# humansensinglab/AGenDA

Hardware: AMD Instinct MI355X
Metric: 512x512 images/sec + DAAM heatmaps, 50 DDIM steps, SD-1.5 (higher is better)
Workload: dtype bf16

## Files before the change

### agenda_amd/_lib.py

```python
from __future__ import annotations

import ctypes as C
import os

_HERE = os.path.dirname(os.path.abspath(__file__))
LIB_PATH = os.environ.get("AGD_LIB") or os.path.join(_HERE, "libagenda_hip.so")
AGD_MAX_LEVELS = 8
AGD_N_CLASSES = 11


class AgdConfig(C.Structure):
    _fields_ = [
        ("struct_size", C.c_int),
        ("in_channels", C.c_int), ("out_channels", C.c_int), ("n_levels", C.c_int),
        ("block_out_channels", C.c_int * AGD_MAX_LEVELS),
        ("down_cross", C.c_int * AGD_MAX_LEVELS),
        ("num_heads", C.c_int * AGD_MAX_LEVELS),
        ("layers_per_block", C.c_int), ("cross_attention_dim", C.c_int),
        ("use_linear_projection", C.c_int), ("norm_num_groups", C.c_int),
        ("vae_latent_channels", C.c_int), ("vae_out_channels", C.c_int), ("vae_n_levels", C.c_int),
        ("vae_block_out_channels", C.c_int * AGD_MAX_LEVELS),
        ("vae_layers_per_block", C.c_int), ("vae_norm_num_groups", C.c_int),
        ("vae_scaling_factor", C.c_float),
        ("max_tokens", C.c_int),
# ... 70 lines not shown
    "agd_adapter_configure": (C.c_int, [_P, C.POINTER(AgdAdapterConfig)]),
    "agd_adapter_set_cond_hw": (C.c_int, [_P, _P, C.c_int, C.c_int, C.c_int, C.c_int, _P]),
    "agd_adapter_features": (C.c_int, [_P, _P]),
    "agd_adapter_set_schedule": (C.c_int, [_P, C.POINTER(C.c_float), C.c_int]),
    "agd_adapter_clear": (C.c_int, [_P]),
    "agd_adapter_add_counts": (C.c_int, [_P, C.POINTER(C.c_longlong)]),
    "agd_ip_adapter_begin": (C.c_int, [_P, C.c_int, C.c_int]),
    "agd_ip_adapter_tensor": (C.c_int, [_P, C.c_char_p, _P, C.c_int, C.c_int, C.POINTER(C.c_longlong)]),
    "agd_ip_adapter_commit": (C.c_int, [_P]),
    "agd_ip_adapter_unload": (C.c_int, [_P]),
    "agd_ip_adapter_set": (C.c_int, [_P, _P, C.c_int, C.c_float, _P]),
    "agd_ip_adapter_clear": (C.c_int, [_P]),
    "agd_ip_adapter_tokens": (C.c_int, [_P, _P]),
    "agd_ip_adapter_block": (C.c_int, [_P, C.c_char_p, _P, C.c_int, C.c_int, C.c_int, _P, _P]),
    "agd_ip_adapter_counts": (C.c_int, [_P, C.POINTER(C.c_longlong)]),
    "agd_image_encoder_begin": (C.c_int, [_P, C.POINTER(AgdVisionConfig)]),
    "agd_image_encoder_tensor": (C.c_int, [_P, C.c_char_p, _P, C.c_int, C.c_int, C.POINTER(C.c_longlong)]),
    "agd_image_encoder_commit": (C.c_int, [_P]),
    "agd_image_encoder_unload": (C.c_int, [_P]),
    "agd_image_embeds": (C.c_int, [_P, _P, C.c_int, C.c_int, C.c_int, _P, _P]),
    "agd_gligen_configure": (C.c_int, [_P, C.POINTER(AgdGligenConfig)]),
    "agd_gligen_set": (C.c_int, [_P, _P, _P, _P, C.c_int, _P]),
    "agd_gligen_set_schedule": (C.c_int, [_P, C.POINTER(C.c_int), C.c_int]),
    "agd_gligen_clear": (C.c_int, [_P]),
    "agd_gligen_objs": (C.c_int, [_P, _P]),
    "agd_gligen_fuser": (C.c_int, [_P, C.c_char_p, _P, C.c_int, C.c_int, C.c_int, _P, _P]),
    "agd_lora_add": (C.c_int, [_P, C.c_char_p, _P, _P, C.c_int, C.c_float]),
    "agd_lora_set_scale": (C.c_int, [_P, C.c_float, _P]),
    "agd_lora_clear": (C.c_int, [_P]),
    "agd_lora_count": (C.c_int, [_P]),
    "agd_lora_scale": (C.c_float, [_P]),
    "agd_unet_forward": (C.c_int, [_P, _P, C.c_int, C.c_int, C.c_float, _P, _P]),
    "agd_unet_forward_ts": (C.c_int, [_P, _P, C.c_int, C.c_int, C.POINTER(C.c_float), _P, _P]),
    "agd_cfg_ddim_step": (C.c_int, [_P, _P, _P, C.c_int, C.c_int, C.c_float, C.c_float, C.c_float, _P]),
    "agd_denoise": (C.c_int, [_P, _P, C.c_int, C.c_int, C.c_int, C.POINTER(C.c_float), C.POINTER(C.c_float),
                              C.POINTER(C.c_float), C.c_float, _P]),
    "agd_denoise_plms": (C.c_int, [_P, _P, C.c_int, C.c_int, C.c_int, C.POINTER(C.c_float), C.POINTER(C.c_float),
                                   C.POINTER(C.c_float), C.c_float, _P]),
    "agd_denoise_dpm": (C.c_int, [_P, _P, C.c_int, C.c_int, C.c_int, C.POINTER(C.c_float), C.POINTER(C.c_float), C.c_float, _P]),
    "agd_vae_decode": (C.c_int, [_P, _P, C.c_int, C.c_int, _P, _P, _P]),
    "agd_vae_encode": (C.c_int, [_P, _P, C.c_int, C.c_int, _P, _P, _P]),
    "agd_safety_scores_hw": (C.c_int, [_P, _P, C.c_int, C.c_int, C.c_int, _P, _P, _P]),
    "agd_controlnet_set_cond_hw": (C.c_int, [_P, _P, C.c_int, C.c_int, C.c_int, C.c_int, _P]),
    "agd_controlnet_residuals_hw": (C.c_int, [_P, _P, C.c_int, C.c_int, C.c_int, C.c_float, C.c_float, C.c_int, _P, C.POINTER(C.c_longlong), _P]),
    "agd_inpaint_prepare_hw": (C.c_int, [_P, _P, C.c_int, _P, C.c_int, C.c_int, C.c_int, C.c_int, _P, _P, _P, _P]),
    "agd_inpaint_set_hw": (C.c_int, [_P, _P, C.c_int, _P, C.c_int, _P, C.c_int, C.c_int, C.c_int, _P]),
    "agd_unet_forward_hw": (C.c_int, [_P, _P, C.c_int, C.c_int, C.c_int, C.c_float, _P, _P]),
    "agd_unet_forward_ts_hw": (C.c_int, [_P, _P, C.c_int, C.c_int, C.c_int, C.POINTER(C.c_float), _P, _P]),
    "agd_cfg_ddim_step_hw": (C.c_int, [_P, _P, _P, C.c_int, C.c_int, C.c_int, C.c_float, C.c_float, C.c_float, _P]),
    "agd_denoise_hw": (C.c_int, [_P, _P, C.c_int, C.c_int, C.c_int, C.c_int, C.POINTER(C.c_float), C.POINTER(C.c_float),
                                 C.POINTER(C.c_float), C.c_float, _P]),
    "agd_denoise_plms_hw": (C.c_int, [_P, _P, C.c_int, C.c_int, C.c_int, C.c_int, C.POINTER(C.c_float), C.POINTER(C.c_float),
                                      C.POINTER(C.c_float), C.c_float, _P]),
    "agd_denoise_dpm_hw": (C.c_int, [_P, _P, C.c_int, C.c_int, C.c_int, C.c_int, C.POINTER(C.c_float), C.POINTER(C.c_float), C.c_float, _P]),
    "agd_vae_decode_hw": (C.c_int, [_P, _P, C.c_int, C.c_int, C.c_int, _P, _P, _P]),
    "agd_vae_encode_hw": (C.c_int, [_P, _P, C.c_int, C.c_int, C.c_int, _P, _P, _P]),
    "agd_record_reset_hw": (C.c_int, [_P, C.c_int, C.c_int, C.c_int, _P]),
    "agd_set_option": (C.c_int, [_P, C.c_char_p, C.c_int]),
    "agd_record_config": (C.c_int, [_P, C.c_int, C.c_int, C.c_int]),
    "agd_record_reset": (C.c_int, [_P, C.c_int, C.c_int, _P]),
    "agd_daam_global": (C.c_int, [_P, C.c_int, C.c_int, _P, _P]),
    "agd_hook_global": (C.c_int, [_P, _P, _P]),
    "agd_hook_count": (C.c_int, [_P]),
    "agd_hook_last_map": (C.c_int, [_P, _P, C.c_int, _P]),
    "agd_cross_attn": (C.c_int, [_P, C.c_char_p, _P, _P, C.c_int, C.c_int, C.c_int, _P, C.c_int, _P]),
    "agd_attn_processor": (C.c_int, [_P, C.c_char_p, _P, _P, _P, C.c_int, C.c_int, C.c_int, _P, C.c_int, _P]),
    "agd_hook_reset": (C.c_int, [_P, C.c_int, C.c_int, _P]),
    "agd_hook_num_maps": (C.c_int, [_P]),
    "agd_hook_map_dims": (C.c_int, [_P, C.c_int, C.POINTER(C.c_int)]),
    "agd_hook_map": (C.c_int, [_P, C.c_int, _P, _P]),
    "agd_op_attn_reg_loss": (C.c_int, [_P, C.c_int, C.c_int, C.c_int, _P, _P, _P, C.c_float, _P, _P, _P]),
    "agd_attn_processor_backward": (C.c_int, [_P, C.c_char_p, _P, _P, _P, _P, C.c_int, C.c_int, C.c_int, C.c_int, _P, _P, _P]),
    "agd_op_conv2d": (C.c_int, [_P, _P, _P, _P] + [C.c_int] * 9 + [_P]),
    "agd_op_conv2d_ex": (C.c_int, [_P, _P, _P, _P] + [C.c_int] * 10 + [_P]),
    "agd_op_linear": (C.c_int, [_P, _P, _P, _P, _P, C.c_int, C.c_int, C.c_int, C.c_int, _P]),
    "agd_op_groupnorm": (C.c_int, [_P, _P, _P, _P, C.c_int, C.c_int, C.c_int, C.c_int, C.c_float, C.c_int, _P]),
    "agd_op_groupnorm_ex": (C.c_int, [_P] * 5 + [C.c_int] * 5 + [C.c_float, C.c_int, _P, C.c_int, _P, C.c_int, C.POINTER(C.c_int), _P]),
    "agd_op_gn_fold": (C.c_int, [_P, _P] + [C.c_int] * 5 + [C.c_float] + [_P] * 4 + [C.c_int, C.c_int] + [_P] * 5 + [_P]),
    "agd_op_conv_groupnorm": (C.c_int, [_P] * 6 + [C.c_int] * 6 + [C.c_float, C.c_int, C.c_int, _P]),
    "agd_op_layernorm": (C.c_int, [_P, _P, _P, _P, C.c_int, C.c_int, C.c_float, _P]),
    "agd_op_layernorm_ex": (C.c_int, [_P, _P, _P, _P, C.c_int, C.c_int, C.c_float, C.POINTER(C.c_int), _P]),
    "agd_op_ff_fused": (C.c_int, [_P] * 8 + [C.c_int, C.c_int, C.c_float, _P]),
    "agd_op_attn_chain": (C.c_int, [_P] * 9 + [C.c_int] * 5 + [C.c_float, _P]),
    "agd_op_xattn_premul": (C.c_int, [_P] * 9 + [C.c_int] * 5 + [C.c_float, _P]),
    "agd_op_attention": (C.c_int, [_P, _P, _P, _P, C.c_int, C.c_int, C.c_int, C.c_int, C.c_int, C.c_float, _P, _P]),
    "agd_op_attention_ex": (C.c_int, [_P, _P, _P, _P] + [C.c_int] * 5 + [C.c_float, C.c_int, _P, _P, _P, C.c_int, C.c_int, _P, C.c_int, C.c_int, C.c_int, _P]),
    "agd_op_attention_long": (C.c_int, [_P, _P, _P, _P] + [C.c_int] * 5 + [C.c_float, C.c_int, _P, C.c_int, C.c_int, _P]),
    "agd_op_attention_headsum": (C.c_int, [_P, _P, _P, _P, C.c_int, C.c_int, C.c_int, C.c_int, C.c_int, C.c_float, _P, _P]),
    "agd_op_attention_backward": (C.c_int, [_P, _P, _P, _P] + [C.c_int] * 6 + [C.c_float, _P, _P, _P]),
    "agd_op_hook_headmean": (C.c_int, [_P, C.c_int, C.c_int, C.c_int, C.c_int, _P, _P]),
    "agd_op_bicubic_clamp_mean": (C.c_int, [_P, C.c_int, C.c_int, C.c_int, C.c_int, _P, _P]),
    "agd_op_heatmap_u8": (C.c_int, [_P, C.c_int, C.c_int, _P, _P]),
    "agd_op_resize_u8_pil": (C.c_int, [_P, C.c_int, C.c_int, C.c_int, C.c_int, C.c_int, C.c_int, _P, _P]),
    "agd_op_stack_heatmaps": (C.c_int, [_P, _P, _P, C.c_longlong, _P, _P, _P]),
    "agd_op_window_gather": (C.c_int, [_P, _P] + [C.c_int] * 8 + [_P]),
    "agd_op_window_mean": (C.c_int, [_P, _P] + [C.c_int] * 6 + [_P]),
    "agd_denoise_panorama": (C.c_int, [_P, _P] + [C.c_int] * 7 + [C.POINTER(C.c_float)] * 3 + [C.c_float, _P]),
    "agd_daam_global_panorama": (C.c_int, [_P, C.c_int, C.c_int, _P, _P]),
    "agd_freeu_set": (C.c_int, [_P] + [C.c_float] * 4),
    "agd_freeu_clear": (C.c_int, [_P]),
    "agd_freeu_counts": (C.c_int, [_P, C.POINTER(C.c_longlong)]),
    "agd_op_freeu": (C.c_int, [_P, _P, _P, _P] + [C.c_int] * 5 + [C.c_float, C.c_float, _P]),
    "agd_guidance_rescale_set": (C.c_int, [_P, C.c_float]),
    "agd_guidance_rescale_clear": (C.c_int, [_P]),
    "agd_guidance_rescale_counts": (C.c_int, [_P, C.POINTER(C.c_longlong)]),
    "agd_op_guidance_rescale": (C.c_int, [_P, _P] + [C.c_int] * 4 + [C.c_float, C.c_float, _P, _P]),
    "agd_pag_set": (C.c_int, [_P, C.POINTER(C.c_float), C.c_int, C.POINTER(C.c_char_p), C.c_int]),
    "agd_pag_clear": (C.c_int, [_P]),
    "agd_pag_counts": (C.c_int, [_P, C.POINTER(C.c_longlong), C.POINTER(C.c_longlong)]),
    "agd_op_pag_v_rows": (C.c_int, [_P, _P, _P, C.c_int, C.c_int, _P]),
    "agd_op_pag_fold": (C.c_int, [_P, _P, C.c_longlong, C.c_float, _P]),
    "agd_deepcache_set": (C.c_int, [_P, C.POINTER(C.c_int), C.c_int, C.c_int]),
    "agd_deepcache_clear": (C.c_int, [_P]),
    "agd_deepcache_counts": (C.c_int, [_P, C.POINTER(C.c_longlong)]),
    "agd_deepcache_forward_hw": (C.c_int, [_P, _P, C.c_int, C.c_int, C.c_int, C.c_float, C.c_int, C.c_int, _P, _P]),
    "agd_op_deepcache_capture": (C.c_int, [_P, _P, _P, C.c_longlong, _P, _P, C.c_longlong, _P]),
    "agd_profile_begin": (C.c_int, [_P]),
    "agd_profile_end": (C.c_int, [_P, C.POINTER(C.c_double), C.POINTER(C.c_double), C.POINTER(C.c_longlong)]),
    "agd_profile_end_ex": (C.c_int, [_P, C.c_double, C.c_double] + [C.POINTER(C.c_double)] * 5 + [C.POINTER(C.c_longlong)]),
    "agd_profile_class_name": (C.c_char_p, [C.c_int]),
    "agd_version": (C.c_char_p, []),
}

EXPORTS = tuple(_SIGS.keys())
_lib = None


def load():
    global _lib
    if _lib is not None:
        return _lib
    if not os.path.exists(LIB_PATH):
        raise AgendaHipError(
            f"{LIB_PATH} not found: build it with `python -c 'import __graft_entry__ as g; g.build()'` "
            "or `make -C agenda_amd/csrc`. There is no CPU fallback.")
    lib = C.CDLL(LIB_PATH)
    for name, (res, args) in _SIGS.items():
        fn = getattr(lib, name)
        fn.restype = res
        fn.argtypes = args
    _lib = lib
    return lib


def check(rc: int, ctx=None, what: str = ""):
    if rc != 0:
        msg = load().agd_last_error(ctx)
        raise AgendaHipError(f"{what} failed (rc={rc}): {msg.decode() if msg else '?'}")


def ptr(t):
    if t is None:
        return None
    assert t.is_contiguous(), "tensor must be contiguous"
    return C.c_void_p(t.data_ptr())


def current_stream_ptr():
    import torch
    return C.c_void_p(torch.cuda.current_stream().cuda_stream)
```

### agenda_amd/csrc/kernels.h

```cpp
#pragma once
#include "common.h"

#define AGD_MAX_DEVICES 16
struct SplitKWs { float* p = nullptr; size_t cap = 0; };

struct IgemmP {
  const bf16_t* sc0 = nullptr; const bf16_t* sc1 = nullptr; int sc_C0 = 0, sc_C1 = 0;
  int ups4 = 0;
  const bf16_t* src0; const bf16_t* src1;
  int C0, C1;
  int Hin, Win, Hout, Wout;
  int ksize, stride, pad, up;
  const bf16_t* W;
  const float* bias; int bias_mode;
  const float* rowadd; int rowadd_ld;
  const bf16_t* residual; int ldr;
  void* out; int out_f32; int ldo;
  int M, N, K;
  float alpha;
  int geglu;
  int act;
  int batch;
  long long sA0, sA1, sW, sO, sR;
  const bf16_t* zero_page;
  SplitKWs* ws;
  float* splitk_ws;
  int colstat_rows;
  float* colstat_out;
  float* rowstat_out; int rowstat_slots;
  const float* ln_stats; int ln_slots; const float* ln_cs; float ln_invC, ln_eps;
  int* cfg_out;
  int w_per_image;
  int wmajor;
  int warm;
  int halo;
  int p8;
  const float* gn_gamma; const float* gn_beta; bf16_t* gn_y; int gn_groups; float gn_eps; int gn_silu; int gn_keep_out; int* gn_fused;
  int kg2;
  int smap;
  int wreg, wreg_mmin, wreg_mmax;
  const bf16_t* Wfrag; int wfrag_ni;
  int xb_m, xb_n;
  int xcd_block;
  int pc;
  int stagger;
  int dbg;
};
int launch_igemm(const IgemmP& p, hipStream_t st);
int igemm_query(const IgemmP& p, int* cfg3);

struct AttnP {
  const bf16_t* q; const bf16_t* k; const bf16_t* v; bf16_t* o;
  int ldq, ldk, ldv, ldo;
  long long sq, sk, sv, so;
  int B, H, D, Nq, Nk;
  float scale;
  int record_mode; int rec_b0;
  float* rec; long long rec_img_stride; long long rec_head_stride;
  int rec_T;
  int rec_hpb;
  int nqt;
  int causal;
  const float* mask;
  const bf16_t* k2; const bf16_t* v2; int ldk2, ldv2; long long sk2, sv2; int Nk2;
};
int launch_attention(const AttnP& p, hipStream_t st);
constexpr int ATTN_LONG_MAX_KEYS = 320;
int launch_attention_long(const AttnP& p, hipStream_t st);

struct FFusedP {
  const bf16_t* h; bf16_t* out;
  const bf16_t* w1f;
  const float* cs1; const float* b1;
  const bf16_t* w2f;
  const float* b2;
  int M; float ln_eps;
  const bf16_t* wpf; const float* bp; const bf16_t* xres; bf16_t* pout; float* colstat;
  int xres_rows;
  int premul;
};
int launch_ff_fused(const FFusedP& p, int C, hipStream_t st);
struct AttnChainP {
  const bf16_t* h; bf16_t* out;
  const float* gamma; const float* beta; float ln_eps;
  const bf16_t* wqf;
  const bf16_t* wof; const float* bo;
  const bf16_t* kv; int ldkv; long long skv;
  int M, HW, T; float scale;
  int record; float* rec; long long rec_img_stride, rec_head_stride; int rec_T, rec_b0, rec_hpb;
  float* rowstat_out;
  const bf16_t* o1; const bf16_t* wo1f; const float* bo1;
  int rows32;
  int src_rows;
};
int launch_attn_chain(const AttnChainP& p, int C, int heads, hipStream_t st);
struct QkvChainP {
  const bf16_t* x;
  const bf16_t* wbf; long long wb_stride; const float* rowadd;
  bf16_t* h;
  const float* gamma; const float* beta; float ln_eps;
  const bf16_t* wqkvf;
  bf16_t* qkv;
  int M, HW;
  long long rowadd_stride;
  const float* gn_part; int gn_bm, gn_groups; float gn_eps; const float* gn_gamma; const float* gn_beta;
  int rows64;
  int sched2;
};
int launch_qkv_chain(const QkvChainP& p, int C, hipStream_t st);
int launch_frag_order_w1(const bf16_t* src, bf16_t* dst, int C, int HID, hipStream_t st);
int launch_frag_order_w(const bf16_t* src, bf16_t* dst, int N, int K, int NI, int KC, hipStream_t st);

#define XATTN_TP 80
struct XattnPremulP {
  const bf16_t* kv; int ldkv; long long skv;
  const bf16_t* wqT;
  const bf16_t* wo;
  const float* gamma; const float* wqb;
  int B, T, C, H; float scale;
  bf16_t* kpp; float* kcs; float* kbs; bf16_t* vpp;
};
int launch_xattn_premul(const XattnPremulP& p, hipStream_t st);
struct XattnSP {
  const bf16_t* x;
  const float* ln_stats; int ln_slots; float ln_invC, ln_eps;
  const bf16_t* kpp; const float* kcs; const float* kbs;
  bf16_t* P;
  int M, HW, C, H, T;
  float* rec; long long rec_img_stride, rec_head_stride; int rec_T, rec_b0;
};
int launch_xattn_s(const XattnSP& p, hipStream_t st);
int launch_matvec_bf16(const bf16_t* W, const float* v, float* out, int N, int K, hipStream_t st);
int launch_rowstat_bf16(const bf16_t* x, float* out, int M, int C, hipStream_t st);

struct GroupNormP {
  const bf16_t* x0; const bf16_t* x1; int C0, C1;
  bf16_t* y;
  const float* gamma; const float* beta;
  int B, HW, groups; float eps; int silu;
  float* ws;
  const float* part0; const float* part1; int bm0, bm1;
  int* path;
};
int groupnorm_check(int B, int C0, int C1, int HW, int groups);
int layernorm_check(int rows, int C);
int launch_groupnorm(const GroupNormP& p, hipStream_t st);
int launch_gn_fold_weight(const float* part, int bm, int B, int HW, int C, int groups, float eps, const float* gamma, const float* beta,
                          const bf16_t* W, const float* bias, int N, bf16_t* Wb, float* rowadd, hipStream_t st, int frag_ni = 0);
long long groupnorm_ws_floats(int B, int C, int HW, int groups);
int launch_layernorm(const bf16_t* x, bf16_t* y, const float* g, const float* b, int rows, int C, float eps, hipStream_t st,
                     int* inst = nullptr);

int launch_convert_weight(const float* w, bf16_t* out, int N, int Cin, int taps, int Cpad, int geglu_bn, hipStream_t st);
int launch_f32_to_bf16(const float* x, bf16_t* y, long long n, hipStream_t st);
int launch_bf16_to_f32(const bf16_t* x, float* y, long long n, hipStream_t st);
bool igemm_can_fuse_shortcut(const IgemmP& p);
int launch_upsample_phase_weight(const bf16_t* w, bf16_t* out, int Cout, int Cin, hipStream_t st);
int launch_prep_latents(const float* lat_nchw, bf16_t* out_nhwc, int B, int C, int HW, int Cpad, int dup, float scale, hipStream_t st);
int launch_timestep_embed(float t, float* out, int dim, hipStream_t st);
int launch_small_linear(const float* x, const bf16_t* W, const float* bias, float* out, int M, int N, int K, int silu_in,
                        int silu_out, hipStream_t st);
int launch_cfg_ddim(const float* eps_nhwc, int ldc, float* lat_nchw, int B, int C, int HW, float guidance,
                    float a_t, float a_p, int vpred, const float* factor, hipStream_t st);
int launch_cfg_plms(const float* eps_nhwc, int ldc, float* lat, const float* src, const float* h1, const float* h2, const float* h3,
                    float* store, int B, int C, int HW, float guidance, const float* w4, float a, float b, const float* factor, hipStream_t st);
int launch_cfg_dpm(const float* eps_nhwc, int ldc, float* lat, const float* prev, float* store, int B, int C, int HW, float guidance,
                   const float* coef5 , const float* factor, hipStream_t st);
int launch_guidance_factor(const float* eps_nhwc, int ldc, int B, int C, int HW, float guidance, float phi, float* factor, hipStream_t st);
int launch_ln_fold_weight(const bf16_t* W, const float* gamma, const float* beta, const float* bias, int N, int K, int geglu_bn, bf16_t* Wf,
                          float* colsum, float* bias_f, hipStream_t st);
int launch_image_u8(const float* x_nhwc, int ldc, unsigned char* out, long long npix, int C, hipStream_t st);
int launch_nchw_from_nhwc_f32(const float* x, int ldc, float* out, int B, int C, int HW, hipStream_t st);
int launch_softmax_rows(const float* s, bf16_t* p, int rows, int cols, hipStream_t st);

struct HeatLayer { const float* acc; int h, w; int heads; long long img_stride; long long head_stride; };
int launch_daam_global(const HeatLayer* layers, int n_layers, int total_maps, int T, int Sh, int Sw, int img, float* out, hipStream_t st);
int launch_hook_accum(const float* map, int B, int T, int side, int S, float* sum, hipStream_t st);
int launch_scale(float* x, long long n, float s, hipStream_t st);
// ... 83 lines not shown
```

### agenda_amd/csrc/model.hip

```cpp
#include "../../include/agenda_hip.h"
#include "kernels.h"

#include <algorithm>
#include <cmath>
#include <cstdarg>
#include <cstdio>
#include <cstring>
#include <functional>
#include <string>
#include <unordered_map>
#include <unordered_set>
#include <vector>

static thread_local char g_err[2048] = "";
#define AGD_API extern "C" __attribute__((visibility("default")))
extern "C" void agd_set_error(const char* fmt, ...) {
  va_list ap; va_start(ap, fmt); vsnprintf(g_err, sizeof(g_err), fmt, ap); va_end(ap);
}
#define CK(expr) do { if ((expr) != 0) return -1; } while (0)
#define FAIL(...) do { agd_set_error(__VA_ARGS__); return -1; } while (0)

struct WMat { bf16_t* w = nullptr; int N = 0, Cin = 0, Cpad = 0, taps = 0;
              int sc_cols = 0;
              bf16_t* wfrag = nullptr; int wfrag_ni = 0; };
struct Act { bf16_t* p = nullptr; int B = 0, H = 0, W = 0, C = 0; float* cpart = nullptr; int cpart_bm = 0;
             bf16_t* normed = nullptr; const float* normed_gamma = nullptr;
             long long n() const { return (long long)B * H * W * C; } };
struct NextGn { const float* gamma = nullptr; const float* beta = nullptr; float eps = 0.f; int silu = 0; };

struct Arena {
  char* base = nullptr; size_t cap = 0, off = 0, peak = 0;
  void* alloc(size_t bytes) {
    size_t a = (off + 255) & ~(size_t)255;
    if (a + bytes > cap) { agd_set_error("activation arena exhausted: need %zu + %zu > %zu bytes (raise workspace_bytes)", a, bytes, cap); return nullptr; }
    off = a + bytes; if (off > peak) peak = off;
    return base + a;
  }
  size_t mark() const { return off; }
  void release(size_t m) { off = m; }
};

enum { PC_CONV3 = 0, PC_GEMM, PC_ATTN_SELF, PC_ATTN_CROSS, PC_GN, PC_LN, PC_ELEM, PC_HEAT, PC_VAE_ATTN, PC_OTHER, PC_TOUCH };
static const char* kClassNames[AGD_N_CLASSES] = {"igemm_conv3x3", "igemm_linear_1x1", "attn_self_flash", "attn_cross_daam",
                                                 "groupnorm", "layernorm", "elementwise", "heatmap", "vae_attn_softmax", "other", "weight_touch"};

struct DBuf {
  void* p = nullptr; size_t cap = 0;
  template <typename T> T* as() const { return (T*)p; }
  int ensure(size_t bytes) {
    if (p && bytes <= cap) return 0;
    if (p) { (void)hipDeviceSynchronize(); (void)hipFree(p); p = nullptr; cap = 0; }
    const size_t want = bytes ? bytes : 256;
    if (hipMalloc(&p, want) != hipSuccess) { p = nullptr; agd_set_error("hipMalloc(%zu) failed", want); return -1; }
    cap = want;
    return 0;
  }
  void release() { if (p) (void)hipFree(p); p = nullptr; cap = 0; }
};

struct XLayer {
  std::string name; int C = 0, heads = 0, level = 0; bool mid = false;
  bool cn = false;
  WMat wkv; DBuf kvb; bf16_t* kv = nullptr; DBuf accb; float* acc = nullptr; int acc_h = 0, acc_w = 0;
  int acc_heads = 0;
  DBuf wqTb, wkvTb, woTb; WMat wqT, wkvT, woT;
  bf16_t* pm_wqT = nullptr; float* pm_wqb = nullptr; bool pm_ready = false;
  DBuf pm_kppb, pm_vppb, pm_csb; bf16_t* pm_kpp = nullptr; bf16_t* pm_vpp = nullptr; float* pm_kcs = nullptr; float* pm_kbs = nullptr;
};

struct Fuser {
  std::string pre; int C = 0, heads = 0;
  WMat wqkv, wkv; float ta = 0.f, td = 0.f; float* bo_s = nullptr; float* b2_s = nullptr;
  DBuf gkvb;
};

struct IpaLayer {
  std::string pre; int C = 0, heads = 0, cols = 0;
  DBuf wk, wv, kppb, vppb, csbsb;
};

enum : int {
  TBF_FF            = 1 << 0,
  TBF_ATTN2         = 1 << 1,
  TBF_ATTN1_OUT     = 1 << 2,
  TBF_FF_PROJ       = 1 << 3,
  TBF_QKV           = 1 << 4,
  TBF_ATTN2_640     = 1 << 5,
  TBF_LAZY_DUP      = 1 << 6,
  TBF_QKV_GN        = 1 << 7,
  TBF_QKV_640       = 1 << 8,
  TBF_FF_PREMUL     = 1 << 9,
  TBF_ATTN2_ROWS32  = 1 << 10,
  TBF_QKV_ROWS64    = 1 << 11,
  TBF_QKV_SCHED2    = 1 << 12,
  TBF_DEFAULT       = 0x1fff & ~TBF_QKV_640,
};

struct ProfEv { int cls; double flops, bytes; hipEvent_t a, b; };

struct EvalCond {
  float cn_scale = 0.f;
  bool grounded = false;
  float ad_scale = 0.f;
  bool ipa = false;
  bool pag = false;
  int dc = 0;
  int dc_branch = 0;
};
enum : int { DC_CAPTURE = 1, DC_SHALLOW = 2 };

struct agd_ctx {
  int device = 0; agd_config cfg{}; std::string err;
  std::unordered_map<std::string, WMat> W;
  std::unordered_map<std::string, float*> V;
  std::unordered_map<std::string, int> Vn;
  std::vector<void*> owned;
  Arena arena; bf16_t* zero_page = nullptr;
  float* stage = nullptr; size_t stage_bytes = 0;
  bool finalized = false;
  WMat tproj_all; float* tproj_bias = nullptr; float* tproj_out = nullptr; int tproj_total = 0;
  const float* tproj_cur = nullptr;
  int tproj_cur_ld = 0;
  float* tsteps_buf = nullptr; int tsteps_cap = 0;
  std::unordered_map<std::string, int> tproj_off;
  float* temb_buf = nullptr;
  float* t_dev = nullptr;
  std::vector<XLayer> xl; std::unordered_map<std::string, int> xl_idx;
  DBuf ctxb; bf16_t* ctx_bf16 = nullptr; int ctx_B2 = 0, ctx_T = 0;
  int rec_mode = 0, rec_is_train = 0, rec_T_cfg = 0, rec_T = 0, rec_B = 0, rec_L = 0, rec_Lh = 0, rec_Lw = 0;
  DBuf hook_sumb, hook_scratchb, hook_headsb, hook_storeb;
  struct HookRec { size_t off; int Bp, T, N; };
  std::vector<HookRec> hook_recs; size_t hook_store_used = 0;
  DBuf bwd_wsb;
  float* hook_sum = nullptr; float* hook_scratch = nullptr; int hook_count = 0, hook_Bp = 0, hook_T = 0;
  int rec_base = 0, rec_call = 0;
  int pano_B = 0, pano_Lh = 0, pano_Lw = 0, pano_stride = 0;
  DBuf pano_ctxb;
  DBuf pano_viewb, pano_hmb;
  DBuf latb, epsb, vae_imgb, plmsb, dpmb;
  bf16_t* lat_bf16 = nullptr; float* eps_nhwc = nullptr;
  SplitKWs splitk;
  int opt_cfg_share = 1;
  int opt_ln_fold = 1;
  int opt_gn_fused = 1;
  int opt_warm = 3;
  int opt_gn_proj_fold = 1;
  int opt_p8 = 1;
  int opt_halo = 1;
  int opt_tb_fuse = TBF_DEFAULT;
  int opt_ups4 = 7;
  int opt_ffproj = 1;
  int opt_sc_fuse = 3;
  int opt_wreg = 3;
  int opt_kg2 = 1;
  int opt_side = 0;
  hipStream_t side = nullptr; hipEvent_t ev_fork = nullptr, ev_join = nullptr;
  int opt_smap = 1;
  int opt_reduce_gn = 1;
  int opt_xcd_block = 1;
  int opt_pc = 49;
  agd_vision_config vis{}; bool vis_on = false; float* vis_concepts = nullptr;
  agd_vision_config ienc{}; int ienc_state = 0;
  int opt_xpre = 1;
  int opt_touch = 3;
  unsigned* touch_sink = nullptr;
  agd_controlnet_config cnc{}; bool cn_on = false;
  WMat cn_tproj_all; float* cn_tproj_bias = nullptr; float* cn_tproj_out = nullptr; int cn_tproj_total = 0;
  int cn_nres = 0; float* cn_zb = nullptr; float* cn_zbs = nullptr; int cn_zb_total = 0; std::vector<int> cn_zb_off; float cn_zscale = NAN;
  DBuf cn_embb; int cn_emb_B2 = 0, cn_emb_Lh = 0, cn_emb_Lw = 0, cn_emb_rep = 0;
  std::vector<float> cn_sched;
  int ip_mode = 0, ip_B = 0, ip_Lh = 0, ip_Lw = 0, ip_Cm = 0, ip_Cc = 0;
  DBuf ip_maskb, ip_condb, ip_noiseb;
  std::vector<float> ip_sched;
  bool i2_on = false; int i2_B = 0, i2_Lh = 0, i2_Lw = 0; float i2_scale = 1.f;
  int i2_prep_B = 0, i2_prep_Lh = 0, i2_prep_Lw = 0;
  DBuf i2_latb;
  std::vector<std::string> lora_keys; std::vector<LoraMergeD> lora_d; int lora_tiles = 0;
// ... 340 lines not shown
  if (long_ctx && a.record_mode != 0) {
    const double fl = 6.0 * a.B * a.H * (double)a.Nq * a.Nk * a.D;
    const double by = 2.0 * a.B * a.H * (double)a.D * (2.0 * a.Nq + 3.0 * a.Nk) + 8.0 * (a.B - a.rec_b0) * a.H * (double)a.rec_T * a.Nq;
    ProfScope ps(c, st, PC_ATTN_CROSS, fl, by);
    CK(launch_attention_long(a, st));
  } else CK(run_attention(c, st, PC_ATTN_CROSS, a));
  if (hook_call) {
    ProfScope ps(c, st, PC_HEAT, 0);
    CK(launch_hook_headmean(c->hook_headsb.as<float>(), c->hook_Bp, xl.heads, T, N, c->hook_scratch, st));
    if (c->rec_is_train) {
      const size_t bytes = (size_t)c->hook_Bp * T * N * 4, need = c->hook_store_used + bytes;
      if (need > c->hook_storeb.cap) {
        DBuf bigger; CK(bigger.ensure(need * 2 > ((size_t)64 << 20) ? need * 2 : ((size_t)64 << 20)));
        if (c->hook_store_used && hipMemcpyAsync(bigger.p, c->hook_storeb.p, c->hook_store_used, hipMemcpyDeviceToDevice, st) != hipSuccess) FAIL("hook store copy");
        hipStreamSynchronize(st);
        c->hook_storeb.release(); c->hook_storeb = bigger;
      }
      if (hipMemcpyAsync((char*)c->hook_storeb.p + c->hook_store_used, c->hook_scratch, bytes, hipMemcpyDeviceToDevice, st) != hipSuccess) FAIL("hook store");
      c->hook_recs.push_back({c->hook_store_used, c->hook_Bp, T, N});
      c->hook_store_used = need;
    }
    CK(launch_hook_accum(c->hook_scratch, c->hook_Bp, T, side, c->rec_L, c->hook_sum, st));
    c->hook_count++;
  }
  return 0;
}

static int fuser_rows(agd_ctx* c, hipStream_t st, const Fuser& f, bf16_t* h, int B, int HW, bf16_t* qkv, bf16_t* att,
                      const std::function<int(const bf16_t*, int, const WMat&, const GemmOpt&)>& last) {
  const int C = f.C, D = C / f.heads, M = B * HW, NO = c->glc.max_objs;
  if (B != c->gl_B2) FAIL("gligen: the grounding objects are set for %d rows, this forward has %d (agd_gligen_set)", c->gl_B2, B);
  const std::string t = f.pre + "transformer_blocks.0.fuser.";
  bf16_t* n = (bf16_t*)c->arena.alloc((size_t)M * C * 2); bf16_t* ff = (bf16_t*)c->arena.alloc((size_t)M * 4 * C * 2);
  if (!n || !ff) return -1;
  GETV(g1, t + "norm1.weight"); GETV(b1, t + "norm1.bias"); GETV(g2, t + "norm2.weight"); GETV(b2, t + "norm2.bias");
  GETW(wo, t + "attn.to_out.0.weight"); GETW(w1, t + "ff.net.0.proj.weight"); GETV(bb1, t + "ff.net.0.proj.bias"); GETW(w2, t + "ff.net.2.weight");
  { ProfScope ps(c, st, PC_LN, 0, 4.0 * M * (double)C); CK(launch_layernorm(h, n, g1, b1, M, C, 1e-5f, st)); }
  { GemmOpt o; CK(run_conv(c, st, n, C, nullptr, 0, 1, 1, M, f.wqkv, 1, qkv, o, c->zero_page)); }
  AttnP a{}; a.q = qkv; a.k = qkv + C; a.v = qkv + 2 * C; a.o = att;
  a.ldq = a.ldk = a.ldv = 3 * C; a.ldo = C; a.sq = a.sk = a.sv = (long long)HW * 3 * C; a.so = (long long)HW * C;
  a.B = B; a.H = f.heads; a.D = D; a.Nq = HW; a.Nk = HW; a.scale = 1.0f / sqrtf((float)D);
  a.k2 = f.gkvb.as<bf16_t>(); a.v2 = a.k2 + C; a.ldk2 = a.ldv2 = 2 * C; a.sk2 = a.sv2 = (long long)NO * 2 * C; a.Nk2 = NO;
  { const double fl = 4.0 * B * f.heads * (double)HW * (HW + NO) * D, by = 2.0 * B * (double)C * (4.0 * HW + 2.0 * NO);
    ProfScope ps(c, st, PC_ATTN_SELF, fl, by); CK(launch_attention(a, st)); }
  { GemmOpt o; o.bias = f.bo_s; o.alpha = f.ta; o.residual = h; CK(run_conv(c, st, att, C, nullptr, 0, 1, 1, M, *wo, 1, h, o, c->zero_page)); }
  { ProfScope ps(c, st, PC_LN, 0, 4.0 * M * (double)C); CK(launch_layernorm(h, n, g2, b2, M, C, 1e-5f, st)); }
  { GemmOpt o; o.bias = bb1; o.geglu = 1; CK(run_conv(c, st, n, C, nullptr, 0, 1, 1, M, *w1, 1, ff, o, c->zero_page)); }
  GemmOpt o; o.bias = f.b2_s; o.alpha = f.td; o.residual = h;
  return last(ff, 4 * C, *w2, o);
}

static int dup_half(agd_ctx* c, hipStream_t st, bf16_t* p, long long half_elems) {
  ProfScope ps(c, st, PC_ELEM, 0);
  if (hipMemcpyAsync(p + half_elems, p, (size_t)half_elems * 2, hipMemcpyDeviceToDevice, st) != hipSuccess) FAIL("dup_half copy failed");
  return 0;
}

enum TbHead  { HEAD_GN,
               HEAD_FOLD,
               HEAD_QKV,
               HEAD_QKV_GN };
enum TbDup   { DUP_NONE, DUP_COPY,
               DUP_LAZY };
enum TbAttn2 { ATTN2_CHAIN,
               ATTN2_PREMUL,
               ATTN2_KERNELS };
enum TbFf    { FF_FUSED,
               FF_FUSED_PROJ,
               FF_FUSED_PREMUL,
               FF_FFPROJ,
               FF_PLAIN };

struct TBlockPlan {
  bool fold;
  bool x_normed;
  bool gfold;
  TbHead head; int qkv_rows64, qkv_sched2;
  bool attn1_in_chain;
  TbDup dup;
  const Fuser* fuser;
  const IpaLayer* ipa;
  XLayer* xl;
  TbAttn2 attn2; int chain_rows32;
  bool daam;
  TbFf ff;
  bool wreg_proj;
  bool stats_head, stats_attn1, stats_attn2;
  bool stats_ipa;
};

static const float kTbLnEps = 1e-5f;

struct TBlock {
  agd_ctx* c; hipStream_t st; const std::string& pre; const std::string t; const Act& x; Act& out; int heads, groups;
  int C, HW, Bs, B;
  const float* gn_g = nullptr; const float* gn_b = nullptr; const WMat* w_in = nullptr; const float* b_in = nullptr;
  bf16_t* ln = nullptr;
  bf16_t* h = nullptr; bf16_t* qkv = nullptr; bf16_t* att = nullptr;
  const bf16_t* xres;
  int M; const int Mshared;
  float* stats = nullptr; int slots = 0;
  bf16_t* ipaP = nullptr;
  TBlock(agd_ctx* c_, hipStream_t st_, const std::string& pre_, const Act& x_, Act& out_, int heads_, int groups_, int dup)
    : c(c_), st(st_), pre(pre_), t(pre_ + "transformer_blocks.0."), x(x_), out(out_), heads(heads_), groups(groups_), C(x_.C), HW(x_.H * x_.W),
      Bs(x_.B), B(dup ? 2 * x_.B : x_.B), xres(x_.p), M(x_.B * x_.H * x_.W), Mshared(M) {}

  int produce(const bf16_t* A, int K, const WMat& w, GemmOpt o, bool shaped, bool want_stats) {
    const int gb_ = shaped ? M / HW : 1, gh_ = shaped ? x.H : 1, gw_ = shaped ? x.W : M;
    stats = nullptr; slots = 0;
    if (want_stats) {
      int cfg[3] = {0, 0, 0}; GemmOpt qo = o; qo.query_cfg = cfg; qo.want_rowstat = 1;
      CK(run_conv(c, st, A, K, nullptr, 0, gb_, gh_, gw_, w, 1, h, qo, c->zero_page));
      slots = (w.N + cfg[1] - 1) / cfg[1];
      stats = (float*)c->arena.alloc((size_t)B * HW * slots * 2 * sizeof(float)); if (!stats) return -1;
      o.rowstat_out = stats; o.rowstat_slots = slots;
    }
    return run_conv(c, st, A, K, nullptr, 0, gb_, gh_, gw_, w, 1, h, o, c->zero_page);
  }
  int consume(bool fold, const std::string& lnkey, const std::string& wkey, const float* bias, int geglu, bf16_t* outp) {
    if (fold) {
      const std::string k = wkey + ".lnfold";
      GETW(wf, k); GETV(cs, k + ".cs"); GETV(bf, k + ".bias");
      GemmOpt o; o.bias = bf; o.geglu = geglu; o.ln_stats = stats; o.ln_slots = slots; o.ln_cs = cs; o.ln_invC = 1.0f / (float)C; o.ln_eps = kTbLnEps;
      if (geglu && C == 1280 && M >= 1024 && M <= 4096 && (c->opt_wreg & 1) && wf->wfrag) o.wreg = 2;
      return run_conv(c, st, h, C, nullptr, 0, 1, 1, M, *wf, 1, outp, o, c->zero_page);
    }
    GETV(g, lnkey + ".weight"); GETV(b, lnkey + ".bias");
    { ProfScope ps(c, st, PC_LN, 0, 4.0 * M * (double)C); CK(launch_layernorm(h, ln, g, b, M, C, kTbLnEps, st)); }
    GETW(w, wkey); GemmOpt o; o.bias = bias; o.geglu = geglu;
    return run_conv(c, st, ln, C, nullptr, 0, 1, 1, M, *w, 1, outp, o, c->zero_page);
  }
};

static TBlockPlan tblock_plan(const TBlock& s, int dup) {
  agd_ctx* c = s.c; const Act& x = s.x; const std::string& pre = s.pre; const std::string& t = s.t;
  const int C = s.C, HW = s.HW, heads = s.heads, groups = s.groups;
  auto tb = [c](int bit) { return (c->opt_tb_fuse & bit) != 0; };
  auto has = [c](const std::string& key) { return c->W.count(key) != 0; };
  TBlockPlan p{};
  p.fold = c->opt_ln_fold == 1 || (c->opt_ln_fold == 2 && C <= 320) || (c->opt_ln_fold == 3 && C <= 640);
  p.x_normed = x.normed && x.normed_gamma == s.gn_g;
  p.wreg_proj = C == 640 && (c->opt_wreg & 2);
  const bool sums = c->opt_gn_fused && x.cpart && x.cpart_bm > 0 && HW % x.cpart_bm == 0;
  p.gfold = c->opt_gn_proj_fold && sums && C <= (c->opt_gn_proj_fold >= 2 ? 640 : 320) && HW % 128 == 0;
  if (p.gfold) {
    const bool qkv = tb(TBF_QKV) && C == 320 && s.w_in->N == C && has(t + "attn1.qkv.frag");
    const bool gn_inside = qkv && tb(TBF_QKV_GN) && groups <= 32 && has(pre + "proj_in.frag");
    p.head = gn_inside ? HEAD_QKV_GN : qkv ? HEAD_QKV : HEAD_FOLD;
    p.qkv_rows64 = qkv && tb(TBF_QKV_ROWS64) && HW % 64 == 0;
  } else if (C == 640 && tb(TBF_QKV) && tb(TBF_QKV_640) && tb(TBF_QKV_GN) && sums && HW % 64 == 0 && groups <= 32 && !p.x_normed && !dup &&
             has(pre + "proj_in.frag") && has(t + "attn1.qkv.frag")) {
    p.head = HEAD_QKV_GN;
  } else p.head = HEAD_GN;
  p.qkv_sched2 = tb(TBF_QKV_SCHED2);
  const bool ff_fused = tb(TBF_FF) && p.fold && C == 320 && has(t + "ff.w1.frag");
  if (ff_fused) {
    const bool proj = tb(TBF_FF_PROJ) && has(pre + "proj_out.frag");
    p.ff = !proj ? FF_FUSED : tb(TBF_FF_PREMUL) && has(t + "ff.w2p.frag") ? FF_FUSED_PREMUL : FF_FUSED_PROJ;
  } else p.ff = c->opt_ffproj && has(pre + "ffproj.weight") ? FF_FFPROJ : FF_PLAIN;
  auto itx = c->xl_idx.find(t + "attn2");
  p.xl = itx == c->xl_idx.end() ? nullptr : &c->xl[itx->second];
  p.daam = p.xl && daam_records(c, *p.xl, s.B, x.H, x.W);
  const bool premul = p.xl && p.xl->pm_ready && c->opt_xpre && p.fold && HW % 64 == 0 && c->rec_mode != 2 && c->ctx_T <= XATTN_TP && !dup &&
                      (!p.daam || p.xl->acc_heads == p.xl->heads);
  const bool chain = !premul && tb(TBF_ATTN2) && (C == 320 || (C == 640 && tb(TBF_ATTN2_640))) && heads == 8 && HW % (C == 320 ? 128 : 64) == 0 &&
                     c->ctx_T <= 96 && c->rec_mode != 2 && has(t + "attn2.to_q.frag");
  p.attn2 = premul ? ATTN2_PREMUL : chain ? ATTN2_CHAIN : ATTN2_KERNELS;
  p.chain_rows32 = tb(TBF_ATTN2_ROWS32);
  if (c->cur.grounded) { auto itf = c->gl_idx.find(pre); if (itf != c->gl_idx.end()) p.fuser = &c->gl_f[itf->second]; }
  if (c->cur.ipa) { auto iti = c->ipa_idx.find(pre); if (iti != c->ipa_idx.end()) p.ipa = &c->ipa_l[iti->second]; }
  const bool lazy = dup && tb(TBF_LAZY_DUP) && chain && C == 320 && (p.ff == FF_FUSED_PROJ || p.ff == FF_FUSED_PREMUL) && !p.fuser && !p.ipa;
  p.dup = !dup ? DUP_NONE : lazy ? DUP_LAZY : DUP_COPY;
  p.attn1_in_chain = chain && tb(TBF_ATTN1_OUT) && p.dup != DUP_COPY && has(t + "attn1.to_out.frag") && !p.fuser && !p.ipa;
  p.stats_head = p.fold; p.stats_attn1 = p.fold && !chain; p.stats_attn2 = p.fold && !ff_fused && !p.ipa; p.stats_ipa = p.fold && !ff_fused && p.ipa;
  return p;
}

static int qkv_chain_params(const TBlock& s, const TBlockPlan& p, const bf16_t* wb, const float* radd, QkvChainP& qp) {
  agd_ctx* c = s.c; const Act& x = s.x; const int C = s.C;
  GETW(fqkv, s.t + "attn1.qkv.frag"); GETV(g1, s.t + "norm1.weight"); GETV(b1, s.t + "norm1.bias");
  qp.x = x.p; qp.wbf = wb; qp.wb_stride = (long long)s.w_in->N * C; qp.rowadd = radd; qp.rowadd_stride = C; qp.h = s.h; qp.gamma = g1; qp.beta = b1; qp.ln_eps = kTbLnEps;
  qp.wqkvf = fqkv->w; qp.qkv = s.qkv; qp.M = s.M; qp.HW = s.HW; qp.rows64 = p.qkv_rows64; qp.sched2 = p.qkv_sched2;
  if (p.head == HEAD_QKV_GN) {
    GETW(fpi, s.pre + "proj_in.frag");
    if (!s.b_in) FAIL("proj_in without bias");
    qp.wbf = fpi->w; qp.wb_stride = 0; qp.rowadd = s.b_in; qp.rowadd_stride = 0;
    qp.gn_part = x.cpart; qp.gn_bm = x.cpart_bm; qp.gn_groups = s.groups; qp.gn_eps = 1e-6f; qp.gn_gamma = s.gn_g; qp.gn_beta = s.gn_b;
  }
  return 0;
}

static int tb_head(TBlock& s, const TBlockPlan& p) {
  agd_ctx* c = s.c; hipStream_t st = s.st; const Act& x = s.x; const WMat* w = s.w_in; const int C = s.C;
  if (p.head == HEAD_GN) {
    if (p.x_normed) s.ln = x.normed;
    else CK(run_gn(c, st, x.p, C, nullptr, 0, s.Bs, s.HW, s.gn_g, s.gn_b, s.groups, 1e-6f, 0, s.ln, &x));
    GemmOpt o; o.bias = s.b_in;
    if (p.wreg_proj) o.wreg = 1;
    return s.produce(s.ln, C, *w, o, false, p.stats_head);
  }
  if (p.gfold) { if (w->taps != 1 || w->Cpad != C) FAIL("gn_proj_fold: proj_in weight [N=%d taps=%d Cpad=%d] is not a 1x1 over %d channels", w->N, w->taps, w->Cpad, C); }
  else if (w->taps != 1 || w->Cpad != C || w->N != C || !s.b_in) FAIL("qkv chain: proj_in weight [N=%d taps=%d Cpad=%d] is not a biased 1x1 over %d channels", w->N, w->taps, w->Cpad, C);
  bf16_t* wb = nullptr; float* radd = nullptr;
  if (p.head != HEAD_QKV_GN) {
    wb = (bf16_t*)c->arena.alloc((size_t)s.Bs * w->N * C * 2);
    radd = (float*)c->arena.alloc((size_t)s.Bs * w->N * sizeof(float));
    if (!wb || !radd) return -1;
    ProfScope ps(c, st, PC_GN, 0, 2.0 * s.Bs * (double)w->N * C * 2);
    CK(launch_gn_fold_weight(x.cpart, x.cpart_bm, s.Bs, s.HW, C, s.groups, 1e-6f, s.gn_g, s.gn_b, w->w, s.b_in, w->N, wb, radd, st, p.head == HEAD_QKV ? C / 64 : 0));
  }
  if (p.head == HEAD_FOLD) {
    WMat wi = *w; wi.w = wb;
    GemmOpt o; o.rowadd = radd; o.rowadd_ld = w->N; o.w_per_image = 1;
    return s.produce(x.p, C, wi, o, true, p.stats_head);
  }
  QkvChainP qp{}; CK(qkv_chain_params(s, p, wb, radd, qp));
  s.stats = nullptr; s.slots = 0;
  ProfScope ps(c, st, PC_GEMM, 8.0 * s.M * (double)C * C, 2.0 * s.M * (double)C * 5.0 + 2.0 * (p.gfold ? s.Bs + 3.0 : 4.0) * C * (double)C);
  return launch_qkv_chain(qp, C, st);
}

static int tb_self_attention(TBlock& s, const TBlockPlan& p) {
  agd_ctx* c = s.c; const std::string& t = s.t; const int C = s.C, HW = s.HW, D = C / s.heads;
  if (p.head == HEAD_GN || p.head == HEAD_FOLD) CK(s.consume(p.fold, t + "norm1", t + "attn1.qkv", nullptr, 0, s.qkv));
  AttnP a{}; a.q = s.qkv; a.k = s.qkv + C; a.v = s.qkv + 2 * C; a.o = s.att;
  a.ldq = a.ldk = a.ldv = 3 * C; a.ldo = C; a.sq = a.sk = a.sv = (long long)HW * 3 * C; a.so = (long long)HW * C;
  a.B = s.Bs; a.H = s.heads; a.D = D; a.Nq = HW; a.Nk = HW; a.scale = 1.0f / sqrtf((float)D);
  if (c->cur.pag && c->pag_layers.count(s.pre)) {
    const double M = (double)s.Bs * HW;
    ProfScope ps(c, s.st, PC_ELEM, 0, 4.0 * M * C);
    CK(launch_pag_v_rows(s.qkv, s.att, s.Bs * HW, C, s.st));
    c->pag_counts[1]++;
  } else CK(run_attention(c, s.st, PC_ATTN_SELF, a));
  if (p.attn1_in_chain) return 0;
  GETW(wo, t + "attn1.to_out.0.weight"); GETV(bo, t + "attn1.to_out.0.bias");
  GemmOpt oo; oo.bias = bo; oo.residual = s.h;
  return s.produce(s.att, C, *wo, oo, false, p.stats_attn1);
}

static int tb_duplicate(TBlock& s, const TBlockPlan& p) {
  agd_ctx* c = s.c; hipStream_t st = s.st; const int C = s.C, M = s.Mshared;
  if (p.dup == DUP_NONE) return 0;
  s.M = s.B * s.HW;
  if (p.dup == DUP_LAZY) return 0;
  CK(dup_half(c, st, s.h, (long long)M * C));
  if (p.stats_attn1) { ProfScope ps(c, st, PC_ELEM, 0);
    if (hipMemcpyAsync(s.stats + (size_t)M * s.slots * 2, s.stats, (size_t)M * s.slots * 2 * sizeof(float), hipMemcpyDeviceToDevice, st) != hipSuccess) FAIL("dup stats copy failed"); }
  Act x2 = alloc_act(c, s.B, s.x.H, s.x.W, C); if (!x2.p) return -1;
  { ProfScope ps(c, st, PC_ELEM, 0);
    if (hipMemcpyAsync(x2.p, s.x.p, (size_t)M * C * 2, hipMemcpyDeviceToDevice, st) != hipSuccess) FAIL("dup copy failed"); }
  CK(dup_half(c, st, x2.p, (long long)M * C));
  s.xres = x2.p;
  return 0;
}

static int tb_fuser(TBlock& s, const TBlockPlan& p) {
  return fuser_rows(s.c, s.st, *p.fuser, s.h, s.B, s.HW, s.qkv, s.att,
                    [&](const bf16_t* A, int K, const WMat& w, const GemmOpt& o) { return s.produce(A, K, w, o, false, p.stats_attn1); });
}

static int ipa_scores_rows(agd_ctx* c, hipStream_t st, const IpaLayer& l, const bf16_t* h, int B, int HW, bf16_t* P) {
  if (B != c->ipa_B2) FAIL("ip_adapter: the image tokens are set for %d rows, this forward has %d (agd_ip_adapter_set)", c->ipa_B2, B);
  IpaScoreP sp{}; sp.h = h; sp.kpp = l.kppb.as<bf16_t>(); sp.cs = l.csbsb.as<float>(); sp.bs = sp.cs + (size_t)B * l.cols; sp.P = P;
  sp.B = B; sp.HW = HW; sp.C = l.C; sp.H = l.heads; sp.nt = c->ipa_nt; sp.colsP = l.cols; sp.eps = 1e-5f;
  const double M = (double)B * HW;
  ProfScope ps(c, st, PC_ATTN_CROSS, 2.0 * M * l.cols * l.C, 2.0 * M * l.C + 2.0 * B * (double)l.cols * l.C + 2.0 * M * l.cols);
  return launch_ipa_scores(sp, st);
}
static int ipa_add_rows(agd_ctx* c, hipStream_t st, const IpaLayer& l, bf16_t* h, int B, int HW, const bf16_t* P) {
  IpaAddP ap{}; ap.h = h; ap.P = P; ap.vpp = l.vppb.as<bf16_t>(); ap.B = B; ap.HW = HW; ap.C = l.C; ap.colsP = l.cols; ap.s = c->ipa_scale;
  const double M = (double)B * HW;
  ProfScope ps(c, st, PC_ATTN_CROSS, 2.0 * M * l.cols * l.C, 4.0 * M * l.C + 2.0 * B * (double)l.cols * l.C + 2.0 * M * l.cols);
  return launch_ipa_add(ap, st);
}
static int tb_ip_adapter_scores(TBlock& s, const TBlockPlan& p) {
  agd_ctx* c = s.c;
  if (s.C != p.ipa->C) FAIL("ip_adapter: %s has %d channels, its to_k_ip / to_v_ip were loaded for %d", s.pre.c_str(), s.C, p.ipa->C);
  s.ipaP = (bf16_t*)c->arena.alloc((size_t)s.M * p.ipa->cols * 2); if (!s.ipaP) return -1;
  CK(ipa_scores_rows(c, s.st, *p.ipa, s.h, s.B, s.HW, s.ipaP));
  c->ipa_counts[0]++;
  return 0;
}
static int tb_ip_adapter_add(TBlock& s, const TBlockPlan& p) {
  agd_ctx* c = s.c;
  CK(ipa_add_rows(c, s.st, *p.ipa, s.h, s.B, s.HW, s.ipaP));
  c->ipa_counts[1]++;
  if (p.stats_ipa) {
    s.slots = 1; s.stats = (float*)c->arena.alloc((size_t)s.M * 2 * sizeof(float)); if (!s.stats) return -1;
    ProfScope ps(c, s.st, PC_LN, 0, 2.0 * s.M * (double)s.C);
    CK(launch_rowstat_bf16(s.h, s.stats, s.M, s.C, s.st));
  }
  return 0;
}

static int tb_attn2_chain(TBlock& s, const TBlockPlan& p) {
  agd_ctx* c = s.c; const std::string& t = s.t; const XLayer& xl = *p.xl; const int C = s.C, HW = s.HW, B = s.B, M = s.M, heads = s.heads;
  GETW(fq, t + "attn2.to_q.frag"); GETW(fo, t + "attn2.to_out.frag");
  GETV(g2, t + "norm2.weight"); GETV(b2, t + "norm2.bias"); GETV(bo, t + "attn2.to_out.0.bias");
  const int T = c->ctx_T, D = C / heads;
  AttnChainP ap{}; ap.h = s.h; ap.out = s.h; ap.gamma = g2; ap.beta = b2; ap.ln_eps = kTbLnEps; ap.wqf = fq->w; ap.wof = fo->w; ap.bo = bo;
  ap.kv = xl.kv; ap.ldkv = 2 * C; ap.skv = (long long)T * 2 * C; ap.M = M; ap.HW = HW; ap.T = T; ap.scale = 1.0f / sqrtf((float)D);
  double rec_bytes = 0;
  if (p.daam) {
    ap.record = 1; ap.rec_b0 = B / 2; ap.rec_T = c->rec_T; ap.rec_hpb = heads / xl.acc_heads;
    ap.rec_head_stride = (long long)c->rec_T * HW; ap.rec_img_stride = ap.rec_head_stride * xl.acc_heads;
    ap.rec = xl.acc + (size_t)c->rec_base * ap.rec_img_stride;
    rec_bytes = 8.0 * (B - ap.rec_b0) * xl.acc_heads * (double)c->rec_T * HW;
  }
  if (p.attn1_in_chain || p.dup == DUP_LAZY) {
    ap.out = (bf16_t*)c->arena.alloc((size_t)M * C * 2); if (!ap.out) return -1;
  }
  if (p.attn1_in_chain) {
    GETW(f1o, t + "attn1.to_out.frag"); GETV(bo1, t + "attn1.to_out.0.bias");
    ap.o1 = s.att; ap.wo1f = f1o->w; ap.bo1 = bo1;
  }
  if (p.dup == DUP_LAZY) ap.src_rows = s.Mshared;
  ap.rows32 = p.chain_rows32;
  if (p.stats_attn2) {
    s.slots = 1; s.stats = (float*)c->arena.alloc((size_t)M * 2 * sizeof(float)); if (!s.stats) return -1;
    ap.rowstat_out = s.stats;
  }
  const double gemms = p.attn1_in_chain ? 6.0 : 4.0;
  ProfScope ps(c, s.st, PC_ATTN_CROSS, gemms * M * (double)C * C + 4.0 * B * heads * (double)HW * T * D, gemms * M * (double)C + gemms * C * (double)C + 4.0 * B * (double)T * C + rec_bytes);
  CK(launch_attn_chain(ap, C, heads, s.st));
  s.h = ap.out;
  return 0;
}

static int tb_attn2_premul(TBlock& s, const TBlockPlan& p) {
  agd_ctx* c = s.c; const XLayer& xl = *p.xl; const int C = s.C, HW = s.HW, B = s.B, M = s.M, heads = s.heads;
  if (!s.stats || s.slots <= 0) FAIL("attn2_premul: the GEMM in front of attn2 left no row statistics for norm2");
  GETV(bo, s.t + "attn2.to_out.0.bias");
  const int HT = heads * XATTN_TP;
  bf16_t* P = (bf16_t*)c->arena.alloc((size_t)M * HT * 2); if (!P) return -1;
  XattnSP sp{}; sp.x = s.h; sp.ln_stats = s.stats; sp.ln_slots = s.slots; sp.ln_invC = 1.0f / (float)C; sp.ln_eps = kTbLnEps;
  sp.kpp = xl.pm_kpp; sp.kcs = xl.pm_kcs; sp.kbs = xl.pm_kbs; sp.P = P; sp.M = M; sp.HW = HW; sp.C = C; sp.H = heads; sp.T = c->ctx_T;
  double rec_bytes = 0;
  if (p.daam) {
    sp.rec_b0 = B / 2; sp.rec_T = c->rec_T; sp.rec_head_stride = (long long)c->rec_T * HW; sp.rec_img_stride = sp.rec_head_stride * xl.acc_heads;
    sp.rec = xl.acc + (size_t)c->rec_base * sp.rec_img_stride;
    rec_bytes = 8.0 * (B - sp.rec_b0) * heads * (double)c->rec_T * HW;
  }
  { ProfScope ps(c, s.st, PC_ATTN_CROSS, 2.0 * M * (double)HT * C, 2.0 * M * (double)C + 2.0 * B * (double)HT * C + 2.0 * M * (double)HT + rec_bytes);
    CK(launch_xattn_s(sp, s.st)); }
  WMat wv; wv.w = xl.pm_vpp; wv.N = C; wv.Cin = HT; wv.Cpad = HT; wv.taps = 1;
  GemmOpt oo; oo.bias = bo; oo.residual = s.h; oo.w_per_image = 1;
  return s.produce(P, HT, wv, oo, true, p.stats_attn2);
}

static int tb_attn2(TBlock& s, const TBlockPlan& p) {
  agd_ctx* c = s.c; const std::string& t = s.t;
  if (!p.xl) FAIL("cross-attn layer %s not registered", (t + "attn2").c_str());
  if (c->ctx_B2 != s.B) FAIL("context batch %d != unet batch %d (call agd_set_context)", c->ctx_B2, s.B);
  if (p.attn2 == ATTN2_CHAIN) return tb_attn2_chain(s, p);
  if (p.attn2 == ATTN2_PREMUL) return tb_attn2_premul(s, p);
  CK(s.consume(p.fold, t + "norm2", t + "attn2.to_q.weight", nullptr, 0, s.qkv));
  CK(cross_attention(c, s.st, *p.xl, s.qkv, s.B, s.HW, s.x.H, s.x.W, s.att, true));
  GETW(wo, t + "attn2.to_out.0.weight"); GETV(bo, t + "attn2.to_out.0.bias");
  GemmOpt oo; oo.bias = bo; oo.residual = s.h;
  return s.produce(s.att, s.C, *wo, oo, false, p.stats_attn2);
}

static int tb_ff_fused(TBlock& s, const TBlockPlan& p) {
  agd_ctx* c = s.c; const std::string& t = s.t; Act& out = s.out; const int C = s.C, M = s.M;
  GETW(f1, t + "ff.w1.frag"); GETW(f2, t + "ff.w2.frag");
  const std::string k = t + "ff.net.0.proj.weight.lnfold";
  GETV(cs, k + ".cs"); GETV(bf, k + ".bias"); GETV(b2, t + "ff.net.2.bias");
  FFusedP fp{}; fp.h = s.h; fp.out = s.h; fp.w1f = f1->w; fp.cs1 = cs; fp.b1 = bf; fp.w2f = f2->w; fp.b2 = b2; fp.M = M; fp.ln_eps = kTbLnEps;
  const bool proj = p.ff != FF_FUSED;
  if (proj) {
    GETW(fpw, s.pre + "proj_out.frag"); GETV(bp, s.pre + "proj_out.bias");
    fp.wpf = fpw->w; fp.bp = bp; fp.xres = s.xres; fp.pout = out.p;
    if (p.ff == FF_FUSED_PREMUL) {
      GETW(f2p, t + "ff.w2p.frag"); GETV(bcp, s.pre + "ffproj.bias");
      fp.w2f = f2p->w; fp.bp = bcp; fp.premul = 1;
    }
    if (p.dup == DUP_LAZY) fp.xres_rows = s.Mshared;
    out.cpart_bm = 0;
    if (out.cpart && c->opt_gn_fused && s.HW % 128 == 0) { fp.colstat = out.cpart; out.cpart_bm = 128; }
  }
  ProfScope ps(c, s.st, PC_GEMM, 2.0 * M * (double)C * (proj ? 13.0 : 12.0) * C, (proj ? 8.0 : 4.0) * M * (double)C + 2.0 * (proj ? 13.0 : 12.0) * C * (double)C);
  return launch_ff_fused(fp, C, s.st);
}

static int tb_feed_forward(TBlock& s, const TBlockPlan& p) {
  agd_ctx* c = s.c; hipStream_t st = s.st; const std::string& t = s.t; const int C = s.C, M = s.M;
  if (p.ff == FF_FUSED || p.ff == FF_FUSED_PROJ || p.ff == FF_FUSED_PREMUL) CK(tb_ff_fused(s, p));
  else {
    bf16_t* ff = (bf16_t*)c->arena.alloc((size_t)M * 4 * C * 2); if (!ff) return -1;
    GETV(b1, t + "ff.net.0.proj.bias");
    CK(s.consume(p.fold, t + "norm3", t + "ff.net.0.proj.weight", b1, 1, ff));
    if (p.ff == FF_FFPROJ) {
      GETW(wc, s.pre + "ffproj.weight"); GETV(bc, s.pre + "ffproj.bias");
      GemmOpt o; o.bias = bc; o.residual = s.xres; o.out_act = &s.out; o.rows_per_image = s.HW;
      return run_conv(c, st, ff, 4 * C, s.h, C, 1, 1, M, *wc, 1, s.out.p, o, c->zero_page);
    }
    GETW(w2, t + "ff.net.2.weight"); GETV(b2, t + "ff.net.2.bias");
    GemmOpt o2; o2.bias = b2; o2.residual = s.h;
    CK(run_conv(c, st, ff, 4 * C, nullptr, 0, 1, 1, M, *w2, 1, s.h, o2, c->zero_page));
  }
  if (p.ff != FF_FUSED && p.ff != FF_PLAIN) return 0;
  GETW(w, s.pre + "proj_out.weight"); GETV(b, s.pre + "proj_out.bias");
  GemmOpt o; o.bias = b; o.residual = s.xres; o.out_act = &s.out; o.rows_per_image = s.HW;
  if (p.wreg_proj) o.wreg = 1;
  return run_conv(c, st, s.h, C, nullptr, 0, 1, 1, M, *w, 1, s.out.p, o, c->zero_page);
}

static int transformer(agd_ctx* c, hipStream_t st, const std::string& pre, const Act& x, int heads, int groups, Act& out, int dup = 0) {
  TBlock s(c, st, pre, x, out, heads, groups, dup);
  const int B = s.B, HW = s.HW, C = s.C;
  out = alloc_act(c, B, x.H, x.W, C, true); if (!out.p) return -1;
  const size_t mk = c->arena.mark();
  Act n = alloc_act(c, B, x.H, x.W, C); if (!n.p) return -1;
  Act h = alloc_act(c, B, x.H, x.W, C); if (!h.p) return -1;
  s.ln = n.p; s.h = h.p;
  s.qkv = (bf16_t*)c->arena.alloc((size_t)B * HW * 3 * C * 2); if (!s.qkv) return -1;
  s.att = (bf16_t*)c->arena.alloc((size_t)B * HW * C * 2); if (!s.att) return -1;
  GETV(gg, pre + "norm.weight"); GETV(gb, pre + "norm.bias"); GETW(w_in, pre + "proj_in.weight"); GETV(b_in, pre + "proj_in.bias");
  s.gn_g = gg; s.gn_b = gb; s.w_in = w_in; s.b_in = b_in;
  const TBlockPlan p = tblock_plan(s, dup);
  CK(tb_head(s, p));
  CK(tb_self_attention(s, p));
  CK(tb_duplicate(s, p));
  if (p.fuser) CK(tb_fuser(s, p));
  if (p.ipa) CK(tb_ip_adapter_scores(s, p));
  CK(tb_attn2(s, p));
  if (p.ipa) CK(tb_ip_adapter_add(s, p));
  CK(tb_feed_forward(s, p));
  c->arena.release(mk);
  return 0;
}

static int time_embed(agd_ctx* c, hipStream_t st, const float* ts, int n, float* scratch, float* out, bool cn = false) {
  const int dim = c->cfg.block_out_channels[0], td = dim * 4;
  const std::string pre = cn ? "controlnet." : "unet.";
  ProfScope ps(c, st, PC_ELEM, 0);
  float* e0 = scratch; float* e1 = e0 + (size_t)n * dim; float* e2 = e1 + (size_t)n * td;
  for (int i = 0; i < n; ++i) CK(launch_timestep_embed(ts[i], e0 + (size_t)i * dim, dim, st));
  GETW(w1, pre + "time_embedding.linear_1.weight"); GETV(b1, pre + "time_embedding.linear_1.bias");
  GETW(w2, pre + "time_embedding.linear_2.weight"); GETV(b2, pre + "time_embedding.linear_2.bias");
  CK(launch_small_linear(e0, w1->w, b1, e1, n, td, w1->Cpad, 0, 1, st));
  CK(launch_small_linear(e1, w2->w, b2, e2, n, td, w2->Cpad, 0, 0, st));
  if (cn) CK(launch_small_linear(e2, c->cn_tproj_all.w, c->cn_tproj_bias, out, n, c->cn_tproj_total, td, 1, 0, st));
  else CK(launch_small_linear(e2, c->tproj_all.w, c->tproj_bias, out, n, c->tproj_total, td, 1, 0, st));
  return 0;
}

static int adapter_add(agd_ctx* c, hipStream_t st, int level, const Act& h, Act& out);
static int down_mid_walk(agd_ctx* c, hipStream_t st, const std::string& u, const bf16_t* xin, int B2, int Lh, int Lw, bool shared,
                         const bf16_t* conv_in_res, const std::function<int(const Act&)>& on_sample, Act& h, int stop_layer = -1) {
  const agd_config& g = c->cfg;
  const int nl = g.n_levels, G = g.norm_num_groups;
  const int Bh = shared ? B2 / 2 : B2;
  const bool inject = c->cur.ad_scale != 0.f && u == "unet.";
  h = alloc_act(c, B2, Lh, Lw, g.block_out_channels[0], true); if (!h.p) return -1;
  { GETW(w, u + "conv_in.weight"); GETV(b, u + "conv_in.bias"); GemmOpt o; o.bias = b; o.out_act = &h; o.residual = conv_in_res;
    CK(run_conv(c, st, xin, 64, nullptr, 0, Bh, Lh, Lw, *w, 3, h.p, o, c->zero_page)); }
  if (shared) {
    CK(dup_half(c, st, h.p, (long long)Bh * Lh * Lw * h.C));
    if (h.cpart_bm > 0) {
      const size_t nb = (size_t)((long long)Bh * Lh * Lw / h.cpart_bm) * h.C * 2 * sizeof(float);
      if (hipMemcpyAsync((char*)h.cpart + nb, h.cpart, nb, hipMemcpyDeviceToDevice, st) != hipSuccess) FAIL("dup partials copy failed");
    }
  }
// ... 2018 lines not shown
  int bm = 0;
  if (fused) {
    int cfg[3] = {0, 0, 0};
    CK(igemm_query(p, cfg));
    bm = cfg[0];
    if (cfg[2] != 1 || bm < 1 || HW % bm || HW % 64) { agd_set_error("op_conv_groupnorm: shape not eligible for producer statistics (tile %d, splits %d)", cfg[0], cfg[2]); return -1; }
    p.colstat_out = part; p.colstat_rows = HW;
  }
  CK(launch_igemm(p, st));
  GroupNormP g{}; g.x0 = hb; g.C0 = Cout; g.y = yb; g.gamma = gamma; g.beta = beta; g.B = B; g.HW = HW; g.groups = groups; g.eps = eps; g.silu = silu; g.ws = ws;
  if (fused) { g.part0 = part; g.bm0 = bm; }
  CK(launch_groupnorm(g, st));
  CK(launch_bf16_to_f32(yb, yf, (long long)B * HW * Cout, st));
  CK(launch_nchw_from_nhwc_f32(yf, Cout, y, B, Cout, HW, st));
  hipStreamSynchronize(st);
  return 0;
}

AGD_API int agd_op_layernorm_ex(const float* x, const float* gamma, const float* beta, float* y, int rows, int C, float eps, int* inst, void* stream) {
  hipStream_t st = S(stream); Tmp tmp;
  if (inst) *inst = 0;
  if (layernorm_check(rows, C)) return -1;
  bf16_t* xb = tmp.get<bf16_t>((size_t)rows * C); bf16_t* yb = tmp.get<bf16_t>((size_t)rows * C);
  if (!xb || !yb) return -1;
  CK(launch_f32_to_bf16(x, xb, (long long)rows * C, st));
  CK(launch_layernorm(xb, yb, gamma, beta, rows, C, eps, st, inst));
  CK(launch_bf16_to_f32(yb, y, (long long)rows * C, st));
  hipStreamSynchronize(st);
  return 0;
}
AGD_API int agd_op_layernorm(const float* x, const float* gamma, const float* beta, float* y, int rows, int C, float eps, void* stream) {
  return agd_op_layernorm_ex(x, gamma, beta, y, rows, C, eps, nullptr, stream);
}

AGD_API int agd_op_ff_fused(const float* x, const float* gamma, const float* beta, const float* w1, const float* b1, const float* w2,
                            const float* b2, float* y, int M, int C, float eps, void* stream) {
  hipStream_t st = S(stream); Tmp tmp;
  if (C != 320) { agd_set_error("op_ff_fused: C = %d (320 only)", C); return -1; }
  const int H8 = 8 * C, H4 = 4 * C;
  bf16_t* xb = tmp.get<bf16_t>((size_t)M * C); bf16_t* yb = tmp.get<bf16_t>((size_t)M * C);
  bf16_t* w1b = tmp.get<bf16_t>((size_t)H8 * C); bf16_t* w1l = tmp.get<bf16_t>((size_t)H8 * C); bf16_t* w1f = tmp.get<bf16_t>((size_t)H8 * C);
  bf16_t* w2b = tmp.get<bf16_t>((size_t)C * H4); bf16_t* w2f = tmp.get<bf16_t>((size_t)C * H4);
  float* cs = tmp.get<float>(H8); float* bf = tmp.get<float>(H8);
  if (!xb || !yb || !w1b || !w1l || !w1f || !w2b || !w2f || !cs || !bf) return -1;
  CK(launch_f32_to_bf16(x, xb, (long long)M * C, st));
  CK(launch_convert_weight(w1, w1b, H8, C, 1, C, 16, st));
  CK(launch_ln_fold_weight(w1b, gamma, beta, b1, H8, C, 16, w1l, cs, bf, st));
  CK(launch_frag_order_w1(w1l, w1f, C, H4, st));
  CK(launch_convert_weight(w2, w2b, C, H4, 1, H4, 0, st));
  CK(launch_frag_order_w(w2b, w2f, C, H4, C / 64, 128, st));
  FFusedP fp{}; fp.h = xb; fp.out = yb; fp.w1f = w1f; fp.cs1 = cs; fp.b1 = bf; fp.w2f = w2f; fp.b2 = b2; fp.M = M; fp.ln_eps = eps;
  CK(launch_ff_fused(fp, C, st));
  CK(launch_bf16_to_f32(yb, y, (long long)M * C, st));
  hipStreamSynchronize(st);
  return 0;
}

AGD_API int agd_op_attn_chain(const float* x, const float* gamma, const float* beta, const float* wq, const float* kv, const float* wo,
                              const float* bo, float* y, float* probs_sum, int B, int HW, int T, int C, int heads, float eps, void* stream) {
  hipStream_t st = S(stream); Tmp tmp;
  const long long M = (long long)B * HW;
  bf16_t* xb = tmp.get<bf16_t>((size_t)M * C); bf16_t* yb = tmp.get<bf16_t>((size_t)M * C); bf16_t* kvb = tmp.get<bf16_t>((size_t)B * T * 2 * C);
  bf16_t* wqb = tmp.get<bf16_t>((size_t)C * C); bf16_t* wqf = tmp.get<bf16_t>((size_t)C * C);
  bf16_t* wob = tmp.get<bf16_t>((size_t)C * C); bf16_t* wof = tmp.get<bf16_t>((size_t)C * C);
  if (!xb || !yb || !kvb || !wqb || !wqf || !wob || !wof) return -1;
  if (C != 320 && C != 640) { agd_set_error("op_attn_chain: C %d", C); return -1; }
  CK(launch_f32_to_bf16(x, xb, M * C, st));
  CK(launch_f32_to_bf16(kv, kvb, (long long)B * T * 2 * C, st));
  CK(launch_convert_weight(wq, wqb, C, C, 1, C, 0, st)); CK(launch_frag_order_w(wqb, wqf, C, C, 5, C, st));
  CK(launch_convert_weight(wo, wob, C, C, 1, C, 0, st)); CK(launch_frag_order_w(wob, wof, C, C, 5, C, st));
  AttnChainP ap{}; ap.h = xb; ap.out = yb; ap.gamma = gamma; ap.beta = beta; ap.ln_eps = eps; ap.wqf = wqf; ap.wof = wof; ap.bo = bo;
  ap.rows32 = (heads >> 8) & 1; heads &= 255;
  ap.kv = kvb; ap.ldkv = 2 * C; ap.skv = (long long)T * 2 * C; ap.M = (int)M; ap.HW = HW; ap.T = T; ap.scale = 1.0f / sqrtf((float)(C / heads));
  if (probs_sum) {
    if (hipMemsetAsync(probs_sum, 0, (size_t)B * T * HW * 4, st) != hipSuccess) { agd_set_error("memset probs"); return -1; }
    ap.record = 1; ap.rec = probs_sum; ap.rec_b0 = 0; ap.rec_T = T; ap.rec_hpb = heads; ap.rec_head_stride = (long long)T * HW; ap.rec_img_stride = (long long)T * HW;
  }
  CK(launch_attn_chain(ap, C, heads, st));
  CK(launch_bf16_to_f32(yb, y, M * C, st));
  hipStreamSynchronize(st);
  return 0;
}

AGD_API int agd_op_xattn_premul(const float* x, const float* gamma, const float* beta, const float* wq, const float* kv, const float* wo,
                                const float* bo, float* y, float* probs, int B, int HW, int T, int C, int heads, float eps, void* stream) {
  hipStream_t st = S(stream); Tmp tmp;
  const long long M = (long long)B * HW;
  if (heads < 1 || C % heads || (C / heads) % 8 || C % 160 || C % 64 || HW % 64 || T < 1 || T > XATTN_TP || (heads * XATTN_TP) % 64) { agd_set_error("op_xattn_premul: C %d heads %d HW %d T %d", C, heads, HW, T); return -1; }
  const size_t HT = (size_t)heads * XATTN_TP;
  bf16_t* xb = tmp.get<bf16_t>((size_t)M * C); bf16_t* yb = tmp.get<bf16_t>((size_t)M * C); bf16_t* kvb = tmp.get<bf16_t>((size_t)B * T * 2 * C);
  bf16_t* wqb = tmp.get<bf16_t>((size_t)C * C); bf16_t* wqT = tmp.get<bf16_t>((size_t)C * C); bf16_t* wob = tmp.get<bf16_t>((size_t)C * C);
  float* wqbeta = tmp.get<float>(C); float* rst = tmp.get<float>((size_t)M * 2);
  bf16_t* kpp = tmp.get<bf16_t>((size_t)B * HT * C); bf16_t* vpp = tmp.get<bf16_t>((size_t)B * HT * C); float* kcs = tmp.get<float>((size_t)B * HT * 2);
  bf16_t* P = tmp.get<bf16_t>((size_t)M * HT);
  if (!xb || !yb || !kvb || !wqb || !wqT || !wob || !wqbeta || !rst || !kpp || !vpp || !kcs || !P) return -1;
  CK(launch_f32_to_bf16(x, xb, M * C, st));
  CK(launch_f32_to_bf16(kv, kvb, (long long)B * T * 2 * C, st));
  CK(launch_convert_weight(wq, wqb, C, C, 1, C, 0, st)); CK(launch_transpose_bf16(wqb, C, C, wqT, st));
  CK(launch_convert_weight(wo, wob, C, C, 1, C, 0, st));
  CK(launch_matvec_bf16(wqb, beta, wqbeta, C, C, st));
  CK(launch_rowstat_bf16(xb, rst, (int)M, C, st));
  XattnPremulP pm{}; pm.kv = kvb; pm.ldkv = 2 * C; pm.skv = (long long)T * 2 * C; pm.wqT = wqT; pm.wo = wob; pm.gamma = gamma; pm.wqb = wqbeta;
  pm.B = B; pm.T = T; pm.C = C; pm.H = heads; pm.scale = 1.0f / sqrtf((float)(C / heads)); pm.kpp = kpp; pm.kcs = kcs; pm.kbs = kcs + (size_t)B * HT; pm.vpp = vpp;
  CK(launch_xattn_premul(pm, st));
  XattnSP sp{}; sp.x = xb; sp.ln_stats = rst; sp.ln_slots = 1; sp.ln_invC = 1.0f / (float)C; sp.ln_eps = eps; sp.kpp = kpp; sp.kcs = pm.kcs; sp.kbs = pm.kbs; sp.P = P;
  sp.M = (int)M; sp.HW = HW; sp.C = C; sp.H = heads; sp.T = T;
  if (probs) {
    if (hipMemsetAsync(probs, 0, (size_t)B * heads * T * HW * 4, st) != hipSuccess) { agd_set_error("memset probs"); return -1; }
    sp.rec = probs; sp.rec_b0 = 0; sp.rec_T = T; sp.rec_head_stride = (long long)T * HW; sp.rec_img_stride = sp.rec_head_stride * heads;
  }
  CK(launch_xattn_s(sp, st));
  WMat wv; wv.w = vpp; wv.N = C; wv.Cin = (int)HT; wv.Cpad = (int)HT; wv.taps = 1;
  GemmOpt oo; oo.bias = bo; oo.residual = xb; oo.w_per_image = 1;
  CK(run_conv(nullptr, st, P, (int)HT, nullptr, 0, B, 1, HW, wv, 1, yb, oo, op_zero_page()));
  CK(launch_bf16_to_f32(yb, y, M * C, st));
  hipStreamSynchronize(st);
  return 0;
}

AGD_API int agd_op_attention(const float* q, const float* k, const float* v, float* o, int B, int H, int D, int Nq, int Nk,
                                float scale, float* probs_out, void* stream) {
  hipStream_t st = S(stream); Tmp tmp;
  const int C = H * D;
  bf16_t* qb = tmp.get<bf16_t>((size_t)B * Nq * C); bf16_t* kb = tmp.get<bf16_t>((size_t)B * Nk * C);
  bf16_t* vb = tmp.get<bf16_t>((size_t)B * Nk * C); bf16_t* ob = tmp.get<bf16_t>((size_t)B * Nq * C);
  if (!qb || !kb || !vb || !ob) return -1;
  CK(launch_f32_to_bf16(q, qb, (long long)B * Nq * C, st));
  CK(launch_f32_to_bf16(k, kb, (long long)B * Nk * C, st));
  CK(launch_f32_to_bf16(v, vb, (long long)B * Nk * C, st));
  AttnP a{}; a.q = qb; a.k = kb; a.v = vb; a.o = ob; a.ldq = a.ldk = a.ldv = a.ldo = C;
  a.sq = (long long)Nq * C; a.so = a.sq; a.sk = (long long)Nk * C; a.sv = a.sk;
  a.B = B; a.H = H; a.D = D; a.Nq = Nq; a.Nk = Nk; a.scale = scale;
  if (probs_out) {
    if (hipMemsetAsync(probs_out, 0, (size_t)B * H * Nk * Nq * 4, st) != hipSuccess) { agd_set_error("memset probs"); return -1; }
    a.record_mode = 1; a.rec_b0 = 0; a.rec = probs_out; a.rec_T = Nk;
    a.rec_head_stride = (long long)Nk * Nq; a.rec_img_stride = a.rec_head_stride * H;
  }
  CK(launch_attention(a, st));
  CK(launch_bf16_to_f32(ob, o, (long long)B * Nq * C, st));
  hipStreamSynchronize(st);
  return 0;
}

AGD_API int agd_op_attention_ex(const float* q, const float* k, const float* v, float* o, int B, int H, int D, int Nq, int Nk, float scale,
                                int causal, const float* mask, const float* k2, const float* v2, int Nk2, int layout, float* probs_out,
                                int record, int rec_b0, int rec_T, void* stream) {
  if (D != 32 && D != 40 && D != 64 && D != 80 && D != 128 && D != 160) { agd_set_error("attention_ex: unsupported head dim D=%d", D); return -1; }
  if (B < 1 || H < 1 || Nq < 1 || Nk < 1) { agd_set_error("attention_ex: bad shape B=%d H=%d Nq=%d Nk=%d", B, H, Nq, Nk); return -1; }
  if (!q || !k || !v || !o) { agd_set_error("attention_ex: q, k, v and o are required"); return -1; }
  if (layout < 0 || layout > 2) { agd_set_error("attention_ex: layout=%d (0 packed, 1 fused q|k|v rows, 2 fused k|v rows)", layout); return -1; }
  if (layout == 1 && Nq != Nk) { agd_set_error("attention_ex: layout=1 (fused q|k|v rows) needs Nq == Nk (got Nq=%d Nk=%d)", Nq, Nk); return -1; }
  if (record < 0 || record > 2 || (record != 0) != (probs_out != nullptr)) { agd_set_error("attention_ex: record=%d needs probs_out, and probs_out needs record 1 or 2", record); return -1; }
  if (record && Nk > 96) { agd_set_error("attention_ex: recording needs Nk <= 96 (got Nk=%d)", Nk); return -1; }
  if (record && (rec_b0 < 0 || rec_b0 > B)) { agd_set_error("attention_ex: rec_b0=%d outside [0, %d]", rec_b0, B); return -1; }
  if (record && (rec_T < 1 || rec_T > Nk)) { agd_set_error("attention_ex: rec_T=%d outside [1, %d]", rec_T, Nk); return -1; }
  if ((k2 != nullptr) != (v2 != nullptr)) { agd_set_error("attention_ex: k2 and v2 come together"); return -1; }
  if (!k2 && Nk2 != 0) { agd_set_error("attention_ex: Nk2=%d without a second source", Nk2); return -1; }
  hipStream_t st = S(stream); Tmp tmp;
  const int C = H * D;
  const long long nq = (long long)B * Nq * C, nk = (long long)B * Nk * C, nk2 = k2 ? (long long)B * (Nk2 > 0 ? Nk2 : 0) * C : 0;
  bf16_t* qb = tmp.get<bf16_t>((size_t)nq); bf16_t* kb = tmp.get<bf16_t>((size_t)nk); bf16_t* vb = tmp.get<bf16_t>((size_t)nk);
  bf16_t* ob = tmp.get<bf16_t>((size_t)nq);
  bf16_t* k2b = k2 ? tmp.get<bf16_t>((size_t)nk2 + 8) : nullptr; bf16_t* v2b = k2 ? tmp.get<bf16_t>((size_t)nk2 + 8) : nullptr;
  bf16_t* fused = layout ? tmp.get<bf16_t>((size_t)(layout == 1 ? 3 : 2) * nk) : nullptr;
  bf16_t* fused2 = (layout && k2) ? tmp.get<bf16_t>((size_t)2 * nk2 + 8) : nullptr;
  if (!qb || !kb || !vb || !ob || (k2 && (!k2b || !v2b)) || (layout && !fused) || (layout && k2 && !fused2)) return -1;
// ... 1587 lines not shown
```

### agenda_amd/csrc/tblock.hip

```cpp
#include "kernels.h"
#include <type_traits>

typedef __attribute__((ext_vector_type(2))) float f32x2_t;
#ifdef AGD_EXPERIMENTS
int g_tb_variant = 0;
extern "C" __attribute__((visibility("default"))) void agd_set_tb_variant(int v) { g_tb_variant = v; }
#endif
#ifdef AGD_STAMPS
__device__ unsigned long long g_tb_ts[256];
__device__ int g_tb_ts_sel[2] = {-1, 0};
extern "C" __attribute__((visibility("default"))) int agd_tb_ts(int wg, int wave, unsigned long long* out) {
  if (out) return hipMemcpyFromSymbol(out, HIP_SYMBOL(g_tb_ts), 256 * 8) == hipSuccess ? 0 : -1;
  const int sel[2] = {wg, wave};
  return hipMemcpyToSymbol(HIP_SYMBOL(g_tb_ts_sel), sel, 8) == hipSuccess ? 0 : -1;
}
#define TB_TS_DECL const bool ts_on = (int)blockIdx.x == g_tb_ts_sel[0] && (int)threadIdx.x == g_tb_ts_sel[1] * 64; int ts_n = 0; if (ts_on) g_tb_ts[250] = __builtin_amdgcn_s_memrealtime();
#define TB_TS(k) do { if (ts_on && ts_n < 240) g_tb_ts[ts_n++] = ((unsigned long long)(k) << 56) | (__builtin_amdgcn_s_memtime() & 0x00FFFFFFFFFFFFFFull); } while (0)
#define TB_TS_END do { if (ts_on) { asm volatile("s_waitcnt vmcnt(0)" ::: "memory"); TB_TS(99); g_tb_ts[255] = ts_n; g_tb_ts[251] = __builtin_amdgcn_s_memrealtime(); } } while (0)
#else
#define TB_TS_DECL
#define TB_TS(k) do { } while (0)
#define TB_TS_END do { } while (0)
#endif

// ... 33 lines not shown
}
int launch_frag_order_w(const bf16_t* src, bf16_t* dst, int N, int K, int NI, int KC, hipStream_t st) {
  if (N % (NI * 16) || K % KC || KC % 32) { agd_set_error("frag_order_w: N %d K %d NI %d KC %d", N, K, NI, KC); return -1; }
  hipLaunchKernelGGL(frag_order_w_kernel, dim3(1024), dim3(256), 0, st, src, dst, N, K, NI, KC);
  HIP_CHECK_RET(hipGetLastError());
  return 0;
}

#define TB_OOB 0x80000000u
template <int C> AGD_DEV int panel_swz(int ch, int row) {
  if constexpr ((C * 2) % 256 == 128) return (ch & ~7) | ((ch & 7) ^ ((row >> 1) & 7));
  else return (ch & ~15) | ((ch & 15) ^ (row & 15));
}
template <int C> struct XOff {
  static constexpr int XG = ((C * 2) % 256 == 128) ? 2 : 4;
  int xo[4];
  AGD_DEV XOff(int q, int px) {
#pragma unroll
    for (int t = 0; t < 4; ++t) xo[t] = ((C * 2) % 256 == 128) ? (((4 * (t & 1) + q) ^ ((px >> 1) & 7)) << 4) : (((4 * t + q) ^ px) << 4);
  }
  AGD_DEV int at(int ks) const { return (ks / XG) * (XG * 64) + xo[ks % XG]; }
};

template <int C, int BM = 128, int NW = 8>
AGD_DEV void panel_load_dma(const bf16_t* src, int m0, int M, char* panel, int wid, int lane) {
  constexpr int CHR = C / 8, PIECES = BM * CHR / 64;
  static_assert(PIECES % NW == 0, "pieces split evenly over the workgroup's waves");
#pragma unroll
  for (int i = 0; i < PIECES / NW; ++i) {
    const int piece = i * NW + wid, pos = piece * 64 + lane;
    const int row = pos / CHR, pc = pos - row * CHR;
    const int lc = panel_swz<C>(pc, row);
    const int m = m0 + row;
    const unsigned voff = m < M ? (unsigned)(((long long)m * C + lc * 8) * 2) : TB_OOB;
    bufdma16(src, panel + piece * 1024, voff, 0u);
  }
}

template <int C, int BM = 128>
AGD_DEV void panel_row_stats(const char* panel, float* lnst, int tid, float eps) {
  constexpr int CHR = C / 8, TPR = 512 / BM, PER = CHR / TPR;
  static_assert(CHR % TPR == 0, "chunks per row split over the row's threads");
  const int row = tid / TPR, part = tid % TPR;
  float S = 0.f, Q = 0.f;
#pragma unroll
  for (int cc = 0; cc < PER; ++cc) {
    const u32x4 v = *(const u32x4*)(panel + row * (C * 2) + panel_swz<C>(part * PER + cc, row) * 16);
#pragma unroll
    for (int e = 0; e < 4; ++e) {
      const float a = __uint_as_float(v[e] << 16), b = __uint_as_float(v[e] & 0xFFFF0000u);
      S += a + b; Q += a * a + b * b;
    }
  }
#pragma unroll
  for (int o = 1; o < TPR; o <<= 1) { S += __shfl_xor(S, o); Q += __shfl_xor(Q, o); }
  if (part == 0) {
    const float mu = S * (1.0f / C);
    float var = Q * (1.0f / C) - mu * mu; var = var < 0.f ? 0.f : var;
    *(f32x2_t*)(lnst + row * 2) = f32x2_t{mu, rsqrtf(var + eps)};
  }
}

typedef u32x4 __attribute__((aligned(8))) u32x4_a8;
template <int NI> AGD_DEV void load_row_chunk(const bf16_t* p, u32x2 (&r)[NI]) {
#pragma unroll
  for (int t = 0; t + 1 < NI; t += 2) { const u32x4 v = *(const u32x4_a8*)(p + 4 * t); r[t] = u32x2{v[0], v[1]}; r[t + 1] = u32x2{v[2], v[3]}; }
  if (NI & 1) r[NI - 1] = *(const u32x2*)(p + 4 * (NI - 1));
}
template <int NI> AGD_DEV void store_row_chunk(bf16_t* p, const u32x2 (&r)[NI]) {
#pragma unroll
  for (int t = 0; t + 1 < NI; t += 2) *(u32x4_a8*)(p + 4 * t) = u32x4{r[t][0], r[t][1], r[t + 1][0], r[t + 1][1]};
  if (NI & 1) *(u32x2*)(p + 4 * (NI - 1)) = r[NI - 1];
}

#define TB_F 10
#define TB_D 8
template <int C>
AGD_DEV void panel_gemm_head(u32x4 (&ring)[TB_F], const bf16_t* wf, unsigned wbase, unsigned lane16, unsigned wbytes = C * C * 2) {
  const auto wrs = __builtin_amdgcn_make_buffer_rsrc((void*)wf, 0, wbytes, 0x00020000);
#pragma unroll
  for (int f = 0; f < TB_D; ++f) ring[f % TB_F] = __builtin_bit_cast(u32x4, __builtin_amdgcn_raw_buffer_load_b128(wrs, lane16, wbase + (unsigned)f * 1024u, 0));
}
struct TbNoHook { AGD_DEV void operator()() const {} };
template <int C, bool ZERO = true, int MI = 4, class Late = TbNoHook>
AGD_DEV void panel_gemm_body(u32x4 (&ring)[TB_F], f32x4 (&acc)[MI][5], const bf16_t* wf, unsigned wbase, unsigned lane16, const char* xrow, const XOff<C>& xo,
                             unsigned wbytes = C * C * 2, Late&& late = Late()) {
  constexpr int NI = 5, KS = C / 32, NFR = KS * NI, PITCH = C * 2;
  const auto wrs = __builtin_amdgcn_make_buffer_rsrc((void*)wf, 0, wbytes, 0x00020000);
  if constexpr (ZERO) {
#pragma unroll
  for (int i = 0; i < MI; ++i)
#pragma unroll
    for (int j = 0; j < NI; ++j) acc[i][j] = f32x4{0.f, 0.f, 0.f, 0.f};
  }
  bf16x8 xf[MI];
#pragma unroll
  for (int f = 0; f < NFR; ++f) {
    if (f + TB_D < NFR) ring[(f + TB_D) % TB_F] = __builtin_bit_cast(u32x4, __builtin_amdgcn_raw_buffer_load_b128(wrs, lane16, wbase + (unsigned)(f + TB_D) * 1024u, 0));
    if (f == NFR - TB_D) late();
    __builtin_amdgcn_sched_barrier(0);
    if (f % NI == 0) {
      const int ks = f / NI;
#pragma unroll
      for (int i = 0; i < MI; ++i) xf[i] = *(const bf16x8*)(xrow + i * 16 * PITCH + xo.at(ks));
    }
#pragma unroll
    for (int i = 0; i < MI; ++i)
      acc[i][f % NI] = __builtin_amdgcn_mfma_f32_16x16x32_bf16(__builtin_bit_cast(bf16x8, ring[f % TB_F]), xf[i], acc[i][f % NI], 0, 0, 0);
  }
}

template <int C, int VAR = 0, int POST = 0>
__global__ __launch_bounds__(512, 2) void ff_fused_kernel(const FFusedP p) {
  constexpr int BM = 128, HID = 4 * C, HC = 128, NCH = HID / HC, KS1 = C / 32, KS2 = HC / 32, NI2 = C / 64;
  constexpr int PITCH = C * 2;
  static_assert(C % 64 == 0 && (C / 8) % 8 == 0 && KS1 % 2 == 0, "panel geometry");
  extern __shared__ __attribute__((aligned(16))) char smem[];
  char* panel = smem;
  char* hbuf = smem + BM * PITCH;
  float* lnst = (float*)(hbuf + 2 * BM * HC * 2);
  float* cbufs = lnst + BM * 2;

  const int tid = threadIdx.x, lane = tid & 63;
  const int wid = __builtin_amdgcn_readfirstlane(tid >> 6);
  const int mh = wid >> 2, nq = wid & 3;
  const int m0 = blockIdx.x * BM;
  TB_TS_DECL
  TB_TS(1);

  panel_load_dma<C>(p.h, m0, p.M, panel, wid, lane);
  asm volatile("s_waitcnt vmcnt(0)" ::: "memory");
  __syncthreads();
  panel_row_stats<C>(panel, lnst, tid, p.ln_eps);
  { const auto cs1r0 = __builtin_amdgcn_make_buffer_rsrc((void*)p.cs1, 0, (unsigned)(2 * HID * 4), 0x00020000);
    const auto b1r0 = __builtin_amdgcn_make_buffer_rsrc((void*)p.b1, 0, (unsigned)(2 * HID * 4), 0x00020000);
    const unsigned off = (unsigned)((((tid >> 7) & 1) ? HID : 0) + (tid & (HC - 1))) * 4u;
    ((float*)(hbuf + 2 * BM * HC * 2) + BM * 2)[tid] = __builtin_bit_cast(float, wid < 4 ? __builtin_amdgcn_raw_buffer_load_b32(cs1r0, off, 0, 0) : __builtin_amdgcn_raw_buffer_load_b32(b1r0, off, 0, 0)); }
  __syncthreads();

  f32x4 acc2[4][NI2];
#pragma unroll
  for (int i = 0; i < 4; ++i)
#pragma unroll
    for (int j = 0; j < NI2; ++j) acc2[i][j] = f32x4{0.f, 0.f, 0.f, 0.f};
  f32x4 acc1[4][4];

  const auto w1rs = __builtin_amdgcn_make_buffer_rsrc((void*)p.w1f, 0, (unsigned)(2 * HID * C * 2), 0x00020000);
  const auto w2rs = __builtin_amdgcn_make_buffer_rsrc((void*)p.w2f, 0, (unsigned)(HID * C * 2), 0x00020000);
#define ldw1(sbase, f) __builtin_bit_cast(u32x4, __builtin_amdgcn_raw_buffer_load_b128(w1rs, lane16, (sbase) + (unsigned)(f) * 1024u, 0))
#define ldw2(sbase, f) __builtin_bit_cast(u32x4, __builtin_amdgcn_raw_buffer_load_b128(w2rs, lane16, (sbase) + (unsigned)(f) * 1024u, 0))
  constexpr bool NOW = (VAR & 2) != 0, NOX = (VAR & 4) != 0;

  constexpr int F = TB_F, D = TB_D, DX = 2, N2 = KS2 * NI2, N1 = KS1 * 4;
  static_assert((N1 + N2) % F == 0 && D < F && D <= N2 && DX <= D, "ring geometry");
  u32x4 ring[F];

  auto lane_now = [&]() __attribute__((always_inline)) { int l = lane; asm volatile("" : "+v"(l)); return l; };
  auto gemm2 = [&](int c, bool pre, bool has_next, unsigned nexts) __attribute__((always_inline)) {
    const int l_ = lane_now(), q = l_ >> 4, px = l_ & 15;
    const unsigned lane16 = (unsigned)l_ * 16u;
    const char* hb = hbuf + (c & 1) * (BM * HC * 2) + (64 * mh + px) * (HC * 2);
    const unsigned wp = __builtin_amdgcn_readfirstlane((unsigned)(((c * 4 + nq) * KS2) * NI2) * 1024u);
    if (!pre && !NOW) {
#pragma unroll
      for (int f = 0; f < DX; ++f) ring[f % F] = ldw2(wp, f);
    }
    if constexpr (!NOW) {
#pragma unroll
      for (int f = DX; f < D; ++f) ring[f % F] = ldw2(wp, f);
    }
    bf16x8 hf[4];
#pragma unroll
    for (int f = 0; f < N2; ++f) {
      const int tgt = f + D;
      if constexpr (!NOW) {
        if (tgt < N2) ring[tgt % F] = ldw2(wp, tgt);
        else if (has_next) ring[tgt % F] = ldw1(nexts, tgt - N2);
      }
      __builtin_amdgcn_sched_barrier(0);
      if (f % NI2 == 0 && (!NOX || f == 0)) {
#pragma unroll
        for (int i = 0; i < 4; ++i) hf[i] = *(const bf16x8*)(hb + i * 16 * (HC * 2) + (((4 * (f / NI2) + q) ^ px) << 4));
      }
#pragma unroll
      for (int i = 0; i < 4; ++i)
        acc2[i][f % NI2] = __builtin_amdgcn_mfma_f32_16x16x32_bf16(__builtin_bit_cast(bf16x8, ring[f % F]), hf[i], acc2[i][f % NI2], 0, 0, 0);
    }
  };

  auto gemm1 = [&](int c, bool pre, bool has_next, unsigned nexts) __attribute__((always_inline)) {
#pragma unroll
    for (int i = 0; i < 4; ++i)
#pragma unroll
      for (int j = 0; j < 4; ++j) acc1[i][j] = f32x4{0.f, 0.f, 0.f, 0.f};
    const unsigned wp = __builtin_amdgcn_readfirstlane((unsigned)(((c * 4 + nq) * KS1) * 4) * 1024u);
    const int l_ = lane_now(), q = l_ >> 4, px = l_ & 15;
    const unsigned lane16 = (unsigned)l_ * 16u;
    const int sx = (px >> 1) & 7;
    const int xoff0 = ((q ^ sx) << 4), xoff1 = (((4 + q) ^ sx) << 4);
    const char* xrow = panel + (64 * mh + px) * PITCH;
    if (!pre && !NOW) {
#pragma unroll
      for (int f = 0; f < D; ++f) ring[(N2 + f) % F] = ldw1(wp, f);
    }
    bf16x8 xf[4];
#pragma unroll
    for (int f = 0; f < N1; ++f) {
      const int tgt = f + D;
      if constexpr (!NOW) {
        if (tgt < N1) ring[(N2 + tgt) % F] = ldw1(wp, tgt);
        else if (has_next && tgt - N1 < DX) ring[(N2 + tgt) % F] = ldw2(nexts, tgt - N1);
      }
      __builtin_amdgcn_sched_barrier(0);
      if (f % 4 == 0 && (!NOX || f == 0)) {
        const int ks = f / 4;
#pragma unroll
        for (int i = 0; i < 4; ++i) xf[i] = *(const bf16x8*)(xrow + i * 16 * PITCH + (ks >> 1) * 128 + ((ks & 1) ? xoff1 : xoff0));
      }
#pragma unroll
      for (int i = 0; i < 4; ++i)
        acc1[i][f % 4] = __builtin_amdgcn_mfma_f32_16x16x32_bf16(__builtin_bit_cast(bf16x8, ring[(N2 + f) % F]), xf[i], acc1[i][f % 4], 0, 0, 0);
    }
  };

  const auto cs1rs = __builtin_amdgcn_make_buffer_rsrc((void*)p.cs1, 0, (unsigned)(2 * HID * 4), 0x00020000);
  const auto b1rs = __builtin_amdgcn_make_buffer_rsrc((void*)p.b1, 0, (unsigned)(2 * HID * 4), 0x00020000);
  auto cload = [&](int c) __attribute__((always_inline)) {
    const unsigned off = (unsigned)((((tid >> 7) & 1) ? HID : 0) + HC * c + (tid & (HC - 1))) * 4u;
    return __builtin_bit_cast(float, wid < 4 ? __builtin_amdgcn_raw_buffer_load_b32(cs1rs, off, 0, 0) : __builtin_amdgcn_raw_buffer_load_b32(b1rs, off, 0, 0));
  };
  auto cstore = [&](int c, float v) __attribute__((always_inline)) { cbufs[(c % 3) * (4 * HC) + tid] = v; };
  static_assert(HC == 128, "one float per thread and chunk");
  auto geglu = [&](int c) __attribute__((always_inline)) {
    const int l_ = lane_now(), q = l_ >> 4, px = l_ & 15;
    const int rbase = 64 * mh + px;
    const float* cb = cbufs + (c % 3) * (4 * HC) + 32 * nq + 8 * q;
    char* hb = hbuf + (c & 1) * (BM * HC * 2);
    float mu[4], rs[4];
#pragma unroll
    for (int i = 0; i < 4; ++i) { const f32x2_t v = *(const f32x2_t*)(lnst + (rbase + 16 * i) * 2); mu[i] = v[0]; rs[i] = v[1]; }
#pragma unroll
    for (int t = 0; t < 2; ++t) {
      const f32x4 csv = *(const f32x4*)(cb + 4 * t), csg = *(const f32x4*)(cb + HC + 4 * t), bv = *(const f32x4*)(cb + 2 * HC + 4 * t), bg = *(const f32x4*)(cb + 3 * HC + 4 * t);
#pragma unroll
      for (int i = 0; i < 4; ++i) {
        float o[4];
#pragma unroll
        for (int r = 0; r < 4; ++r) {
          const float v = rs[i] * (acc1[i][t][r] - mu[i] * csv[r]) + bv[r];
          const float g = rs[i] * (acc1[i][2 + t][r] - mu[i] * csg[r]) + bg[r];
          o[r] = (VAR & 1) ? v + g : v * gelu_erf_f(g);
        }
        *(u32x2*)(hb + (rbase + 16 * i) * (HC * 2) + (((4 * nq + q) ^ px) << 4) + 8 * t) = u32x2{pack_bf2(o[0], o[1]), pack_bf2(o[2], o[3])};
      }
    }
  };

  bool pre2 = false;
  if constexpr (NOW) {
    const unsigned lane16 = (unsigned)lane * 16u;
#pragma unroll
    for (int f = 0; f < F; ++f) ring[f] = ldw1(0u, f);
  }
  auto interval = [&](int k) __attribute__((always_inline)) {
    const bool cn = k + 1 < NCH;
    float cv = 0.f;
    if (cn) cv = cload(k + 1);
    if (!(VAR & 8) && mh == 1 && k >= 1 && k <= NCH) geglu(k - 1);
    const int c2 = k - 1 - mh, c2n = k - mh;
    const bool v2 = c2 >= 0 && c2 < NCH, v1 = k < NCH, v2n = c2n >= 0 && c2n < NCH;
    const unsigned w1s = __builtin_amdgcn_readfirstlane((unsigned)(((k * 4 + nq) * KS1) * 4) * 1024u);
    const unsigned w2ns = __builtin_amdgcn_readfirstlane((unsigned)(((c2n * 4 + nq) * KS2) * NI2) * 1024u);
    if (v2) gemm2(c2, pre2, v1, w1s);
    if (v1) gemm1(k, v2, v2n, w2ns);
    pre2 = v1 && v2n;
    if (!(VAR & 8) && mh == 0 && k < NCH) geglu(k);
    if (cn) cstore(k + 1, cv);
    if (k <= NCH) __syncthreads();
  };
  static_assert(NCH >= 4, "steady intervals");
  TB_TS(2);
#pragma unroll 1
  for (int k = 0; k < 2; ++k) interval(k);
  TB_TS(3);
  if (mh == 0) {
    for (int k = 2; k < NCH; ++k) {
      const unsigned w1s = __builtin_amdgcn_readfirstlane((unsigned)(((k * 4 + nq) * KS1) * 4) * 1024u);
      const unsigned w2ns = __builtin_amdgcn_readfirstlane((unsigned)(((k * 4 + nq) * KS2) * NI2) * 1024u);
      const bool cn = k + 1 < NCH;
      float cv = 0.f;
      if (cn) cv = cload(k + 1);
      gemm2(k - 1, true, true, w1s);
      TB_TS(10);
      gemm1(k, true, true, w2ns);
      TB_TS(11);
      if (!(VAR & 8)) geglu(k);
      TB_TS(12);
      if (cn) cstore(k + 1, cv);
      __syncthreads();
      TB_TS(13);
    }
  } else {
    for (int k = 2; k < NCH; ++k) {
      const bool cn = k + 1 < NCH;
      float cv = 0.f;
      if (cn) cv = cload(k + 1);
      if (!(VAR & 8)) geglu(k - 1);
      TB_TS(12);
      const unsigned w1s = __builtin_amdgcn_readfirstlane((unsigned)(((k * 4 + nq) * KS1) * 4) * 1024u);
      const unsigned w2ns = __builtin_amdgcn_readfirstlane((unsigned)((((k - 1) * 4 + nq) * KS2) * NI2) * 1024u);
      gemm2(k - 2, true, true, w1s);
      TB_TS(10);
      gemm1(k, true, true, w2ns);
      TB_TS(11);
      if (cn) cstore(k + 1, cv);
      __syncthreads();
      TB_TS(13);
    }
  }
  TB_TS(4);
  pre2 = true;
#pragma unroll 1
  for (int k = NCH; k <= NCH + 1; ++k) interval(k);
  TB_TS(5);

  const int l_e = lane_now(), q = l_e >> 4, px = l_e & 15;
  const int rbase = 64 * mh + px;
  const unsigned lane16 = (unsigned)l_e * 16u;
  const char* xrow = panel + rbase * PITCH;
  const int ncol0 = (C / 4) * nq + 4 * NI2 * q;
  constexpr bool post = POST != 0;
  constexpr bool premul = POST == 2;
  static_assert(F == TB_F, "the proj_out stage reuses the weight ring");
  const unsigned pwbase = __builtin_amdgcn_readfirstlane((unsigned)(nq * KS1 * NI2) * 1024u);
  if (post) panel_gemm_head<C>(ring, p.wpf, pwbase, lane16);
  if constexpr (!premul) {
  float b2v[NI2 * 4];
#pragma unroll
  for (int t = 0; t < NI2; ++t) *(f32x4*)&b2v[4 * t] = *(const f32x4*)(p.b2 + ncol0 + 4 * t);
#pragma unroll
  for (int i = 0; i < 4; ++i) {
    const int row = rbase + 16 * i, m = m0 + row;
    if (!post && m >= p.M) continue;
    u32x2 pk[NI2];
#pragma unroll
    for (int t = 0; t < NI2; ++t) {
      const int n = ncol0 + 4 * t;
      char* pa = panel + row * PITCH + panel_swz<C>(n >> 3, row) * 16 + (n & 7) * 2;
      const u32x2 r = *(const u32x2*)pa;
      pk[t][0] = pack_bf2(acc2[i][t][0] + b2v[4 * t] + __uint_as_float(r[0] << 16), acc2[i][t][1] + b2v[4 * t + 1] + __uint_as_float(r[0] & 0xFFFF0000u));
      pk[t][1] = pack_bf2(acc2[i][t][2] + b2v[4 * t + 2] + __uint_as_float(r[1] << 16), acc2[i][t][3] + b2v[4 * t + 3] + __uint_as_float(r[1] & 0xFFFF0000u));
      if (post) *(u32x2*)pa = pk[t];
    }
    if (!post) store_row_chunk<NI2>(p.out + (long long)m * C + ncol0, pk);
  }
  }
  if constexpr (post) {
  if constexpr (!premul) __syncthreads();
  u32x2 xr[4][NI2];
  auto ld_xr = [&]() __attribute__((always_inline)) {
#pragma unroll
    for (int i = 0; i < 4; ++i) { const int m = m0 + rbase + 16 * i, ms = m < p.M ? (p.xres_rows > 0 ? m % p.xres_rows : m) : 0; load_row_chunk<NI2>(p.xres + (long long)ms * C + ncol0, xr[i]); }
  };
  ld_xr();
  panel_gemm_body<C, !premul>(ring, acc2, p.wpf, pwbase, lane16, xrow, XOff<C>(q, px));
  float bpv[NI2 * 4];
#pragma unroll
  for (int t = 0; t < NI2; ++t) *(f32x4*)&bpv[4 * t] = *(const f32x4*)(p.bp + ncol0 + 4 * t);
  float cs[NI2 * 4], cq[NI2 * 4];
#pragma unroll
  for (int e = 0; e < NI2 * 4; ++e) { cs[e] = 0.f; cq[e] = 0.f; }
#pragma unroll
  for (int i = 0; i < 4; ++i) {
    const int m = m0 + rbase + 16 * i;
    const bool live = m < p.M;
    const long long mo = (long long)(live ? m : 0) * C + ncol0;
    u32x2 pkk[NI2];
#pragma unroll
    for (int t = 0; t < NI2; ++t) {
      u32x2 pk;
      pk[0] = pack_bf2(acc2[i][t][0] + bpv[4 * t] + __uint_as_float(xr[i][t][0] << 16), acc2[i][t][1] + bpv[4 * t + 1] + __uint_as_float(xr[i][t][0] & 0xFFFF0000u));
      pk[1] = pack_bf2(acc2[i][t][2] + bpv[4 * t + 2] + __uint_as_float(xr[i][t][1] << 16), acc2[i][t][3] + bpv[4 * t + 3] + __uint_as_float(xr[i][t][1] & 0xFFFF0000u));
      pkk[t] = pk;
      if (live) {
        const float a0 = __uint_as_float(pk[0] << 16), a1 = __uint_as_float(pk[0] & 0xFFFF0000u), a2 = __uint_as_float(pk[1] << 16), a3 = __uint_as_float(pk[1] & 0xFFFF0000u);
        cs[4 * t] += a0; cs[4 * t + 1] += a1; cs[4 * t + 2] += a2; cs[4 * t + 3] += a3;
        cq[4 * t] += a0 * a0; cq[4 * t + 1] += a1 * a1; cq[4 * t + 2] += a2 * a2; cq[4 * t + 3] += a3 * a3;
      }
    }
    if (live) store_row_chunk<NI2>(p.pout + mo, pkk);
  }
  if (p.colstat) {
#pragma unroll
    for (int e = 0; e < NI2 * 4; ++e) {
#pragma unroll
      for (int o = 1; o < 16; o <<= 1) { cs[e] += __shfl_xor(cs[e], o); cq[e] += __shfl_xor(cq[e], o); }
    }
    float* stg = (float*)hbuf;
    if (px == 0) {
#pragma unroll
      for (int e = 0; e < NI2 * 4; ++e) { stg[(mh * C + ncol0 + e) * 2] = cs[e]; stg[(mh * C + ncol0 + e) * 2 + 1] = cq[e]; }
    }
    __syncthreads();
    if (tid < C) {
      float* op = p.colstat + ((long long)blockIdx.x * C + tid) * 2;
      op[0] = stg[tid * 2] + stg[(C + tid) * 2]; op[1] = stg[tid * 2 + 1] + stg[(C + tid) * 2 + 1];
    }
  }
  }
  TB_TS_END;
}

int launch_ff_fused(const FFusedP& p, int C, hipStream_t st) {
  if (C != 320) { agd_set_error("ff_fused: C = %d is not built (320 only)", C); return -1; }
  if (p.M < 1 || !p.h || !p.out || !p.w1f || !p.w2f || !p.cs1 || !p.b1 || !p.b2) { agd_set_error("ff_fused: bad arguments"); return -1; }
  if ((long long)p.M * C * 2 >= (1LL << 31)) { agd_set_error("ff_fused: activation too large for 32-bit offsets"); return -1; }
  constexpr int lds = 128 * 320 * 2 + 2 * 128 * 128 * 2 + 128 * 8 + 3 * 4 * 128 * 4;
  const void* kfn = p.wpf ? (p.premul ? (const void*)ff_fused_kernel<320, 0, 2> : (const void*)ff_fused_kernel<320, 0, 1>) : (const void*)ff_fused_kernel<320>;
  if (p.wpf && (!p.bp || !p.xres || !p.pout)) { agd_set_error("ff_fused: the proj_out stage needs bias, residual and output"); return -1; }
  if (p.premul && !p.wpf) { agd_set_error("ff_fused: the pre-multiplied form is the proj_out stage's"); return -1; }
#ifdef AGD_EXPERIMENTS
  static const void* const vars[16] = {(const void*)ff_fused_kernel<320, 0>, (const void*)ff_fused_kernel<320, 1>, (const void*)ff_fused_kernel<320, 2>, (const void*)ff_fused_kernel<320, 3>,
                                       (const void*)ff_fused_kernel<320, 4>, nullptr, (const void*)ff_fused_kernel<320, 6>, (const void*)ff_fused_kernel<320, 7>,
                                       (const void*)ff_fused_kernel<320, 8>, nullptr, (const void*)ff_fused_kernel<320, 10>, nullptr, nullptr, nullptr, (const void*)ff_fused_kernel<320, 14>, nullptr};
  if (!p.wpf && g_tb_variant > 0 && g_tb_variant < 16 && vars[g_tb_variant]) kfn = vars[g_tb_variant];
#endif
  int dev = 0; HIP_CHECK_RET(hipGetDevice(&dev));
  if (dev < 0 || dev >= AGD_MAX_DEVICES) { agd_set_error("ff_fused: device ordinal %d out of range", dev); return -1; }
  HIP_CHECK_RET(hipFuncSetAttribute(kfn, hipFuncAttributeMaxDynamicSharedMemorySize, lds));
  FFusedP pp = p;
  void* args[] = {&pp};
  HIP_CHECK_RET(hipLaunchKernel(kfn, dim3((p.M + 127) / 128), dim3(512), args, lds, st));
  return 0;
}

template <int C, int PRE, int MI = 4>
__global__ __launch_bounds__(512, 2) void attn_chain_kernel(const AttnChainP p) {
  TB_TS_DECL
  TB_TS(0);
  constexpr int NQ = C / 80, MH = 8 / NQ, BM = 16 * MI * MH, QBN = BM / 32;
  static_assert(MI == 4 || (MI == 2 && C == 640), "32-row panels: C = 640 only");
  constexpr int H = 8, D = C / H, KS = C / 32, NI = 5, PITCH = C * 2, CHR = C / 8;
  static_assert(C == 320 || C == 640, "8 heads of 40 / 80");
  constexpr int KB = 3, KEYS = 96, KSTEPS = (D + 15) / 16, DBLK = (D + 31) / 32, CH = D / 8;
  constexpr int KPITCH = ((2 * KSTEPS) | 1) * 16, VPITCH = (DBLK | 1) * 64;
  constexpr int KVSTAGE = KEYS * (KPITCH + VPITCH);
  constexpr int NCHUNK = KEYS * CH, LD_IT = (NCHUNK + 255) / 256;
  extern __shared__ __attribute__((aligned(16))) char smem[];
  char* panel = smem;
  char* kvs = smem + BM * PITCH;
  float* lnst = (float*)(kvs + 2 * KVSTAGE);
  float* pst = lnst + BM * 2;
  float* gbs = pst + NQ * BM * 2;

  const int tid = threadIdx.x, lane = tid & 63;
  const int wid = __builtin_amdgcn_readfirstlane(tid >> 6);
  const int mh = wid / NQ, nq = wid % NQ;
  const int q = lane >> 4, px = lane & 15;
  const int qb = wid & (QBN - 1), hhalf = wid >> 2;
  const bool attn_wave = QBN == 4 || (wid & 3) < QBN;
  const int c = lane & 31, hh = lane >> 5;
  const int m0 = blockIdx.x * BM;
  const int b = m0 / p.HW, pix0 = m0 - b * p.HW;
  const int m0s = p.src_rows > 0 ? m0 % p.src_rows : m0;
  TB_TS(1);
  const int gbi = tid < C / 2 ? tid : 0;
  const f32x4 gbv = *(const f32x4*)((gbi < C / 4 ? p.gamma : p.beta - C) + 4 * gbi);
  panel_load_dma<C, BM>(PRE ? p.o1 : p.h, m0s, p.src_rows > 0 ? p.src_rows : p.M, panel, wid, lane);
  TB_TS(40);

  char* sK = kvs + hhalf * KVSTAGE;
  char* sV = sK + KEYS * KPITCH;
  const int t4 = tid & 255;
  constexpr int KPADC = KPITCH / 16 - CH;
  for (int i = t4; i < KEYS * KPADC; i += 256) { const int r = i / KPADC, cc = CH + i % KPADC; *(u32x4*)(sK + r * KPITCH + cc * 16) = u32x4{0, 0, 0, 0}; }
  TB_TS(41);
  u32x4 kreg[LD_IT], vreg[LD_IT];
  unsigned kvoff[LD_IT];
#pragma unroll
  for (int it = 0; it < LD_IT; ++it) {
    const int idx = t4 + it * 256, r = idx / CH, cc = idx - r * CH;
    kvoff[it] = idx < NCHUNK ? (unsigned)((r * p.ldkv + cc * 8) * 2) : TB_OOB;
  }
  const unsigned kv_bytes = (unsigned)(((long long)(p.T - 1) * p.ldkv + D) * 2);
  const bf16_t* kvb = p.kv + (long long)b * p.skv;
  auto kv_load = [&](int h) {
    const auto krs = __builtin_amdgcn_make_buffer_rsrc((void*)(kvb + h * D), 0, kv_bytes, 0x00020000);
    const auto vrs = __builtin_amdgcn_make_buffer_rsrc((void*)(kvb + C + h * D), 0, kv_bytes, 0x00020000);
#pragma unroll
    for (int it = 0; it < LD_IT; ++it) {
      kreg[it] = __builtin_bit_cast(u32x4, __builtin_amdgcn_raw_buffer_load_b128(krs, kvoff[it], 0, 0));
      vreg[it] = __builtin_bit_cast(u32x4, __builtin_amdgcn_raw_buffer_load_b128(vrs, kvoff[it], 0, 0));
    }
  };
  auto kv_store = [&]() {
#pragma unroll
    for (int it = 0; it < LD_IT; ++it) {
      const int idx = t4 + it * 256, r = idx / CH, cc = idx - r * CH;
      if (idx < NCHUNK) { *(u32x4*)(sK + r * KPITCH + cc * 16) = kreg[it]; *(u32x4*)(sV + r * VPITCH + cc * 16) = vreg[it]; }
    }
  };
  kv_load(4 * hhalf);
  TB_TS(42);

  const int rbase = 16 * MI * mh + px;
  const XOff<C> xo(q, px);
  const char* xrow = panel + rbase * PITCH;
  f32x4 acc[MI][NI];
  u32x4 ring[TB_F];
  const unsigned lane16 = (unsigned)lane * 16u;
  const unsigned wbase = __builtin_amdgcn_readfirstlane((unsigned)(nq * KS * NI) * 1024u);
  auto gemm_head = [&](const bf16_t* wf) { panel_gemm_head<C>(ring, wf, wbase, lane16); };
  auto gemm_body = [&](const bf16_t* wf) { panel_gemm_body<C, true, MI>(ring, acc, wf, wbase, lane16, xrow, xo); };
  auto gemm_body_late = [&](const bf16_t* wf, auto&& late) __attribute__((always_inline)) { panel_gemm_body<C, true, MI>(ring, acc, wf, wbase, lane16, xrow, xo, (unsigned)(C * C * 2), late); };
  const int ncol0 = 16 * NI * nq + 4 * NI * q;

  if constexpr (PRE) gemm_head(p.wo1f);
  TB_TS(2);
  asm volatile("s_waitcnt vmcnt(0)" ::: "memory");
  if (tid < C / 2) *(f32x4*)(gbs + 4 * tid) = gbv;
  __syncthreads();
  TB_TS(3);
  kv_store();
  if constexpr (!PRE) {
    panel_row_stats<C, BM>(panel, lnst, tid, p.ln_eps);
    __syncthreads();
    gemm_head(p.wqf);
  }

  if constexpr (PRE) {
    u32x2 hr[MI][NI];
    auto ld_hr = [&]() __attribute__((always_inline)) {
#pragma unroll
      for (int i = 0; i < MI; ++i) load_row_chunk<NI>(p.h + (long long)(m0s + rbase + 16 * i) * C + ncol0, hr[i]);
    };
    gemm_body_late(p.wo1f, ld_hr);
    TB_TS(4);
    gemm_head(p.wqf);
    float bv1[NI * 4];
#pragma unroll
    for (int t = 0; t < NI; ++t) *(f32x4*)&bv1[4 * t] = *(const f32x4*)(p.bo1 + ncol0 + 4 * t);
    float rs1[MI], rq1[MI];
#pragma unroll
    for (int i = 0; i < MI; ++i) {
      const int m = m0 + rbase + 16 * i;
      bf16_t* op = p.out + (long long)m * C + ncol0;
      u32x2 pkk[NI];
      const u32x2 (&r)[NI] = hr[i];
      rs1[i] = 0.f; rq1[i] = 0.f;
#pragma unroll
      for (int t = 0; t < NI; ++t) {
        u32x2 pk;
        pk[0] = pack_bf2(acc[i][t][0] + bv1[4 * t] + __uint_as_float(r[t][0] << 16), acc[i][t][1] + bv1[4 * t + 1] + __uint_as_float(r[t][0] & 0xFFFF0000u));
        pk[1] = pack_bf2(acc[i][t][2] + bv1[4 * t + 2] + __uint_as_float(r[t][1] << 16), acc[i][t][3] + bv1[4 * t + 3] + __uint_as_float(r[t][1] & 0xFFFF0000u));
        pkk[t] = pk;
        acc[i][t] = f32x4{__uint_as_float(pk[0] << 16), __uint_as_float(pk[0] & 0xFFFF0000u), __uint_as_float(pk[1] << 16), __uint_as_float(pk[1] & 0xFFFF0000u)};
        rs1[i] += (acc[i][t][0] + acc[i][t][1]) + (acc[i][t][2] + acc[i][t][3]);
        rq1[i] += (acc[i][t][0] * acc[i][t][0] + acc[i][t][1] * acc[i][t][1]) + (acc[i][t][2] * acc[i][t][2] + acc[i][t][3] * acc[i][t][3]);
      }
      store_row_chunk<NI>(op, pkk);
      rs1[i] += __shfl_xor(rs1[i], 16); rs1[i] += __shfl_xor(rs1[i], 32);
      rq1[i] += __shfl_xor(rq1[i], 16); rq1[i] += __shfl_xor(rq1[i], 32);
      if (q == 0) *(f32x2_t*)(pst + (nq * BM + rbase + 16 * i) * 2) = f32x2_t{rs1[i], rq1[i]};
    }
    TB_TS(5);
    __syncthreads();
    float g2[NI * 4], b2[NI * 4];
#pragma unroll
    for (int t = 0; t < NI; ++t) { *(f32x4*)&g2[4 * t] = *(const f32x4*)(gbs + ncol0 + 4 * t); *(f32x4*)&b2[4 * t] = *(const f32x4*)(gbs + C + ncol0 + 4 * t); }
#pragma unroll
    for (int i = 0; i < MI; ++i) {
      const int row = rbase + 16 * i;
      float S = 0.f, Q = 0.f;
#pragma unroll
      for (int w = 0; w < NQ; ++w) { const f32x2_t v = *(const f32x2_t*)(pst + (w * BM + row) * 2); S += v[0]; Q += v[1]; }
      const float mu = S * (1.0f / C);
      float var = Q * (1.0f / C) - mu * mu; var = var < 0.f ? 0.f : var;
      const float rstd = rsqrtf(var + p.ln_eps);
#pragma unroll
      for (int t = 0; t < NI; ++t) {
        const int n = ncol0 + 4 * t;
        u32x2 pk;
        pk[0] = pack_bf2((acc[i][t][0] - mu) * rstd * g2[4 * t] + b2[4 * t], (acc[i][t][1] - mu) * rstd * g2[4 * t + 1] + b2[4 * t + 1]);
        pk[1] = pack_bf2((acc[i][t][2] - mu) * rstd * g2[4 * t + 2] + b2[4 * t + 2], (acc[i][t][3] - mu) * rstd * g2[4 * t + 3] + b2[4 * t + 3]);
        *(u32x2*)(panel + row * PITCH + panel_swz<C>(n >> 3, row) * 16 + (n & 7) * 2) = pk;
      }
    }
  } else {
#pragma unroll 2
  for (int i = 0; i < BM * CHR / 512; ++i) {
    const int pos = i * 512 + tid, row = pos / CHR, pc = pos - row * CHR, lc = panel_swz<C>(pc, row);
    u32x4 v = *(u32x4*)(panel + row * PITCH + pc * 16);
// ... 105 lines not shown
        for (int i = 0; i < 16; ++i) { const float pv = __builtin_amdgcn_exp2f(fmaf(sacc[kb][i], sc, -mx)); sacc[kb][i] = pv; rsum += pv; }
      const float inv = 1.0f / xhalf_sum(rsum);
      if (recb) {
#pragma unroll
        for (int kb = 0; kb < KB; ++kb)
#pragma unroll
          for (int i = 0; i < 16; ++i) pacc[kb][i] += sacc[kb][i] * inv;
      }
      f32x16 oacc[DBLK];
#pragma unroll
      for (int db = 0; db < DBLK; ++db)
#pragma unroll
        for (int j = 0; j < 16; ++j) oacc[db][j] = 0.f;
#pragma unroll
      for (int kb = 0; kb < KB; ++kb)
#pragma unroll
        for (int s = 0; s < 2; ++s) {
          bf16x8 pf;
#pragma unroll
          for (int j = 0; j < 8; ++j) pf[j] = (__bf16)sacc[kb][8 * s + j];
          const char* vb = sV + (kb * 32 + 16 * s + tr_row) * VPITCH + tr_col * 2;
#pragma unroll
          for (int db = 0; db < DBLK; ++db) {
            const s16x4 lo = __builtin_amdgcn_ds_read_tr16_b64_v4i16((__attribute__((address_space(3))) s16x4*)(vb + db * 64));
            const s16x4 hi2 = __builtin_amdgcn_ds_read_tr16_b64_v4i16((__attribute__((address_space(3))) s16x4*)(vb + 8 * VPITCH + db * 64));
            const u32x2 l2 = __builtin_bit_cast(u32x2, lo), h2 = __builtin_bit_cast(u32x2, hi2);
            const u32x4 a4 = u32x4{l2[0], l2[1], h2[0], h2[1]};
            oacc[db] = __builtin_amdgcn_mfma_f32_32x32x16_bf16(__builtin_bit_cast(bf16x8, a4), pf, oacc[db], 0, 0, 0);
          }
        }
#pragma unroll
      for (int db = 0; db < DBLK; ++db)
#pragma unroll
        for (int g = 0; g < 4; ++g) {
          const int d0 = db * 32 + 8 * g + 4 * hh;
          if (d0 < D) {
            u32x2 pk;
            pk[0] = pack_bf2(oacc[db][4 * g + 0] * inv, oacc[db][4 * g + 1] * inv);
            pk[1] = pack_bf2(oacc[db][4 * g + 2] * inv, oacc[db][4 * g + 3] * inv);
            *(u32x2*)(prow + panel_swz<C>(CH * h + (d0 >> 3), qr) * 16 + (d0 & 7) * 2) = pk;
          }
        }
      if (recb && hpb < H && ((hi + 1) % hpb) == 0) {
        rec_rmw(h / hpb, pacc);
#pragma unroll
        for (int kb = 0; kb < KB; ++kb)
#pragma unroll
          for (int j = 0; j < 16; ++j) pacc[kb][j] = 0.f;
      }
      }
      TB_TS(10 + hi);
      __syncthreads();
      if (hi + 1 < 4) { kv_store(); __syncthreads(); }
      TB_TS(20 + hi);
    }
    gemm_head(p.wof);
    if (p.record && hpb == H) {
      float* xch = (float*)kvs + (qb * 48) * 64 + lane;
      if (hhalf == 1 && recb && attn_wave) {
#pragma unroll
        for (int kb = 0; kb < KB; ++kb)
#pragma unroll
          for (int i = 0; i < 16; ++i) xch[(kb * 16 + i) * 64] = pacc[kb][i];
      }
      __syncthreads();
      if (hhalf == 0 && recb && attn_wave) {
#pragma unroll
        for (int kb = 0; kb < KB; ++kb)
#pragma unroll
          for (int i = 0; i < 16; ++i) pacc[kb][i] += xch[(kb * 16 + i) * 64];
        rec_rmw(0, pacc);
      }
    }
  }
  TB_TS(30);
  __syncthreads();
  TB_TS(31);

  u32x2 fr[MI][NI];
  auto ld_fr = [&]() __attribute__((always_inline)) {
#pragma unroll
    for (int i = 0; i < MI; ++i) load_row_chunk<NI>((PRE ? (const bf16_t*)p.out : p.h) + (long long)((PRE ? m0 : m0s) + rbase + 16 * i) * C + ncol0, fr[i]);
  };
  gemm_body_late(p.wof, ld_fr);
  TB_TS(32);
  float bv[NI * 4];
#pragma unroll
  for (int t = 0; t < NI; ++t) *(f32x4*)&bv[4 * t] = *(const f32x4*)(p.bo + ncol0 + 4 * t);
  float rs[MI], rq[MI];
  char* const ostg = kvs + 4096 + wid * 5120;
#pragma unroll
  for (int i = 0; i < MI; ++i) {
    rs[i] = 0.f; rq[i] = 0.f;
    u32x2 pkk[NI];
    const u32x2 (&r)[NI] = fr[i];
#pragma unroll
    for (int t = 0; t < NI; ++t) {
      const float v0 = acc[i][t][0] + bv[4 * t] + __uint_as_float(r[t][0] << 16), v1 = acc[i][t][1] + bv[4 * t + 1] + __uint_as_float(r[t][0] & 0xFFFF0000u);
      const float v2 = acc[i][t][2] + bv[4 * t + 2] + __uint_as_float(r[t][1] << 16), v3 = acc[i][t][3] + bv[4 * t + 3] + __uint_as_float(r[t][1] & 0xFFFF0000u);
      u32x2 pk; pk[0] = pack_bf2(v0, v1); pk[1] = pack_bf2(v2, v3);
      pkk[t] = pk;
      const float a0 = __uint_as_float(pk[0] << 16), a1 = __uint_as_float(pk[0] & 0xFFFF0000u), a2 = __uint_as_float(pk[1] << 16), a3 = __uint_as_float(pk[1] & 0xFFFF0000u);
      rs[i] += (a0 + a1) + (a2 + a3); rq[i] += (a0 * a0 + a1 * a1) + (a2 * a2 + a3 * a3);
    }
#pragma unroll
    for (int t = 0; t < NI; ++t) *(u32x2*)(ostg + (16 * (i & 1) + px) * 160 + 40 * q + 8 * t) = pkk[t];
    if (i & 1) {
#pragma unroll
      for (int it = 0; it < 5; ++it) {
        const int id = 64 * it + lane, row = id / 10, pc = id - row * 10;
        const u32x4 v = *(const u32x4*)(ostg + 16 * id);
        *(u32x4*)(p.out + (long long)(m0 + 16 * MI * mh + 16 * (i - 1) + row) * C + 80 * nq + 8 * pc) = v;
      }
    }
  }
  if (p.rowstat_out) {
#pragma unroll
    for (int i = 0; i < MI; ++i) {
      rs[i] += __shfl_xor(rs[i], 16); rs[i] += __shfl_xor(rs[i], 32);
      rq[i] += __shfl_xor(rq[i], 16); rq[i] += __shfl_xor(rq[i], 32);
    }
    float* stg = (float*)kvs;
    if (q == 0) {
#pragma unroll
      for (int i = 0; i < MI; ++i) { stg[(nq * BM + rbase + 16 * i) * 2] = rs[i]; stg[(nq * BM + rbase + 16 * i) * 2 + 1] = rq[i]; }
    }
    __syncthreads();
    if (tid < BM) {
      float S = 0.f, Q = 0.f;
#pragma unroll
      for (int w = 0; w < NQ; ++w) { S += stg[(w * BM + tid) * 2]; Q += stg[(w * BM + tid) * 2 + 1]; }
      *(f32x2_t*)(p.rowstat_out + (long long)(m0 + tid) * 2) = f32x2_t{S, Q};
    }
  }
  TB_TS_END;
}

int launch_attn_chain(const AttnChainP& p, int C, int heads, hipStream_t st) {
  if ((C != 320 && C != 640) || heads != 8) { agd_set_error("attn_chain: C = %d / heads = %d is not built (320 or 640 / 8 only)", C, heads); return -1; }
  const bool r32 = C == 640 && p.rows32 && p.M / 64 < 200 && p.HW % 32 == 0;
  const int BM = C == 320 ? 128 : r32 ? 32 : 64;
  if (p.M < BM || p.M % BM || p.HW % BM || p.M % p.HW) { agd_set_error("attn_chain: M %d / HW %d must be multiples of %d (whole images)", p.M, p.HW, BM); return -1; }
  if (p.T < 1 || p.T > 96) { agd_set_error("attn_chain: %d keys (1..96)", p.T); return -1; }
  if ((long long)p.M * C * 2 >= (1LL << 31)) { agd_set_error("attn_chain: activation too large for 32-bit offsets"); return -1; }
  if (p.record && (p.rec_hpb < 1 || 8 % p.rec_hpb || !p.rec)) { agd_set_error("attn_chain: recorder head group %d", p.rec_hpb); return -1; }
  const int D = C / 8, ks = (D + 15) / 16, db = (D + 31) / 32;
  const int lds = BM * C * 2 + 2 * 96 * ((((2 * ks) | 1) * 16) + ((db | 1) * 64)) + BM * 8 + (C / 80) * BM * 8 + 2 * C * 4;
  const bool pre = p.o1 != nullptr;
  if (pre && (!p.wo1f || !p.bo1 || p.out == p.h)) { agd_set_error("attn_chain: the to_out prologue needs its weights and out != h"); return -1; }
  if (p.src_rows > 0 && (p.src_rows % BM || p.M % p.src_rows || p.out == p.h)) { agd_set_error("attn_chain: src_rows %d must divide M, be a multiple of %d and out != h", p.src_rows, BM); return -1; }
  const void* kfn = C == 320 ? (pre ? (const void*)attn_chain_kernel<320, 1> : (const void*)attn_chain_kernel<320, 0>)
                    : r32    ? (pre ? (const void*)attn_chain_kernel<640, 1, 2> : (const void*)attn_chain_kernel<640, 0, 2>)
                             : (pre ? (const void*)attn_chain_kernel<640, 1> : (const void*)attn_chain_kernel<640, 0>);
  static std::atomic<bool> attr[AGD_MAX_DEVICES][6] = {};
  int dev = 0; HIP_CHECK_RET(hipGetDevice(&dev));
  if (dev < 0 || dev >= AGD_MAX_DEVICES) { agd_set_error("attn_chain: device ordinal %d out of range", dev); return -1; }
  const int slot = (C == 640 ? (r32 ? 4 : 2) : 0) + (pre ? 1 : 0);
  if (!attr[dev][slot]) { HIP_CHECK_RET(hipFuncSetAttribute(kfn, hipFuncAttributeMaxDynamicSharedMemorySize, lds)); attr[dev][slot] = true; }
  AttnChainP pp = p;
  void* args[] = {&pp};
  HIP_CHECK_RET(hipLaunchKernel(kfn, dim3(p.M / BM), dim3(512), args, lds, st));
  return 0;
}

template <int C, int MH = 8 / (C / 80)>
__global__ __launch_bounds__(64 * MH * (C / 80), 2) void qkv_chain_kernel(const QkvChainP p) {
  constexpr int NQ = C / 80, BM = 64 * MH, KS = C / 32, NI = 5, PITCH = C * 2, NT = 64 * MH * NQ;
  extern __shared__ __attribute__((aligned(16))) char smem[];
  char* panel = smem;
  float* pst = (float*)(smem + BM * PITCH);
  const int tid = threadIdx.x, lane = tid & 63;
  const int wid = __builtin_amdgcn_readfirstlane(tid >> 6);
  const int mh = wid / NQ, nq = wid % NQ;
  const int q = lane >> 4, px = lane & 15;
  const int m0 = blockIdx.x * BM;
  const int img = m0 / p.HW;
  TB_TS_DECL
  TB_TS(1);

  panel_load_dma<C, BM, MH * NQ>(p.x, m0, p.M, panel, wid, lane);
  const int rbase = 64 * mh + px;
  const char* xrow = panel + rbase * PITCH;
  f32x4 acc[4][NI];
  u32x4 ring[TB_F];
  const unsigned lane16 = (unsigned)lane * 16u;
  const int ncol0 = 80 * nq + 4 * NI * q;
  const unsigned wbase = __builtin_amdgcn_readfirstlane((unsigned)(nq * KS * NI) * 1024u);
  const bf16_t* wimg = p.wbf + (long long)img * p.wb_stride;
  panel_gemm_head<C>(ring, wimg, wbase, lane16);
  TB_TS(2);
  if (p.gn_part) {
    double* csum = (double*)(smem + BM * PITCH + NQ * BM * 8);
    float* gst = (float*)(csum + 2 * C);
    float* ab = gst + 64;
    const int nt = p.HW / p.gn_bm, cpg = C / p.gn_groups;
    constexpr int CPT = (C + NT - 1) / NT;
    float gam[CPT], bet[CPT];
#pragma unroll
    for (int r = 0; r < CPT; ++r) {
      const int cch = tid + NT * r < C ? tid + NT * r : C - 1;
      gam[r] = p.gn_gamma[cch]; bet[r] = p.gn_beta[cch];
      const float* pp = p.gn_part + ((long long)img * nt * C + cch) * 2;
      double a = 0.0, qq = 0.0;
      for (int t0 = 0; t0 < nt; t0 += 16) {
        f32x2_t v[16];
#pragma unroll
        for (int u = 0; u < 16; ++u) { const int tc = t0 + u < nt ? t0 + u : nt - 1; v[u] = *(const f32x2_t*)(pp + (long long)tc * C * 2); }
#pragma unroll
        for (int u = 0; u < 16; ++u) if (t0 + u < nt) { a += (double)v[u][0]; qq += (double)v[u][1]; }
      }
      if (tid + NT * r < C) { csum[2 * (tid + NT * r)] = a; csum[2 * (tid + NT * r) + 1] = qq; }
    }
    __syncthreads();
    if (tid < p.gn_groups) {
      double a = 0.0, qq = 0.0;
      for (int e = 0; e < cpg; ++e) { a += csum[2 * (tid * cpg + e)]; qq += csum[2 * (tid * cpg + e) + 1]; }
      const double cnt = (double)p.HW * cpg, mean = a / cnt;
      double var = qq / cnt - mean * mean; if (var < 0) var = 0;
      gst[2 * tid] = (float)mean; gst[2 * tid + 1] = (float)(1.0 / sqrt(var + (double)p.gn_eps));
    }
    __syncthreads();
#pragma unroll
    for (int r = 0; r < CPT; ++r) {
      const int cch = tid + NT * r;
      if (cch < C) { const int g = cch / cpg; const float sc = gst[2 * g + 1] * gam[r]; ab[2 * cch] = sc; ab[2 * cch + 1] = bet[r] - gst[2 * g] * sc; }
    }
  }
  TB_TS(3);
  asm volatile("s_waitcnt vmcnt(0)" ::: "memory");
  __syncthreads();
  TB_TS(4);
  if (p.gn_part) {
    const float* ab = (const float*)(smem + BM * PITCH + NQ * BM * 8 + 2 * C * 8) + 64;
    constexpr int CHR = C / 8;
#pragma unroll
    for (int k = 0; k < BM * CHR / NT; ++k) {
      const int id = tid + NT * k, row = id / CHR, pc = id - row * CHR;
      const int c0 = panel_swz<C>(pc, row) * 8;
      u32x4* cp = (u32x4*)(panel + row * PITCH + pc * 16);
      const u32x4 v = *cp;
      u32x4 o;
#pragma unroll
      for (int e = 0; e < 4; ++e) {
        const f32x4 sab = *(const f32x4*)(ab + 2 * (c0 + 2 * e));
        o[e] = pack_bf2(fmaf(__uint_as_float(v[e] << 16), sab[0], sab[1]), fmaf(__uint_as_float(v[e] & 0xFFFF0000u), sab[2], sab[3]));
      }
      *cp = o;
// ... 326 lines not shown
```

### agenda_amd/ops.py

```python
from __future__ import annotations

import ctypes

import torch

from . import _lib


def _f32c(t):
    assert t.is_cuda, "ops run on the GPU only (no CPU fallback)"
    return t.detach().to(torch.float32).contiguous()


_P8 = {0: 0, 1: 2, 2: 4, 3: 8}


def conv2d(x, w, bias=None, stride=1, padding=None, upsample=False, halo=False, p8=0, smap=False, phases=False, pc=0, xcd_block=False):
    lib = _lib.load()
    x, w = _f32c(x), _f32c(w)
    b = _f32c(bias) if bias is not None else None
    B, Cin, H, W = x.shape
    Cout, _, k, _ = w.shape
    pad = (1 if k == 3 else 0) if padding is None else padding
    up = 2 if upsample else 1
# ... 32 lines not shown
    if x1 is not None:
        x1 = _f32c(x1)
        assert x1.shape[0] == B and x1.shape[2:] == x.shape[2:], "x1 must share x's batch and map"
        C1 = x1.shape[1]
    if part is None and part1 is None and x1 is None and not return_path:
        y = torch.empty_like(x)
        _lib.check(lib.agd_op_groupnorm(_lib.ptr(x), _lib.ptr(_f32c(gamma)), _lib.ptr(_f32c(beta)), _lib.ptr(y), B, C0, HW,
                                        groups, float(eps), int(silu), _lib.current_stream_ptr()), None, "agd_op_groupnorm")
        return y
    for t, b_, cs in ((part, bm, C0), (part1, bm1, C1)):
        if t is not None:
            assert b_ and b_ > 0 and t.dtype == torch.float32 and t.numel() == B * (HW // b_) * cs * 2, "partial-sum table [B, HW // bm, Cs, 2] fp32"
    part = _f32c(part) if part is not None else None
    part1 = _f32c(part1) if part1 is not None else None
    y = torch.empty(B, C0 + C1, *x.shape[2:], device=x.device, dtype=torch.float32)
    path = ctypes.c_int(0)
    _lib.check(lib.agd_op_groupnorm_ex(_lib.ptr(x), _lib.ptr(x1), _lib.ptr(_f32c(gamma)), _lib.ptr(_f32c(beta)), _lib.ptr(y), B, C0, C1, HW,
                                       groups, float(eps), int(silu), _lib.ptr(part), int(bm or 0), _lib.ptr(part1), int(bm1 or 0),
                                       ctypes.byref(path), _lib.current_stream_ptr()), None, "agd_op_groupnorm_ex")
    return (y, path.value) if return_path else y


def gn_fold(part, bm, groups, gamma, beta, w, bias=None, eps=1e-6, x=None, frag_ni=0, hw=None):
    lib = _lib.load()
    part, w = _f32c(part), _f32c(w)
    B, nt, Cc = part.shape[:3]
    HW = nt * bm if hw is None else hw
    N = w.shape[0]
    assert w.shape[1] == Cc and part.shape[3] == 2
    b = _f32c(bias) if bias is not None else None
    dev = part.device
    out = {"wb": torch.empty(B, N, Cc, device=dev), "rowadd": torch.empty(B, N, device=dev)}
    if frag_ni > 0:
        out["wb_frag"] = torch.empty(B, N * Cc, device=dev)
        out["wb_frag_ref"] = torch.empty(B, N * Cc, device=dev)
    if x is not None:
        x = _f32c(x)
        assert x.shape[0] == B and x.shape[1] == Cc and x[0, 0].numel() == HW
        out["y"] = torch.empty(B, HW, N, device=dev)
    _lib.check(lib.agd_op_gn_fold(_lib.ptr(x), _lib.ptr(part), int(bm), B, Cc, HW, groups, float(eps), _lib.ptr(_f32c(gamma)), _lib.ptr(_f32c(beta)),
                                  _lib.ptr(w), _lib.ptr(b), N, int(frag_ni), _lib.ptr(out["wb"]), _lib.ptr(out["rowadd"]), _lib.ptr(out.get("wb_frag")),
                                  _lib.ptr(out.get("wb_frag_ref")), _lib.ptr(out.get("y")), _lib.current_stream_ptr()), None, "agd_op_gn_fold")
    return out


def layer_norm(x, gamma, beta, eps=1e-5, return_path=False):
    lib = _lib.load()
    x = _f32c(x)
    Cc = x.shape[-1]
    rows = x.numel() // Cc
    y = torch.empty_like(x)
    if return_path:
        inst = ctypes.c_int(0)
        _lib.check(lib.agd_op_layernorm_ex(_lib.ptr(x), _lib.ptr(_f32c(gamma)), _lib.ptr(_f32c(beta)), _lib.ptr(y), rows, Cc,
                                           float(eps), ctypes.byref(inst), _lib.current_stream_ptr()), None, "agd_op_layernorm_ex")
        return y, divmod(inst.value, 100)
    _lib.check(lib.agd_op_layernorm(_lib.ptr(x), _lib.ptr(_f32c(gamma)), _lib.ptr(_f32c(beta)), _lib.ptr(y), rows, Cc,
                                    float(eps), _lib.current_stream_ptr()), None, "agd_op_layernorm")
    return y


def ff_fused(x, gamma, beta, w1, b1, w2, b2, eps=1e-5):
    lib = _lib.load()
    Cc = x.shape[-1]
    x2 = _f32c(x).reshape(-1, Cc)
    y = torch.empty_like(x2)
    _lib.check(lib.agd_op_ff_fused(_lib.ptr(x2), _lib.ptr(_f32c(gamma)), _lib.ptr(_f32c(beta)), _lib.ptr(_f32c(w1)), _lib.ptr(_f32c(b1)),
                                   _lib.ptr(_f32c(w2)), _lib.ptr(_f32c(b2)), _lib.ptr(y), x2.shape[0], Cc, float(eps),
                                   _lib.current_stream_ptr()), None, "agd_op_ff_fused")
    return y.reshape(x.shape)


def attn_chain(x, gamma, beta, wq, kv, wo, bo, heads=8, eps=1e-5, return_probs=False, rows32=False):
    lib = _lib.load()
    x, kv = _f32c(x), _f32c(kv)
    B, HW, Cc = x.shape
    T = kv.shape[1]
    y = torch.empty_like(x)
    pr = torch.empty(B, T, HW, device=x.device, dtype=torch.float32) if return_probs else None
    _lib.check(lib.agd_op_attn_chain(_lib.ptr(x), _lib.ptr(_f32c(gamma)), _lib.ptr(_f32c(beta)), _lib.ptr(_f32c(wq)), _lib.ptr(kv), _lib.ptr(_f32c(wo)),
                                     _lib.ptr(_f32c(bo)), _lib.ptr(y), _lib.ptr(pr), B, HW, T, Cc, heads | (256 if rows32 else 0), float(eps), _lib.current_stream_ptr()),
               None, "agd_op_attn_chain")
    return (y, pr) if return_probs else y


def xattn_premul(x, gamma, beta, wq, kv, wo, bo, heads=8, eps=1e-5, return_probs=False):
    lib = _lib.load()
    x, kv = _f32c(x), _f32c(kv)
    B, HW, Cc = x.shape
    T = kv.shape[1]
    y = torch.empty_like(x)
    pr = torch.empty(B, heads, T, HW, device=x.device, dtype=torch.float32) if return_probs else None
    _lib.check(lib.agd_op_xattn_premul(_lib.ptr(x), _lib.ptr(_f32c(gamma)), _lib.ptr(_f32c(beta)), _lib.ptr(_f32c(wq)), _lib.ptr(kv), _lib.ptr(_f32c(wo)),
                                       _lib.ptr(_f32c(bo)), _lib.ptr(y), _lib.ptr(pr), B, HW, T, Cc, heads, float(eps), _lib.current_stream_ptr()),
               None, "agd_op_xattn_premul")
    return (y, pr) if return_probs else y


def _given(t):
    t = _f32c(t)
    return t if t.numel() else torch.zeros(1, device=t.device, dtype=torch.float32)


def attention(q, k, v, heads, scale=None, return_probs=False, *, causal=False, mask=None, k2=None, v2=None, layout=0, head_sum=False,
              rec_b0=0, rec_T=None):
    lib = _lib.load()
    q, k, v = _f32c(q), _f32c(k), _f32c(v)
    B, Nq, Cc = q.shape
    Nk = k.shape[1]
    D = Cc // heads
    scale = D ** -0.5 if scale is None else scale
    o = torch.empty_like(q)
    if causal or mask is not None or k2 is not None or v2 is not None or layout != 0 or head_sum or rec_b0 != 0 or rec_T is not None:
        if k.shape != (B, Nk, Cc) or v.shape != k.shape:
            raise ValueError(f"attention: k {tuple(k.shape)} / v {tuple(v.shape)} must both be [B, Nk, H*D] = [{B}, Nk, {Cc}]")
        if mask is not None and tuple(mask.shape) != (B, Nk):
            raise ValueError(f"attention: mask {tuple(mask.shape)} must be {(B, Nk)}")
        if (k2 is None) != (v2 is None) or (k2 is not None and (k2.shape != v2.shape or k2.ndim != 3 or k2.shape[0] != B or k2.shape[2] != Cc)):
            raise ValueError("attention: k2 and v2 come together, both [B, Nk2, H*D]")
        if head_sum and not return_probs:
            raise ValueError("attention: head_sum is a form of return_probs")
        Nk2 = 0 if k2 is None else k2.shape[1]
        probs = None
        if return_probs:
            probs = torch.empty((B, max(Nk, 1), max(Nq, 1)) if head_sum else (B, heads, max(Nk, 1), max(Nq, 1)), device=q.device, dtype=torch.float32)
        _lib.check(lib.agd_op_attention_ex(_lib.ptr(_given(q)), _lib.ptr(_given(k)), _lib.ptr(_given(v)), _lib.ptr(_given(o)), B, heads, D, Nq, Nk, float(scale),
                                           int(bool(causal)), _lib.ptr(None if mask is None else _given(mask)),
                                           _lib.ptr(None if k2 is None else _given(k2)), _lib.ptr(None if v2 is None else _given(v2)), Nk2, int(layout),
                                           _lib.ptr(probs), (2 if head_sum else 1) if return_probs else 0, int(rec_b0),
                                           Nk if rec_T is None else int(rec_T), _lib.current_stream_ptr()), None, "agd_op_attention_ex")
        return (o, probs) if return_probs else o
    probs = torch.empty(B, heads, Nk, Nq, device=q.device, dtype=torch.float32) if return_probs else None
    _lib.check(lib.agd_op_attention(_lib.ptr(q), _lib.ptr(k), _lib.ptr(v), _lib.ptr(o), B, heads, D, Nq, Nk, float(scale),
                                    _lib.ptr(probs), _lib.current_stream_ptr()), None, "agd_op_attention")
    return (o, probs) if return_probs else o


def attention_long(q, k, v, heads, scale=None, *, layout=0, rec_b0=0, rec_T=None, probs=None):
    lib = _lib.load()
    q, k, v = _f32c(q), _f32c(k), _f32c(v)
    B, Nq, Cc = q.shape
    Nk = k.shape[1]
    if k.shape != (B, Nk, Cc) or v.shape != k.shape:
        raise ValueError(f"attention_long: k {tuple(k.shape)} / v {tuple(v.shape)} must both be [B, Nk, H*D] = [{B}, Nk, {Cc}]")
    D = Cc // heads
    scale = D ** -0.5 if scale is None else scale
    o = torch.empty_like(q)
    if probs is None:
        probs = torch.zeros(B, heads, max(Nk, 1), max(Nq, 1), device=q.device, dtype=torch.float32)
    elif tuple(probs.shape) != (B, heads, Nk, Nq) or probs.dtype != torch.float32 or not probs.is_contiguous() or not probs.is_cuda:
        raise ValueError(f"attention_long: probs must be a contiguous fp32 GPU tensor {(B, heads, Nk, Nq)}")
    _lib.check(lib.agd_op_attention_long(_lib.ptr(_given(q)), _lib.ptr(_given(k)), _lib.ptr(_given(v)), _lib.ptr(_given(o)), B, heads, D, Nq, Nk,
                                         float(scale), int(layout), _lib.ptr(probs), int(rec_b0), Nk if rec_T is None else int(rec_T),
                                         _lib.current_stream_ptr()), None, "agd_op_attention_long")
    return o, probs


def attention_headsum(q, k, v, heads, scale=None):
    lib = _lib.load()
    q, k, v = _f32c(q), _f32c(k), _f32c(v)
    B, Nq, Cc = q.shape
    Nk = k.shape[1]
    D = Cc // heads
    scale = D ** -0.5 if scale is None else scale
    o = torch.empty_like(q)
    probs = torch.empty(B, Nk, Nq, device=q.device, dtype=torch.float32)
# ... 172 lines not shown
```

### include/agenda_hip.h

```cpp
#ifndef AGENDA_HIP_H
#define AGENDA_HIP_H
#ifdef __cplusplus
extern "C" {
#endif

typedef struct agd_ctx agd_ctx;

#define AGD_MAX_LEVELS 8

typedef struct agd_config {
  int struct_size;
  int in_channels, out_channels, n_levels;
  int block_out_channels[AGD_MAX_LEVELS];
  int down_cross[AGD_MAX_LEVELS];
  int num_heads[AGD_MAX_LEVELS];
  int layers_per_block, cross_attention_dim, use_linear_projection, norm_num_groups;
  int vae_latent_channels, vae_out_channels, vae_n_levels;
  int vae_block_out_channels[AGD_MAX_LEVELS];
  int vae_layers_per_block, vae_norm_num_groups;
  float vae_scaling_factor;
  int max_tokens;
  int prediction_type;
  long long workspace_bytes;
  int text_hidden, text_layers, text_heads, text_intermediate, text_vocab, text_max_pos;
// ... 91 lines not shown
typedef struct agd_gligen_config {
  int struct_size;
  int max_objs;
  int positive_len;
  int fourier_freqs;
} agd_gligen_config;
int agd_gligen_configure(agd_ctx* ctx, const agd_gligen_config* gcfg);
int agd_gligen_set(agd_ctx* ctx, const float* boxes, const float* pos_emb, const float* masks, int batch2, void* stream);
int agd_gligen_set_schedule(agd_ctx* ctx, const int* flags, int n);
int agd_gligen_clear(agd_ctx* ctx);
int agd_gligen_objs(agd_ctx* ctx, float* out);
int agd_gligen_fuser(agd_ctx* ctx, const char* block_name, const float* x, int batch2, int h, int w, float* out, void* stream);

int agd_unet_forward(agd_ctx* ctx, const float* sample, int batch2, int latent_side, float timestep, float* out,
                     void* stream);
int agd_unet_forward_hw(agd_ctx* ctx, const float* sample, int batch2, int latent_h, int latent_w, float timestep, float* out, void* stream);
int agd_unet_forward_ts(agd_ctx* ctx, const float* sample, int batch2, int latent_side, const float* timesteps, float* out, void* stream);
int agd_unet_forward_ts_hw(agd_ctx* ctx, const float* sample, int batch2, int latent_h, int latent_w, const float* timesteps, float* out,
                           void* stream);

int agd_cfg_ddim_step(agd_ctx* ctx, const float* eps, float* latents, int batch, int latent_side, float guidance,
                      float alpha_t, float alpha_prev, void* stream);
int agd_cfg_ddim_step_hw(agd_ctx* ctx, const float* eps, float* latents, int batch, int latent_h, int latent_w, float guidance,
                         float alpha_t, float alpha_prev, void* stream);

int agd_denoise(agd_ctx* ctx, float* latents, int batch, int latent_side, int n_steps, const float* timesteps,
                const float* alpha_t, const float* alpha_prev, float guidance, void* stream);
int agd_denoise_hw(agd_ctx* ctx, float* latents, int batch, int latent_h, int latent_w, int n_steps, const float* timesteps,
                   const float* alpha_t, const float* alpha_prev, float guidance, void* stream);

int agd_denoise_plms(agd_ctx* ctx, float* latents, int batch, int latent_side, int n_evals, const float* timesteps,
                     const float* sample_coeff, const float* eps_coeff, float guidance, void* stream);
int agd_denoise_plms_hw(agd_ctx* ctx, float* latents, int batch, int latent_h, int latent_w, int n_evals, const float* timesteps,
                        const float* sample_coeff, const float* eps_coeff, float guidance, void* stream);

int agd_denoise_dpm(agd_ctx* ctx, float* latents, int batch, int latent_side, int n_evals, const float* timesteps,
                    const float* coeffs, float guidance, void* stream);
int agd_denoise_dpm_hw(agd_ctx* ctx, float* latents, int batch, int latent_h, int latent_w, int n_evals, const float* timesteps,
                       const float* coeffs, float guidance, void* stream);

int agd_vae_decode(agd_ctx* ctx, const float* latents, int batch, int latent_side, unsigned char* out_u8,
                   float* out_f32, void* stream);
int agd_vae_decode_hw(agd_ctx* ctx, const float* latents, int batch, int latent_h, int latent_w, unsigned char* out_u8,
                      float* out_f32, void* stream);

int agd_vae_encode(agd_ctx* ctx, const float* image, int batch, int side, float* mean_out, float* logvar_out, void* stream);
int agd_vae_encode_hw(agd_ctx* ctx, const float* image, int batch, int h, int w, float* mean_out, float* logvar_out, void* stream);

int agd_set_option(agd_ctx* ctx, const char* name, int value);

int agd_record_config(agd_ctx* ctx, int mode, int is_train, int rec_tokens);
int agd_record_reset(agd_ctx* ctx, int batch, int latent_side, void* stream);
int agd_record_reset_hw(agd_ctx* ctx, int batch, int latent_h, int latent_w, void* stream);
int agd_daam_global(agd_ctx* ctx, int img, int rows, float* out, void* stream);
int agd_hook_global(agd_ctx* ctx, float* out, void* stream);
int agd_hook_count(agd_ctx* ctx);
int agd_hook_last_map(agd_ctx* ctx, float* out, int n_query, void* stream);

int agd_attn_processor(agd_ctx* ctx, const char* layer, const float* hidden, const float* ctx_emb, const float* attn_mask,
                       int batch2, int n_query, int tokens, float* out, int record, void* stream);
int agd_cross_attn(agd_ctx* ctx, const char* layer, const float* hidden, const float* ctx_emb, int batch2,
                   int n_query, int tokens, float* out, int record, void* stream);

int agd_hook_reset(agd_ctx* ctx, int rows, int latent_side, void* stream);
int agd_hook_num_maps(agd_ctx* ctx);
int agd_hook_map_dims(agd_ctx* ctx, int k, int* dims3);
int agd_hook_map(agd_ctx* ctx, int k, float* out, void* stream);
int agd_op_attn_reg_loss(const float* map, int B, int T, int P, const int* obj_idx, const int* fg_idx, const int* bg_idx, float coef,
                         float* loss_out, float* dmap, void* stream);
int agd_attn_processor_backward(agd_ctx* ctx, const char* layer, const float* hidden, const float* ctx_emb, const float* d_out,
                                const float* d_map, int is_train, int batch2, int n_query, int tokens, float* d_hidden, float* d_ctx,
                                void* stream);

int agd_op_conv2d(const float* x_nchw, const float* w, const float* bias, float* y_nchw, int B, int Cin, int H, int W,
                  int Cout, int ksize, int stride, int pad, int upsample, void* stream);
int agd_op_conv2d_ex(const float* x, const float* w, const float* bias, float* y, int B, int Cin, int H, int W, int Cout,
                     int ksize, int stride, int pad, int upsample, int flags, void* stream);
int agd_op_linear(const float* x, const float* w, const float* bias, const float* residual, float* y, int M, int K,
                  int N, int geglu, void* stream);
int agd_op_ff_fused(const float* x, const float* gamma, const float* beta, const float* w1, const float* b1, const float* w2,
                    const float* b2, float* y, int M, int C, float eps, void* stream);
int agd_op_attn_chain(const float* x, const float* gamma, const float* beta, const float* wq, const float* kv, const float* wo,
                      const float* bo, float* y, float* probs_sum, int B, int HW, int T, int C, int heads, float eps, void* stream);
int agd_op_xattn_premul(const float* x, const float* gamma, const float* beta, const float* wq, const float* kv, const float* wo,
                        const float* bo, float* y, float* probs, int B, int HW, int T, int C, int heads, float eps, void* stream);
int agd_op_groupnorm(const float* x_nchw, const float* gamma, const float* beta, float* y_nchw, int B, int C, int HW,
                     int groups, float eps, int silu, void* stream);
int agd_op_groupnorm_ex(const float* x0_nchw, const float* x1_nchw, const float* gamma, const float* beta, float* y_nchw, int B, int C0,
                        int C1, int HW, int groups, float eps, int silu, const float* part0, int bm0, const float* part1, int bm1,
                        int* path, void* stream);
int agd_op_gn_fold(const float* x_nchw, const float* part, int bm, int B, int C, int HW, int groups, float eps, const float* gamma,
                   const float* beta, const float* w, const float* bias, int N, int frag_ni, float* wb, float* rowadd, float* wb_frag,
                   float* wb_frag_ref, float* y, void* stream);
int agd_op_conv_groupnorm(const float* x_nchw, const float* w, const float* bias, const float* gamma, const float* beta, float* y_nchw,
                          int B, int Cin, int H, int W, int Cout, int groups, float eps, int silu, int fused, void* stream);
int agd_op_layernorm(const float* x, const float* gamma, const float* beta, float* y, int rows, int C, float eps,
                     void* stream);
int agd_op_layernorm_ex(const float* x, const float* gamma, const float* beta, float* y, int rows, int C, float eps, int* inst,
                        void* stream);
int agd_op_attention(const float* q, const float* k, const float* v, float* o, int B, int H, int D, int Nq, int Nk,
                     float scale, float* probs_out, void* stream);
int agd_op_attention_ex(const float* q, const float* k, const float* v, float* o, int B, int H, int D, int Nq, int Nk, float scale,
                        int causal, const float* mask, const float* k2, const float* v2, int Nk2, int layout, float* probs_out,
                        int record, int rec_b0, int rec_T, void* stream);
int agd_op_attention_long(const float* q, const float* k, const float* v, float* o, int B, int H, int D, int Nq, int Nk, float scale,
                          int layout, float* probs_inout, int rec_b0, int rec_T, void* stream);
int agd_op_attention_headsum(const float* q, const float* k, const float* v, float* o, int B, int H, int D, int Nq, int Nk,
                             float scale, float* probs_sum_out, void* stream);
int agd_op_attention_backward(const float* q, const float* kv, const float* d_o, const float* d_map, int b0, int B, int H, int D,
                              int N, int T, float scale, float* dq, float* dkv, void* stream);
int agd_op_hook_headmean(const float* heads, int Bp, int H, int T, int N, float* map, void* stream);
int agd_op_bicubic_clamp_mean(const float* maps, int n_maps, int T, int side, int S, float* out, void* stream);

int agd_op_heatmap_u8(const float* hm, int n, int npix, unsigned char* out, void* stream);
int agd_op_resize_u8_pil(const unsigned char* in, int n, int H, int W, int C, int oh, int ow, unsigned char* out, void* stream);
int agd_op_stack_heatmaps(const unsigned char* obj, const unsigned char* fg, const unsigned char* bg, long long npix,
                          unsigned char* rgb, unsigned char* inv, void* stream);

int agd_lora_add(agd_ctx* ctx, const char* target_key, const float* down, const float* up, int rank, float alpha);
int agd_lora_set_scale(agd_ctx* ctx, float s, void* stream);
int agd_lora_clear(agd_ctx* ctx);
int agd_lora_count(agd_ctx* ctx);
float agd_lora_scale(agd_ctx* ctx);

int agd_op_window_gather(const float* canvas, float* views, int B, int C, int Lh, int Lw, int window, int stride, int v0, int n, void* stream);
int agd_op_window_mean(const float* views, float* canvas, int B, int C, int Lh, int Lw, int window, int stride, void* stream);
int agd_denoise_panorama(agd_ctx* ctx, float* canvas, int batch, int Lh, int Lw, int window, int stride, int view_batch, int n_steps,
                         const float* timesteps, const float* alpha_t, const float* alpha_prev, float guidance, void* stream);
int agd_daam_global_panorama(agd_ctx* ctx, int img, int rows, float* out, void* stream);

int agd_freeu_set(agd_ctx* ctx, float s1, float s2, float b1, float b2);
int agd_freeu_clear(agd_ctx* ctx);
int agd_freeu_counts(agd_ctx* ctx, long long* counts);
int agd_op_freeu(const float* hidden_nchw, const float* skip_nchw, float* hidden_out, float* skip_out, int B, int Ch, int Cs, int H, int W,
                 float b, float s, void* stream);

int agd_guidance_rescale_set(agd_ctx* ctx, float phi);
int agd_guidance_rescale_clear(agd_ctx* ctx);
int agd_guidance_rescale_counts(agd_ctx* ctx, long long* launches);
int agd_op_guidance_rescale(agd_ctx* ctx, const float* eps, int ldc, int B, int C, int HW, float guidance, float phi, float* factor, void* stream);

int agd_pag_set(agd_ctx* ctx, const float* scales, int n, const char* const* layers, int n_layers);
int agd_pag_clear(agd_ctx* ctx);
int agd_pag_counts(agd_ctx* ctx, long long* walks, long long* layers);
int agd_op_pag_v_rows(agd_ctx* ctx, const void* qkv, void* att, int M, int C, void* stream);
int agd_op_pag_fold(agd_ctx* ctx, float* eps, long long n, float p, void* stream);

int agd_deepcache_set(agd_ctx* ctx, const int* full_flags, int n, int branch);
int agd_deepcache_clear(agd_ctx* ctx);
int agd_deepcache_counts(agd_ctx* ctx, long long* out);
int agd_deepcache_forward_hw(agd_ctx* ctx, const float* sample, int rows, int Lh, int Lw, float timestep, int branch, int shallow, float* out, void* stream);
int agd_op_deepcache_capture(agd_ctx* ctx, const void* src0, void* dst0, long long bytes0, const void* src1, void* dst1, long long bytes1, void* stream);

#define AGD_N_CLASSES 11
int agd_profile_begin(agd_ctx* ctx);
int agd_profile_end(agd_ctx* ctx, double* ms, double* flops, long long* launches);
int agd_profile_end_ex(agd_ctx* ctx, double mfma_peak_flops, double hbm_peak_bytes, double* ms, double* flops, double* bytes,
                       double* roof_ms, double* roof_ms_hbm_bound, long long* launches);
const char* agd_profile_class_name(int cls);

#ifdef AGD_EXPERIMENTS
int agd_bench_conv(int B, int H, int W, int C0, int C1, int Cout, int ksize, int stride, int up, int geglu, int with_residual,
                   int iters, double* ms_out);
int agd_bench_attention(int B, int H, int D, int Nq, int Nk, int record, int iters, double* ms_out);
int agd_bench_conv_cold(int B, int H, int W, int C0, int Cout, int ksize, int geglu, int with_residual, int warm, int iters, double* ms_out);
int agd_bench_groupnorm(int B, int HW, int C, int iters, double* ms_out);
// ... 10 lines not shown
```

Before: 9.333.

## Fuse cross-attention chain and feed-forward into one kernel for C=320 blocks

Adds a merged kernel for the C=320 transformer blocks. It runs the attn2 chain and then the fused feed-forward in the same workgroup, keeping the attention output panel in LDS instead of writing it to global memory and reloading it. The to_out GEMM's weight ring also prefetches the first FF weight fragments, so the next stage's loads overlap the current one. The aim is to remove one launch and one activation round-trip per block. In exchange, LDS is sized for the larger of the two phases, the combined kernel is larger, and occupancy may suffer.

```diff
diff --git a/agenda_amd/_lib.py b/agenda_amd/_lib.py
--- a/agenda_amd/_lib.py
+++ b/agenda_amd/_lib.py
@@ -176,6 +176,7 @@
     "agd_op_layernorm_ex": (C.c_int, [_P, _P, _P, _P, C.c_int, C.c_int, C.c_float, C.POINTER(C.c_int), _P]),
     "agd_op_ff_fused": (C.c_int, [_P] * 8 + [C.c_int, C.c_int, C.c_float, _P]),
     "agd_op_attn_chain": (C.c_int, [_P] * 9 + [C.c_int] * 5 + [C.c_float, _P]),
+    "agd_op_attn_chain_ff": (C.c_int, [_P] * 22 + [C.c_int] * 4 + [C.c_float, C.c_int, _P]),
     "agd_op_xattn_premul": (C.c_int, [_P] * 9 + [C.c_int] * 5 + [C.c_float, _P]),
     "agd_op_attention": (C.c_int, [_P, _P, _P, _P, C.c_int, C.c_int, C.c_int, C.c_int, C.c_int, C.c_float, _P, _P]),
     "agd_op_attention_ex": (C.c_int, [_P, _P, _P, _P] + [C.c_int] * 5 + [C.c_float, C.c_int, _P, _P, _P, C.c_int, C.c_int, _P, C.c_int, C.c_int, C.c_int, _P]),
diff --git a/agenda_amd/csrc/kernels.h b/agenda_amd/csrc/kernels.h
--- a/agenda_amd/csrc/kernels.h
+++ b/agenda_amd/csrc/kernels.h
@@ -94,6 +94,7 @@
   int src_rows;
 };
 int launch_attn_chain(const AttnChainP& p, int C, int heads, hipStream_t st);
+int launch_attn_chain_ff(const AttnChainP& ap, const FFusedP& fp, int heads, hipStream_t st);
 struct QkvChainP {
   const bf16_t* x;
   const bf16_t* wbf; long long wb_stride; const float* rowadd;
diff --git a/agenda_amd/csrc/model.hip b/agenda_amd/csrc/model.hip
--- a/agenda_amd/csrc/model.hip
+++ b/agenda_amd/csrc/model.hip
@@ -93,6 +93,7 @@
   TBF_ATTN2_ROWS32  = 1 << 10,
   TBF_QKV_ROWS64    = 1 << 11,
   TBF_QKV_SCHED2    = 1 << 12,
+  TBF_TAIL          = 1 << 13,
   TBF_DEFAULT       = 0x1fff & ~TBF_QKV_640,
 };
 
@@ -599,6 +600,7 @@
   const IpaLayer* ipa;
   XLayer* xl;
   TbAttn2 attn2; int chain_rows32;
+  bool tail;
   bool daam;
   TbFf ff;
   bool wreg_proj;
@@ -618,6 +620,7 @@
   int M; const int Mshared;
   float* stats = nullptr; int slots = 0;
   bf16_t* ipaP = nullptr;
+  AttnChainP tail_ap{}; double tail_flops = 0, tail_bytes = 0;
   TBlock(agd_ctx* c_, hipStream_t st_, const std::string& pre_, const Act& x_, Act& out_, int heads_, int groups_, int dup)
     : c(c_), st(st_), pre(pre_), t(pre_ + "transformer_blocks.0."), x(x_), out(out_), heads(heads_), groups(groups_), C(x_.C), HW(x_.H * x_.W),
       Bs(x_.B), B(dup ? 2 * x_.B : x_.B), xres(x_.p), M(x_.B * x_.H * x_.W), Mshared(M) {}
@@ -690,6 +693,7 @@
   p.dup = !dup ? DUP_NONE : lazy ? DUP_LAZY : DUP_COPY;
   p.attn1_in_chain = chain && tb(TBF_ATTN1_OUT) && p.dup != DUP_COPY && has(t + "attn1.to_out.frag") && !p.fuser && !p.ipa;
   p.stats_head = p.fold; p.stats_attn1 = p.fold && !chain; p.stats_attn2 = p.fold && !ff_fused && !p.ipa; p.stats_ipa = p.fold && !ff_fused && p.ipa;
+  p.tail = tb(TBF_TAIL) && chain && C == 320 && ff_fused && !p.ipa;
   return p;
 }
 
@@ -838,7 +842,14 @@
     ap.rowstat_out = s.stats;
   }
   const double gemms = p.attn1_in_chain ? 6.0 : 4.0;
-  ProfScope ps(c, s.st, PC_ATTN_CROSS, gemms * M * (double)C * C + 4.0 * B * heads * (double)HW * T * D, gemms * M * (double)C + gemms * C * (double)C + 4.0 * B * (double)T * C + rec_bytes);
+  const double flops = gemms * M * (double)C * C + 4.0 * B * heads * (double)HW * T * D, bytes = gemms * M * (double)C + gemms * C * (double)C + 4.0 * B * (double)T * C + rec_bytes;
+  if (p.tail) {
+    if (ap.rowstat_out) FAIL("attn2 chain + feed-forward in one launch: nobody reads norm3's row statistics");
+    s.tail_ap = ap; s.tail_flops = flops; s.tail_bytes = bytes - 2.0 * M * (double)C;
+    s.h = ap.out;
+    return 0;
+  }
+  ProfScope ps(c, s.st, PC_ATTN_CROSS, flops, bytes);
   CK(launch_attn_chain(ap, C, heads, s.st));
   s.h = ap.out;
   return 0;
@@ -896,7 +907,12 @@
     out.cpart_bm = 0;
     if (out.cpart && c->opt_gn_fused && s.HW % 128 == 0) { fp.colstat = out.cpart; out.cpart_bm = 128; }
   }
-  ProfScope ps(c, s.st, PC_GEMM, 2.0 * M * (double)C * (proj ? 13.0 : 12.0) * C, (proj ? 8.0 : 4.0) * M * (double)C + 2.0 * (proj ? 13.0 : 12.0) * C * (double)C);
+  const double flops = 2.0 * M * (double)C * (proj ? 13.0 : 12.0) * C, bytes = (proj ? 8.0 : 4.0) * M * (double)C + 2.0 * (proj ? 13.0 : 12.0) * C * (double)C;
+  if (p.tail) {
+    ProfScope ps(c, s.st, PC_ATTN_CROSS, s.tail_flops + flops, s.tail_bytes + bytes - 2.0 * M * (double)C);
+    return launch_attn_chain_ff(s.tail_ap, fp, s.heads, s.st);
+  }
+  ProfScope ps(c, s.st, PC_GEMM, flops, bytes);
   return launch_ff_fused(fp, C, s.st);
 }
 
@@ -3081,6 +3097,56 @@
   return 0;
 }
 
+AGD_API int agd_op_attn_chain_ff(const float* x, const float* g2, const float* be2, const float* wq, const float* kv, const float* wo, const float* bo,
+                                 const float* o1, const float* wo1, const float* bo1,
+                                 const float* g3, const float* be3, const float* w1, const float* b1, const float* w2, const float* b2,
+                                 const float* wp, const float* bp, const float* xres, float* y, float* colstat, float* probs_sum,
+                                 int B, int HW, int T, int heads, float eps, int flags, void* stream) {
+  hipStream_t st = S(stream); Tmp tmp;
+  const int C = 320, H8 = 8 * C, H4 = 4 * C;
+  const bool fuse = flags & 1, premul = (flags & 2) != 0, shared = (flags & 4) != 0, rec_half = (flags & 8) != 0;
+  if (B < 1 || HW < 1 || T < 1) { agd_set_error("op_attn_chain_ff: B %d HW %d T %d", B, HW, T); return -1; }
+  if ((shared && (B % 2 || !o1)) || (rec_half && B % 2) || (premul && !wp) || (colstat && !wp) || (wp && (!bp || !xres)) || (o1 && (!wo1 || !bo1))) { agd_set_error("op_attn_chain_ff: inconsistent arguments"); return -1; }
+  const long long M = (long long)B * HW, Min = shared ? M / 2 : M;
+  bf16_t* xb = tmp.get<bf16_t>((size_t)Min * C); bf16_t* hb = tmp.get<bf16_t>((size_t)M * C); bf16_t* yb = tmp.get<bf16_t>((size_t)M * C); bf16_t* kvb = tmp.get<bf16_t>((size_t)B * T * 2 * C);
+  bf16_t* o1b = o1 ? tmp.get<bf16_t>((size_t)Min * C) : nullptr; bf16_t* xrb = wp ? tmp.get<bf16_t>((size_t)Min * C) : nullptr;
+  bf16_t* sq = tmp.get<bf16_t>((size_t)C * C); bf16_t* wqf = tmp.get<bf16_t>((size_t)C * C); bf16_t* wof = tmp.get<bf16_t>((size_t)C * C);
+  bf16_t* wo1f = o1 ? tmp.get<bf16_t>((size_t)C * C) : nullptr; bf16_t* wpf = wp ? tmp.get<bf16_t>((size_t)C * C) : nullptr;
+  bf16_t* w1b = tmp.get<bf16_t>((size_t)H8 * C); bf16_t* w1l = tmp.get<bf16_t>((size_t)H8 * C); bf16_t* w1f = tmp.get<bf16_t>((size_t)H8 * C);
+  bf16_t* w2b = tmp.get<bf16_t>((size_t)C * H4); bf16_t* w2f = tmp.get<bf16_t>((size_t)C * H4);
+  float* cs = tmp.get<float>(H8); float* bf = tmp.get<float>(H8);
+  if (!xb || !hb || !yb || !kvb || (o1 && (!o1b || !wo1f)) || (wp && (!xrb || !wpf)) || !sq || !wqf || !wof || !w1b || !w1l || !w1f || !w2b || !w2f || !cs || !bf) return -1;
+  CK(launch_f32_to_bf16(x, xb, Min * C, st));
+  CK(launch_f32_to_bf16(kv, kvb, (long long)B * T * 2 * C, st));
+  if (o1) CK(launch_f32_to_bf16(o1, o1b, Min * C, st));
+  if (wp) CK(launch_f32_to_bf16(xres, xrb, Min * C, st));
+  CK(launch_convert_weight(wq, sq, C, C, 1, C, 0, st)); CK(launch_frag_order_w(sq, wqf, C, C, 5, C, st));
+  CK(launch_convert_weight(wo, sq, C, C, 1, C, 0, st)); CK(launch_frag_order_w(sq, wof, C, C, 5, C, st));
+  if (o1) { CK(launch_convert_weight(wo1, sq, C, C, 1, C, 0, st)); CK(launch_frag_order_w(sq, wo1f, C, C, 5, C, st)); }
+  if (wp) { CK(launch_convert_weight(wp, sq, C, C, 1, C, 0, st)); CK(launch_frag_order_w(sq, wpf, C, C, 5, C, st)); }
+  CK(launch_convert_weight(w1, w1b, H8, C, 1, C, 16, st));
+  CK(launch_ln_fold_weight(w1b, g3, be3, b1, H8, C, 16, w1l, cs, bf, st));
+  CK(launch_frag_order_w1(w1l, w1f, C, H4, st));
+  CK(launch_convert_weight(w2, w2b, C, H4, 1, H4, 0, st));
+  CK(launch_frag_order_w(w2b, w2f, C, H4, C / 64, 128, st));
+  AttnChainP ap{}; ap.h = xb; ap.out = (o1 || shared) ? hb : xb; ap.gamma = g2; ap.beta = be2; ap.ln_eps = eps; ap.wqf = wqf; ap.wof = wof; ap.bo = bo;
+  ap.kv = kvb; ap.ldkv = 2 * C; ap.skv = (long long)T * 2 * C; ap.M = (int)M; ap.HW = HW; ap.T = T; ap.scale = 1.0f / sqrtf((float)(C / heads));
+  if (o1) { ap.o1 = o1b; ap.wo1f = wo1f; ap.bo1 = bo1; }
+  if (shared) ap.src_rows = (int)Min;
+  if (probs_sum) {
+    const int b0 = rec_half ? B / 2 : 0;
+    if (hipMemsetAsync(probs_sum, 0, (size_t)(B - b0) * T * HW * 4, st) != hipSuccess) { agd_set_error("memset probs"); return -1; }
+    ap.record = 1; ap.rec = probs_sum; ap.rec_b0 = b0; ap.rec_T = T; ap.rec_hpb = heads; ap.rec_head_stride = (long long)T * HW; ap.rec_img_stride = (long long)T * HW;
+  }
+  FFusedP fp{}; fp.h = ap.out; fp.out = yb; fp.w1f = w1f; fp.cs1 = cs; fp.b1 = bf; fp.w2f = w2f; fp.b2 = b2; fp.M = (int)M; fp.ln_eps = eps;
+  if (wp) { fp.wpf = wpf; fp.bp = bp; fp.xres = xrb; fp.pout = yb; fp.premul = premul ? 1 : 0; fp.colstat = colstat; if (shared) fp.xres_rows = (int)Min; }
+  if (fuse) CK(launch_attn_chain_ff(ap, fp, heads, st));
+  else { CK(launch_attn_chain(ap, C, heads, st)); CK(launch_ff_fused(fp, C, st)); }
+  CK(launch_bf16_to_f32(yb, y, M * C, st));
+  hipStreamSynchronize(st);
+  return 0;
+}
+
 AGD_API int agd_op_xattn_premul(const float* x, const float* gamma, const float* beta, const float* wq, const float* kv, const float* wo,
                                 const float* bo, float* y, float* probs, int B, int HW, int T, int C, int heads, float eps, void* stream) {
   hipStream_t st = S(stream); Tmp tmp;
diff --git a/agenda_amd/csrc/tblock.hip b/agenda_amd/csrc/tblock.hip
--- a/agenda_amd/csrc/tblock.hip
+++ b/agenda_amd/csrc/tblock.hip
@@ -139,11 +139,13 @@
   for (int f = 0; f < TB_D; ++f) ring[f % TB_F] = __builtin_bit_cast(u32x4, __builtin_amdgcn_raw_buffer_load_b128(wrs, lane16, wbase + (unsigned)f * 1024u, 0));
 }
 struct TbNoHook { AGD_DEV void operator()() const {} };
-template <int C, bool ZERO = true, int MI = 4, class Late = TbNoHook>
+template <int C, bool ZERO = true, int MI = 4, class Late = TbNoHook, bool NEXT = false>
 AGD_DEV void panel_gemm_body(u32x4 (&ring)[TB_F], f32x4 (&acc)[MI][5], const bf16_t* wf, unsigned wbase, unsigned lane16, const char* xrow, const XOff<C>& xo,
-                             unsigned wbytes = C * C * 2, Late&& late = Late()) {
+                             unsigned wbytes = C * C * 2, Late&& late = Late(), const bf16_t* nextw = nullptr, unsigned nextbytes = 0, unsigned nextbase = 0) {
   constexpr int NI = 5, KS = C / 32, NFR = KS * NI, PITCH = C * 2;
+  static_assert(!NEXT || NFR % TB_F == 0, "the next stage's fragments land in the slots its own ring indexing expects");
   const auto wrs = __builtin_amdgcn_make_buffer_rsrc((void*)wf, 0, wbytes, 0x00020000);
+  const auto nrs = __builtin_amdgcn_make_buffer_rsrc((void*)(NEXT ? nextw : wf), 0, NEXT ? nextbytes : wbytes, 0x00020000);
   if constexpr (ZERO) {
 #pragma unroll
   for (int i = 0; i < MI; ++i)
@@ -153,8 +155,9 @@
   bf16x8 xf[MI];
 #pragma unroll
   for (int f = 0; f < NFR; ++f) {
+    if (f == NFR - TB_D) late();
     if (f + TB_D < NFR) ring[(f + TB_D) % TB_F] = __builtin_bit_cast(u32x4, __builtin_amdgcn_raw_buffer_load_b128(wrs, lane16, wbase + (unsigned)(f + TB_D) * 1024u, 0));
-    if (f == NFR - TB_D) late();
+    else if constexpr (NEXT) ring[(f + TB_D) % TB_F] = __builtin_bit_cast(u32x4, __builtin_amdgcn_raw_buffer_load_b128(nrs, lane16, nextbase + (unsigned)(f + TB_D - NFR) * 1024u, 0));
     __builtin_amdgcn_sched_barrier(0);
     if (f % NI == 0) {
       const int ks = f / NI;
@@ -167,12 +170,19 @@
   }
 }
 
-template <int C, int VAR = 0, int POST = 0>
-__global__ __launch_bounds__(512, 2) void ff_fused_kernel(const FFusedP p) {
+template <int C> AGD_DEV float ff_chunk0_const(const FFusedP& p, int tid, int wid) {
+  constexpr int HID = 4 * C, HC = 128;
+  const auto cs1r0 = __builtin_amdgcn_make_buffer_rsrc((void*)p.cs1, 0, (unsigned)(2 * HID * 4), 0x00020000);
+  const auto b1r0 = __builtin_amdgcn_make_buffer_rsrc((void*)p.b1, 0, (unsigned)(2 * HID * 4), 0x00020000);
+  const unsigned off = (unsigned)((((tid >> 7) & 1) ? HID : 0) + (tid & (HC - 1))) * 4u;
+  return __builtin_bit_cast(float, wid < 4 ? __builtin_amdgcn_raw_buffer_load_b32(cs1r0, off, 0, 0) : __builtin_amdgcn_raw_buffer_load_b32(b1r0, off, 0, 0));
+}
+template <int C, int VAR, int POST, bool RES, bool HEAD = false>
+AGD_DEV void ff_fused_body(const FFusedP& p, char* smem, u32x4 (&ring)[TB_F], float c0 = 0.f) {
   constexpr int BM = 128, HID = 4 * C, HC = 128, NCH = HID / HC, KS1 = C / 32, KS2 = HC / 32, NI2 = C / 64;
   constexpr int PITCH = C * 2;
   static_assert(C % 64 == 0 && (C / 8) % 8 == 0 && KS1 % 2 == 0, "panel geometry");
-  extern __shared__ __attribute__((aligned(16))) char smem[];
+  static_assert(!HEAD || RES, "a stream head in flight belongs to the merged kernel");
   char* panel = smem;
   char* hbuf = smem + BM * PITCH;
   float* lnst = (float*)(hbuf + 2 * BM * HC * 2);
@@ -185,14 +195,14 @@
   TB_TS_DECL
   TB_TS(1);
 
-  panel_load_dma<C>(p.h, m0, p.M, panel, wid, lane);
-  asm volatile("s_waitcnt vmcnt(0)" ::: "memory");
-  __syncthreads();
+  if constexpr (!RES) {
+    panel_load_dma<C>(p.h, m0, p.M, panel, wid, lane);
+    asm volatile("s_waitcnt vmcnt(0)" ::: "memory");
+    __syncthreads();
+  }
   panel_row_stats<C>(panel, lnst, tid, p.ln_eps);
-  { const auto cs1r0 = __builtin_amdgcn_make_buffer_rsrc((void*)p.cs1, 0, (unsigned)(2 * HID * 4), 0x00020000);
-    const auto b1r0 = __builtin_amdgcn_make_buffer_rsrc((void*)p.b1, 0, (unsigned)(2 * HID * 4), 0x00020000);
-    const unsigned off = (unsigned)((((tid >> 7) & 1) ? HID : 0) + (tid & (HC - 1))) * 4u;
-    ((float*)(hbuf + 2 * BM * HC * 2) + BM * 2)[tid] = __builtin_bit_cast(float, wid < 4 ? __builtin_amdgcn_raw_buffer_load_b32(cs1r0, off, 0, 0) : __builtin_amdgcn_raw_buffer_load_b32(b1r0, off, 0, 0)); }
+  if constexpr (HEAD) ((float*)(hbuf + 2 * BM * HC * 2) + BM * 2)[tid] = c0;
+  else ((float*)(hbuf + 2 * BM * HC * 2) + BM * 2)[tid] = ff_chunk0_const<C>(p, tid, wid);
   __syncthreads();
 
   f32x4 acc2[4][NI2];
@@ -210,7 +220,6 @@
 
   constexpr int F = TB_F, D = TB_D, DX = 2, N2 = KS2 * NI2, N1 = KS1 * 4;
   static_assert((N1 + N2) % F == 0 && D < F && D <= N2 && DX <= D, "ring geometry");
-  u32x4 ring[F];
 
   auto lane_now = [&]() __attribute__((always_inline)) { int l = lane; asm volatile("" : "+v"(l)); return l; };
   auto gemm2 = [&](int c, bool pre, bool has_next, unsigned nexts) __attribute__((always_inline)) {
@@ -329,7 +338,7 @@
     const unsigned w1s = __builtin_amdgcn_readfirstlane((unsigned)(((k * 4 + nq) * KS1) * 4) * 1024u);
     const unsigned w2ns = __builtin_amdgcn_readfirstlane((unsigned)(((c2n * 4 + nq) * KS2) * NI2) * 1024u);
     if (v2) gemm2(c2, pre2, v1, w1s);
-    if (v1) gemm1(k, v2, v2n, w2ns);
+    if (v1) gemm1(k, v2 || (HEAD && k == 0), v2n, w2ns);
     pre2 = v1 && v2n;
     if (!(VAR & 8) && mh == 0 && k < NCH) geglu(k);
     if (cn) cstore(k + 1, cv);
@@ -467,6 +476,12 @@
   }
   TB_TS_END;
 }
+template <int C, int VAR = 0, int POST = 0>
+__global__ __launch_bounds__(512, 2) void ff_fused_kernel(const FFusedP p) {
+  extern __shared__ __attribute__((aligned(16))) char smem[];
+  u32x4 ring[TB_F];
+  ff_fused_body<C, VAR, POST, false>(p, smem, ring);
+}
 
 int launch_ff_fused(const FFusedP& p, int C, hipStream_t st) {
   if (C != 320) { agd_set_error("ff_fused: C = %d is not built (320 only)", C); return -1; }
@@ -491,8 +506,8 @@
   return 0;
 }
 
-template <int C, int PRE, int MI = 4>
-__global__ __launch_bounds__(512, 2) void attn_chain_kernel(const AttnChainP p) {
+template <int C, int PRE, int MI, int KEEP>
+AGD_DEV void attn_chain_body(const AttnChainP& p, char* smem, u32x4 (&ring)[TB_F], const bf16_t* nextw = nullptr, unsigned nextbytes = 0, unsigned nextbase = 0) {
   TB_TS_DECL
   TB_TS(0);
   constexpr int NQ = C / 80, MH = 8 / NQ, BM = 16 * MI * MH, QBN = BM / 32;
@@ -503,7 +518,7 @@
   constexpr int KPITCH = ((2 * KSTEPS) | 1) * 16, VPITCH = (DBLK | 1) * 64;
   constexpr int KVSTAGE = KEYS * (KPITCH + VPITCH);
   constexpr int NCHUNK = KEYS * CH, LD_IT = (NCHUNK + 255) / 256;
-  extern __shared__ __attribute__((aligned(16))) char smem[];
+  static_assert(!KEEP || (C == 320 && MI == 4), "the merged block tail: C = 320 only");
   char* panel = smem;
   char* kvs = smem + BM * PITCH;
   float* lnst = (float*)(kvs + 2 * KVSTAGE);
@@ -564,7 +579,6 @@
   const XOff<C> xo(q, px);
   const char* xrow = panel + rbase * PITCH;
   f32x4 acc[MI][NI];
-  u32x4 ring[TB_F];
   const unsigned lane16 = (unsigned)lane * 16u;
   const unsigned wbase = __builtin_amdgcn_readfirstlane((unsigned)(nq * KS * NI) * 1024u);
   auto gemm_head = [&](const bf16_t* wf) { panel_gemm_head<C>(ring, wf, wbase, lane16); };
@@ -836,7 +850,11 @@
 #pragma unroll
     for (int i = 0; i < MI; ++i) load_row_chunk<NI>((PRE ? (const bf16_t*)p.out : p.h) + (long long)((PRE ? m0 : m0s) + rbase + 16 * i) * C + ncol0, fr[i]);
   };
-  gemm_body_late(p.wof, ld_fr);
+  if constexpr (KEEP) {
+    if constexpr (KEEP == 2) panel_gemm_body<C, true, MI, decltype(ld_fr)&, true>(ring, acc, p.wof, wbase, lane16, xrow, xo, (unsigned)(C * C * 2), ld_fr, nextw, nextbytes, nextbase);
+    else gemm_body_late(p.wof, ld_fr);
+    __syncthreads();
+  } else gemm_body_late(p.wof, ld_fr);
   TB_TS(32);
   float bv[NI * 4];
 #pragma unroll
@@ -857,6 +875,14 @@
       const float a0 = __uint_as_float(pk[0] << 16), a1 = __uint_as_float(pk[0] & 0xFFFF0000u), a2 = __uint_as_float(pk[1] << 16), a3 = __uint_as_float(pk[1] & 0xFFFF0000u);
       rs[i] += (a0 + a1) + (a2 + a3); rq[i] += (a0 * a0 + a1 * a1) + (a2 * a2 + a3 * a3);
     }
+    if constexpr (KEEP) {
+#pragma unroll
+      for (int t = 0; t < NI; ++t) {
+        const int row = rbase + 16 * i, n = ncol0 + 4 * t;
+        *(u32x2*)(panel + row * PITCH + panel_swz<C>(n >> 3, row) * 16 + (n & 7) * 2) = pkk[t];
+      }
+      continue;
+    }
 #pragma unroll
     for (int t = 0; t < NI; ++t) *(u32x2*)(ostg + (16 * (i & 1) + px) * 160 + 40 * q + 8 * t) = pkk[t];
     if (i & 1) {
@@ -887,7 +913,24 @@
       *(f32x2_t*)(p.rowstat_out + (long long)(m0 + tid) * 2) = f32x2_t{S, Q};
     }
   }
+  if constexpr (KEEP) { __syncthreads(); return; }
   TB_TS_END;
+}
+template <int C, int PRE, int MI = 4>
+__global__ __launch_bounds__(512, 2) void attn_chain_kernel(const AttnChainP p) {
+  extern __shared__ __attribute__((aligned(16))) char smem[];
+  u32x4 ring[TB_F];
+  attn_chain_body<C, PRE, MI, 0>(p, smem, ring);
+}
+
+template <int PRE, int POST>
+__global__ __launch_bounds__(512, 2) void tail_attn_chain_kernel(const AttnChainP pa, const FFusedP pf) {
+  extern __shared__ __attribute__((aligned(16))) char smem[];
+  u32x4 ring[TB_F];
+  const int wid = __builtin_amdgcn_readfirstlane(threadIdx.x >> 6);
+  const float c0 = ff_chunk0_const<320>(pf, threadIdx.x, wid);
+  attn_chain_body<320, PRE, 4, 2>(pa, smem, ring, pf.w1f, (unsigned)(2 * 4 * 320 * 320 * 2), (unsigned)(wid & 3) * (320 / 32) * 4 * 1024u);
+  ff_fused_body<320, 0, POST, true, true>(pf, smem, ring, c0);
 }
 
 int launch_attn_chain(const AttnChainP& p, int C, int heads, hipStream_t st) {
@@ -917,6 +960,36 @@
   return 0;
 }
 
+int launch_attn_chain_ff(const AttnChainP& ap, const FFusedP& fp, int heads, hipStream_t st) {
+  constexpr int C = 320, BM = 128;
+  if (heads != 8) { agd_set_error("attn_chain_ff: heads = %d is not built (8 only)", heads); return -1; }
+  if (ap.M < BM || ap.M % BM || ap.HW % BM || ap.M % ap.HW) { agd_set_error("attn_chain_ff: M %d / HW %d must be multiples of %d (whole images)", ap.M, ap.HW, BM); return -1; }
+  if (ap.T < 1 || ap.T > 96) { agd_set_error("attn_chain_ff: %d keys (1..96)", ap.T); return -1; }
+  if ((long long)ap.M * C * 2 >= (1LL << 31)) { agd_set_error("attn_chain_ff: activation too large for 32-bit offsets"); return -1; }
+  if (ap.record && (ap.rec_hpb < 1 || 8 % ap.rec_hpb || !ap.rec)) { agd_set_error("attn_chain_ff: recorder head group %d", ap.rec_hpb); return -1; }
+  const bool pre = ap.o1 != nullptr;
+  if (pre && (!ap.wo1f || !ap.bo1 || ap.out == ap.h)) { agd_set_error("attn_chain_ff: the to_out prologue needs its weights and out != h"); return -1; }
+  if (ap.src_rows > 0 && (ap.src_rows % BM || ap.M % ap.src_rows)) { agd_set_error("attn_chain_ff: src_rows %d must divide M and be a multiple of %d", ap.src_rows, BM); return -1; }
+  if (fp.M != ap.M || !fp.w1f || !fp.w2f || !fp.cs1 || !fp.b1 || !fp.b2) { agd_set_error("attn_chain_ff: bad feed-forward arguments"); return -1; }
+  if (fp.wpf ? (!fp.bp || !fp.xres || !fp.pout) : !fp.out) { agd_set_error("attn_chain_ff: the feed-forward needs an output (with proj_out: bias, residual and output)"); return -1; }
+  if (fp.premul && !fp.wpf) { agd_set_error("attn_chain_ff: the pre-multiplied form is the proj_out stage's"); return -1; }
+  constexpr int lds = 128 * 320 * 2 + 2 * 128 * 128 * 2 + 128 * 8 + 3 * 4 * 128 * 4;
+  static_assert(lds >= 128 * 320 * 2 + 2 * 96 * (7 * 16 + 3 * 64) + 128 * 8 + 4 * 128 * 8 + 2 * 320 * 4, "LDS: the maximum of the two phases");
+  const int post = fp.wpf ? (fp.premul ? 2 : 1) : 0;
+  static const void* const kfns[2][3] = {{(const void*)tail_attn_chain_kernel<0, 0>, (const void*)tail_attn_chain_kernel<0, 1>, (const void*)tail_attn_chain_kernel<0, 2>},
+                                         {(const void*)tail_attn_chain_kernel<1, 0>, (const void*)tail_attn_chain_kernel<1, 1>, (const void*)tail_attn_chain_kernel<1, 2>}};
+  const void* kfn = kfns[pre ? 1 : 0][post];
+  static std::atomic<bool> attr[AGD_MAX_DEVICES][6] = {};
+  int dev = 0; HIP_CHECK_RET(hipGetDevice(&dev));
+  if (dev < 0 || dev >= AGD_MAX_DEVICES) { agd_set_error("attn_chain_ff: device ordinal %d out of range", dev); return -1; }
+  const int slot = (pre ? 3 : 0) + post;
+  if (!attr[dev][slot]) { HIP_CHECK_RET(hipFuncSetAttribute(kfn, hipFuncAttributeMaxDynamicSharedMemorySize, lds)); attr[dev][slot] = true; }
+  AttnChainP pa = ap; FFusedP pf = fp;
+  void* args[] = {&pa, &pf};
+  HIP_CHECK_RET(hipLaunchKernel(kfn, dim3(ap.M / BM), dim3(512), args, lds, st));
+  return 0;
+}
+
 template <int C, int MH = 8 / (C / 80)>
 __global__ __launch_bounds__(64 * MH * (C / 80), 2) void qkv_chain_kernel(const QkvChainP p) {
   constexpr int NQ = C / 80, BM = 64 * MH, KS = C / 32, NI = 5, PITCH = C * 2, NT = 64 * MH * NQ;
diff --git a/agenda_amd/ops.py b/agenda_amd/ops.py
--- a/agenda_amd/ops.py
+++ b/agenda_amd/ops.py
@@ -138,6 +138,31 @@
                                      _lib.ptr(_f32c(bo)), _lib.ptr(y), _lib.ptr(pr), B, HW, T, Cc, heads | (256 if rows32 else 0), float(eps), _lib.current_stream_ptr()),
                None, "agd_op_attn_chain")
     return (y, pr) if return_probs else y
+
+
+def attn_chain_ff(x, g2, be2, wq, kv, wo, bo, g3, be3, w1, b1, w2, b2, *, one_launch, o1=None, wo1=None, bo1=None, wp=None, bp=None, xres=None,
+                  premul=False, shared=False, record=True, record_half=False, heads=8, eps=1e-5):
+    lib = _lib.load()
+    x, kv = _f32c(x), _f32c(kv)
+    B, T = kv.shape[0], kv.shape[1]
+    HW, Cc = x.shape[1], x.shape[2]
+    assert Cc == 320 and x.shape[0] == (B // 2 if shared else B)
+    opt = lambda t: _f32c(t) if t is not None else None
+    o1, wo1, bo1, wp, bp, xres = opt(o1), opt(wo1), opt(bo1), opt(wp), opt(bp), opt(xres)
+    out = {"y": torch.empty(B, HW, Cc, device=x.device, dtype=torch.float32)}
+    if wp is not None:
+        out["colstat"] = torch.zeros(max(B * HW // 128, 1), Cc, 2, device=x.device, dtype=torch.float32)
+    if record:
+        out["probs"] = torch.empty(B - (B // 2 if record_half else 0), T, HW, device=x.device, dtype=torch.float32)
+    flags = (1 if one_launch else 0) | (2 if premul else 0) | (4 if shared else 0) | (8 if record_half else 0)
+    keep = [_f32c(t) for t in (g2, be2, wq, wo, bo, g3, be3, w1, b1, w2, b2)]
+    g2, be2, wq, wo, bo, g3, be3, w1, b1, w2, b2 = keep
+    _lib.check(lib.agd_op_attn_chain_ff(_lib.ptr(x), _lib.ptr(g2), _lib.ptr(be2), _lib.ptr(wq), _lib.ptr(kv), _lib.ptr(wo), _lib.ptr(bo),
+                                        _lib.ptr(o1), _lib.ptr(wo1), _lib.ptr(bo1), _lib.ptr(g3), _lib.ptr(be3), _lib.ptr(w1), _lib.ptr(b1),
+                                        _lib.ptr(w2), _lib.ptr(b2), _lib.ptr(wp), _lib.ptr(bp), _lib.ptr(xres), _lib.ptr(out["y"]),
+                                        _lib.ptr(out.get("colstat")), _lib.ptr(out.get("probs")), B, HW, T, heads, float(eps), flags,
+                                        _lib.current_stream_ptr()), None, "agd_op_attn_chain_ff")
+    return out
 
 
 def xattn_premul(x, gamma, beta, wq, kv, wo, bo, heads=8, eps=1e-5, return_probs=False):
diff --git a/include/agenda_hip.h b/include/agenda_hip.h
--- a/include/agenda_hip.h
+++ b/include/agenda_hip.h
@@ -197,6 +197,11 @@
                     const float* b2, float* y, int M, int C, float eps, void* stream);
 int agd_op_attn_chain(const float* x, const float* gamma, const float* beta, const float* wq, const float* kv, const float* wo,
                       const float* bo, float* y, float* probs_sum, int B, int HW, int T, int C, int heads, float eps, void* stream);
+int agd_op_attn_chain_ff(const float* x, const float* g2, const float* be2, const float* wq, const float* kv, const float* wo, const float* bo,
+                         const float* o1, const float* wo1, const float* bo1,
+                         const float* g3, const float* be3, const float* w1, const float* b1, const float* w2, const float* b2,
+                         const float* wp, const float* bp, const float* xres, float* y, float* colstat, float* probs_sum,
+                         int B, int HW, int T, int heads, float eps, int flags, void* stream);
 int agd_op_xattn_premul(const float* x, const float* gamma, const float* beta, const float* wq, const float* kv, const float* wo,
                         const float* bo, float* y, float* probs, int B, int HW, int T, int C, int heads, float eps, void* stream);
 int agd_op_groupnorm(const float* x_nchw, const float* gamma, const float* beta, float* y_nchw, int B, int C, int HW,
```

New measurement: 9.344, median of 4. About the same (+0.1%).
